# timweiland/DiffEqGMRFs.jl

Hardware: AMD Instinct MI355X
Metric: GMRF posterior solves/sec (mean+samples), 256^2 Darcy (higher is better)
Workload: dtype f64; 1 GPU; darcy256: n=65536, 64 blocks x 1024, nnz=1624084; 256 independent posterior(s) per GPU and step (4 stream(s) x batch 64), each factor + mean + 64 samples; mode=problems, samples_per_problem_per_rank=64, l_blocks_kept=False

## Files before the change

### diffeqgmrfs.jl_amd/_cabi.py

```python
from __future__ import annotations

import ctypes as C
import os
from typing import Optional

_HERE = os.path.dirname(os.path.abspath(__file__))
LIB_PATH = os.environ.get("GMRF_HIP_LIBRARY") or os.path.join(_HERE, "csrc", "libgmrf_hip.so")

GMRF_OK = 0
ERR_NOT_SPD, ERR_BAD_SHAPE, ERR_BAND, ERR_HIP, ERR_NO_FACTOR, ERR_NO_DEVICE, ERR_ALLOC, ERR_RCCL = -1, -2, -3, -4, -5, -6, -7, -8
SOLVE_FULL, SOLVE_FORWARD, SOLVE_BACKWARD = 0, 1, 2
VAR_EXACT, VAR_RBMC, VAR_MC = 0, 1, 2
BLOCK_L, BLOCK_C, BLOCK_LINV = 0, 1, 2
ORDER_REFERENCE, ORDER_TWISTED = 0, 1

EXPORTS = [
    "gmrf_bt_create", "gmrf_bt_destroy", "gmrf_last_error", "gmrf_version",
    "gmrf_bt_factor_csc", "gmrf_bt_factor_blocks", "gmrf_bt_refactor_values",
    "gmrf_bt_solve", "gmrf_bt_sample", "gmrf_bt_posterior", "gmrf_bt_set_factor_rhs", "gmrf_bt_normals", "gmrf_bt_marginal_var",
    "gmrf_bt_var_accumulate", "gmrf_bt_logdet", "gmrf_bt_get_block", "gmrf_bt_factor_buffer",
    "gmrf_bt_adopt_shape", "gmrf_bt_adopt_commit", "gmrf_bt_adopt_layout", "gmrf_bt_get_layout", "gmrf_bt_block_range",
    "gmrf_bt_set_keep_l", "gmrf_bt_storage_bytes", "gmrf_bt_set_storage", "gmrf_bt_factor_begin_csc",
    "gmrf_bt_factor_step_async", "gmrf_bt_factor_end", "gmrf_bt_stats",
    "gmrf_bt_set_profiling", "gmrf_bt_set_eager", "gmrf_bt_synchronize", "gmrf_bt_set_batch", "gmrf_bt_select_problem",
    "gmrf_bt_marginal_var_batch", "gmrf_bt_selinv", "gmrf_bt_trace_inv", "gmrf_bt_set_order", "gmrf_bt_get_order", "gmrf_bt_half_stats", "gmrf_bt_export_size", "gmrf_bt_export_factor", "gmrf_bt_import_factor",
    "gmrf_comm_unique_id", "gmrf_comm_create", "gmrf_comm_destroy", "gmrf_comm_bcast_host", "gmrf_comm_allreduce_sum",
    "gmrf_bt_bcast_blocks_async", "gmrf_bt_allgather_blocks_async", "gmrf_comm_wait", "gmrf_comm_bytes", "gmrf_streams_create", "gmrf_streams_destroy",
    "gmrf_bt_packed_size", "gmrf_bt_pack_blocks_async", "gmrf_bt_unpack_blocks_async",
    "gmrf_csr_create", "gmrf_csr_destroy", "gmrf_spmm", "gmrf_spmm_rows", "gmrf_spmm_async", "gmrf_spmm_rows_async",
    "gmrf_darcy_p1_create", "gmrf_darcy_p2_create", "gmrf_darcy_p1_destroy", "gmrf_darcy_p1_pattern", "gmrf_darcy_p1_assemble",
    "gmrf_burgers_p1_create", "gmrf_burgers_p2_create", "gmrf_burgers_line_create", "gmrf_burgers_colloc_create", "gmrf_burgers_p1_destroy", "gmrf_burgers_p1_pattern", "gmrf_burgers_p1_tangent",
    "gmrf_shallow_water_p1_create", "gmrf_shallow_water_p1_destroy", "gmrf_shallow_water_p1_pattern", "gmrf_shallow_water_p1_qpoints",
    "gmrf_shallow_water_p1_assemble", "gmrf_shallow_water_p1_operators",
    "gmrf_assemble_create", "gmrf_assemble_destroy", "gmrf_assemble_pattern", "gmrf_assemble_precision", "gmrf_assemble_rhs",
    "gmrf_burgers_p1_tangent_batch", "gmrf_assemble_precision_batch", "gmrf_assemble_rhs_batch", "gmrf_assemble_objective_batch",
    "gmrf_gn_create", "gmrf_gn_destroy", "gmrf_gn_run", "gmrf_gn_finalize",
    "gmrf_elliptic_p1_create", "gmrf_elliptic_p2_create", "gmrf_elliptic_p1_destroy", "gmrf_elliptic_p1_pattern", "gmrf_elliptic_p1_qpoints",
    "gmrf_elliptic_p1_tangent", "gmrf_elliptic_p1_tangent_batch", "gmrf_elliptic_p1_load", "gmrf_gn_create_elliptic",
    "gmrf_darcy_p1_assemble_batch", "gmrf_dc_create", "gmrf_dc_destroy", "gmrf_dc_run",
    "gmrf_burgers_prior_create", "gmrf_burgers_line_prior_create", "gmrf_burgers_prior_destroy", "gmrf_burgers_prior_pattern", "gmrf_burgers_prior_values_batch",
    "gmrf_bic_create", "gmrf_bic_destroy", "gmrf_bic_run", "gmrf_field_errors_batch",
    "gmrf_bt_logdet_batch", "gmrf_assemble_quadform_batch", "gmrf_gn_posterior",
    "gmrf_test_gemm", "gmrf_test_gemm_desc", "gmrf_test_gemm_pair", "gmrf_test_gemm_rate", "gmrf_test_gemm_shapes", "gmrf_test_potrf_tile", "gmrf_test_potrf_block", "gmrf_test_potrf_route", "gmrf_test_tile_timing", "gmrf_test_persist_stamps", "gmrf_test_persist_aborts", "gmrf_test_factor_fwd", "gmrf_test_gn_route", "gmrf_test_dc_route", "gmrf_test_bic_route", "gmrf_test_var_groups", "gmrf_test_persist_budget", "gmrf_test_clock_probe_start", "gmrf_test_clock_probe_finish",
    "gmrf_test_mfma_f64_rate", "gmrf_test_hbm_rate", "gmrf_test_microbench", "gmrf_test_symbolic_csc",
]


class SparseBlock(C.Structure):
    _fields_ = [("nnz", C.c_int64), ("ptr", C.c_void_p), ("idx", C.c_void_p), ("val", C.c_void_p)]


class Stats(C.Structure):
    _fields_ = [
        ("factor_ms", C.c_double), ("solve_ms", C.c_double), ("sample_ms", C.c_double),
        ("factor_flops", C.c_double), ("sweep_bytes", C.c_double), ("sweep_ms", C.c_double),
        ("n", C.c_int64), ("n_blocks", C.c_int64), ("block_size", C.c_int64),
        ("block_size_padded", C.c_int64), ("factor_bytes", C.c_int64),
        ("kernel_ms", C.c_double * 24), ("kernel_work", C.c_double * 24), ("kernel_launches", C.c_int64 * 24),
        ("sweep_bytes_streamed", C.c_double),
        ("persist_route", C.c_int32), ("persist_aborts", C.c_int32), ("persist_cus", C.c_int32), ("persist_refused", C.c_int32),
        ("sweep_persist", C.c_int32), ("sweep_persist_launches", C.c_int32),
    ]


class GmrfError(RuntimeError):
    def __init__(self, status: int, msg: str, info: int = 0):
        super().__init__(f"libgmrf_hip status {status}: {msg}")
        self.status = status
        self.info = info


class NotPositiveDefinite(GmrfError):
    """Julia's PosDefException(info): `.info` is the failing block (1-based)."""


_lib: Optional[C.CDLL] = None


def load() -> C.CDLL:
    global _lib
    if _lib is not None:
        return _lib
    if not os.path.exists(LIB_PATH):
        raise ImportError(
            f"{LIB_PATH} is missing: build it with `python -c 'import __graft_entry__ as g; g.build()'` "
            "or `make -C diffeqgmrfs.jl_amd/csrc` (the HIP library is the only compute path)")
    try:
        import torch
    except Exception:
        pass
    lib = C.CDLL(LIB_PATH)
    vp, i32, i64, u64, dbl = C.c_void_p, C.c_int32, C.c_int64, C.c_uint64, C.c_double
    P = C.POINTER
    sigs = {
        "gmrf_bt_create": [i32, vp, P(vp)],
        "gmrf_bt_destroy": [vp],
        "gmrf_version": [],
# ... 65 lines not shown
        "gmrf_burgers_p1_create": [i32, vp, i64, i64, dbl, dbl, P(vp)],
        "gmrf_burgers_p2_create": [i32, vp, i64, i64, dbl, dbl, P(vp)],
        "gmrf_burgers_line_create": [i32, vp, i64, i64, dbl, dbl, i32, i32, i32, dbl, P(vp)],
        "gmrf_burgers_colloc_create": [i32, vp, i64, i64, dbl, dbl, dbl, i64, vp, P(vp)],
        "gmrf_burgers_p1_destroy": [vp],
        "gmrf_burgers_p1_pattern": [vp, P(i64), vp, vp, i32],
        "gmrf_burgers_p1_tangent": [vp, vp, vp, vp],
        "gmrf_burgers_p1_tangent_batch": [vp, i64, vp, vp, vp],
        "gmrf_assemble_precision_batch": [vp, i64, vp, i64, vp, dbl, vp],
        "gmrf_assemble_rhs_batch": [vp, i64, vp, vp, vp, vp, dbl, vp],
        "gmrf_assemble_objective_batch": [vp, i64, vp, i64, vp, vp, vp, dbl, vp],
        "gmrf_gn_create": [vp, vp, vp, P(vp)],
        "gmrf_gn_create_elliptic": [vp, vp, vp, P(vp)],
        "gmrf_elliptic_p1_create": [i32, vp, i64, i64, P(vp)],
        "gmrf_elliptic_p2_create": [i32, vp, i64, i64, P(vp)],
        "gmrf_elliptic_p1_destroy": [vp],
        "gmrf_elliptic_p1_pattern": [vp, P(i64), vp, vp, i32],
        "gmrf_elliptic_p1_qpoints": [vp, vp],
        "gmrf_elliptic_p1_tangent": [vp, vp, vp, vp],
        "gmrf_elliptic_p1_tangent_batch": [vp, i64, vp, vp, vp],
        "gmrf_elliptic_p1_load": [vp, i64, vp, vp],
        "gmrf_gn_destroy": [vp],
        "gmrf_gn_run": [vp, vp, i64, vp, vp, vp, vp, dbl, dbl, i32, vp, vp, P(i32)],
        "gmrf_gn_finalize": [vp, P(i32)],
        "gmrf_darcy_p1_assemble_batch": [vp, i64, vp, i64, dbl, vp, vp],
        "gmrf_dc_create": [vp, vp, vp, P(vp)],
        "gmrf_dc_destroy": [vp],
        "gmrf_dc_run": [vp, vp, i64, dbl, vp, i64, vp, dbl, i64, u64, i32, i64, u64, vp, vp, vp, vp, P(i32)],
        "gmrf_burgers_prior_create": [i32, vp, i64, i64, dbl, dbl, dbl, P(vp)],
        "gmrf_burgers_line_prior_create": [i32, vp, i64, i64, dbl, dbl, dbl, i32, i32, dbl, dbl, i32, P(vp)],
        "gmrf_burgers_prior_destroy": [vp],
        "gmrf_burgers_prior_pattern": [vp, P(i64), vp, vp, i32],
        "gmrf_burgers_prior_values_batch": [vp, i64, vp, vp, vp, vp],
        "gmrf_bic_create": [vp, vp, vp, P(vp)],
        "gmrf_bic_destroy": [vp],
        "gmrf_bic_run": [vp, vp, vp, vp, vp, vp, P(i32)],
        "gmrf_field_errors_batch": [i32, vp, i64, i64, i64, vp, vp, vp],
        "gmrf_bt_logdet_batch": [vp, vp],
        "gmrf_assemble_quadform_batch": [vp, i64, vp, i64, vp, vp, vp],
        "gmrf_gn_posterior": [vp, vp, i64, i64, u64, i32, i64, u64, vp, vp, vp, vp, vp, vp, vp, P(i32)],
        "gmrf_shallow_water_p1_create": [i32, vp, i64, i64, P(vp)],
        "gmrf_shallow_water_p1_destroy": [vp],
        "gmrf_shallow_water_p1_pattern": [vp, i32, P(i64), vp, vp, i32],
        "gmrf_shallow_water_p1_qpoints": [vp, vp],
        "gmrf_shallow_water_p1_assemble": [vp, vp, dbl, dbl, dbl, vp, vp, vp, vp],
        "gmrf_shallow_water_p1_operators": [vp, vp, vp, vp, vp, dbl, dbl, dbl, vp, vp, vp, vp],
        "gmrf_spmm": [vp, vp, vp, i64, i64, i64],
        "gmrf_spmm_async": [vp, vp, vp, i64, i64, i64],
        "gmrf_spmm_rows_async": [vp, vp, vp, i64, i64, i64],
        "gmrf_spmm_rows": [vp, vp, vp, i64, i64, i64],
        "gmrf_test_gemm": [i32, i64, i64, i64, i32, i32, i32, i32, dbl, vp, i64, vp, i64, dbl, vp, i64],
        "gmrf_test_gemm_shapes": [vp, P(dbl), i64, P(i64)],
        "gmrf_test_gemm_desc": [i32, i32, vp, vp] + [vp, i64] * 12 + [P(i32)],
        "gmrf_test_gemm_pair": [i32, i32, i32, vp, vp, vp, vp, vp, vp, vp, vp],
        "gmrf_test_gemm_rate": [i32, i64, i64, i64, i32, i32, i32, i32, i32, i32, P(dbl)],
        "gmrf_test_potrf_tile": [i32, vp, vp, P(i32)],
        "gmrf_test_potrf_block": [i32, i64, vp, vp, P(i32)],
        "gmrf_test_potrf_route": [i32, i64, i32, i32, i64, i32, vp, vp, vp, P(i32), P(i32)],
        "gmrf_test_tile_timing": [vp, i32],
        "gmrf_test_persist_stamps": [vp, i32],
        "gmrf_test_persist_aborts": [vp, vp],
        "gmrf_test_factor_fwd": [vp, vp, vp],
        "gmrf_test_gn_route": [vp, P(i32), P(i32)],
        "gmrf_test_dc_route": [vp, vp],
        "gmrf_test_bic_route": [vp, vp],
        "gmrf_test_var_groups": [vp, vp, vp],
        "gmrf_test_persist_budget": [i32, i32, vp, vp],
        "gmrf_test_clock_probe_start": [i32, i32, i32, P(vp)],
        "gmrf_test_clock_probe_finish": [vp, vp, vp],
        "gmrf_test_mfma_f64_rate": [i32, P(dbl)],
        "gmrf_test_hbm_rate": [i32, i64, P(dbl)],
        "gmrf_test_microbench": [i32, vp, i32],
        "gmrf_test_symbolic_csc": [i64, i64, vp, vp, i32, vp],
    }
    for name, args in sigs.items():
        fn = getattr(lib, name)
        fn.argtypes = args
        fn.restype = i32
    lib.gmrf_last_error.argtypes = []
    lib.gmrf_last_error.restype = C.c_char_p
    _lib = lib
    return lib


def check(status: int, info: int = 0):
    if status == GMRF_OK:
        return
    msg = load().gmrf_last_error().decode(errors="replace")
    if status == ERR_NOT_SPD:
        raise NotPositiveDefinite(status, msg, info)
    raise GmrfError(status, msg, info)


def ptr(a) -> C.c_void_p:
    if a is None:
        return C.c_void_p(0)
    if isinstance(a, int):
        return C.c_void_p(a)
    if hasattr(a, "data_ptr"):
        return C.c_void_p(a.data_ptr())
    return C.c_void_p(a.ctypes.data)
```

### diffeqgmrfs.jl_amd/api.py

```python
from __future__ import annotations

import ctypes as C
from typing import List, Optional, Sequence, Tuple

import numpy as np
import scipy.sparse as sp

from . import _cabi
from ._cabi import GmrfError, NotPositiveDefinite


def _is_torch(x) -> bool:
    return hasattr(x, "data_ptr") and hasattr(x, "device")


def _colmajor(b, n: int):
    if _is_torch(b):
        import torch
        if b.dtype != torch.float64:
            raise TypeError("float64 required")
        if b.dim() == 1:
            if b.shape[0] != n:
                raise ValueError("dimension mismatch")
            return b.contiguous(), 1, n, True
# ... 1147 lines not shown
    def trace_inv(self, S: CsrMatrix, dvals):
        nd = 2 if self.batch == 1 else 3
        if dvals.ndim != nd or dvals.shape[-1] != S.nnz or (nd == 3 and dvals.shape[0] != self.batch):
            want = "(m, nnz)" if nd == 2 else "(batch, m, nnz)"
            raise ValueError(f"dvals must be {want} with nnz = {S.nnz}")
        m = int(dvals.shape[-2])
        if _is_torch(dvals):
            import torch
            if dvals.dtype != torch.float64:
                raise TypeError("float64 required")
            dvals = dvals.contiguous()
            out = torch.empty(dvals.shape[:-1], dtype=torch.float64, device=dvals.device)
        else:
            dvals = np.ascontiguousarray(dvals, dtype=np.float64)
            out = np.empty(dvals.shape[:-1], dtype=np.float64)
        _cabi.check(self._lib.gmrf_bt_trace_inv(self._h, S._h, _cabi.ptr(dvals), m, _cabi.ptr(out)))
        return out

    @staticmethod
    def _out_array(out, shape):
        if out is None:
            return np.empty(shape, dtype=np.float64)
        ok = tuple(out.shape) == shape and (out.is_contiguous() and str(out.dtype) == "torch.float64" if _is_torch(out)
                                            else out.flags.c_contiguous and out.dtype == np.float64)
        if not ok:
            raise ValueError(f"out must be a contiguous float64 array of shape {shape}")
        return out

    def var_accumulate(self, acc, method: str, first_id: int, k: int, seed: int = 0x5EED,
                       Q: Optional[CsrMatrix] = None):
        m = {"rbmc": _cabi.VAR_RBMC, "mc": _cabi.VAR_MC}[method]
        _cabi.check(self._lib.gmrf_bt_var_accumulate(self._h, m, first_id, k, seed,
                                                     Q._h if Q is not None else None, _cabi.ptr(acc)))
        return acc

    def stats(self) -> dict:
        s = _cabi.Stats()
        _cabi.check(self._lib.gmrf_bt_stats(self._h, C.byref(s)))
        out = {}
        for f, _ in s._fields_:
            v = getattr(s, f)
            out[f] = list(v) if hasattr(v, "__len__") else v
        return out

    def gemm_shapes(self) -> list:
        n = C.c_int64(0)
        _cabi.check(self._lib.gmrf_test_gemm_shapes(self._h, None, 0, C.byref(n)))
        buf = np.zeros((max(int(n.value), 1), 11))
        _cabi.check(self._lib.gmrf_test_gemm_shapes(self._h, buf.ctypes.data_as(C.POINTER(C.c_double)), buf.shape[0], C.byref(n)))
        names = ("class", "M", "N", "K", "tri", "lower_only", "problems", "k_bounds")
        return [dict({k: int(r[i]) for i, k in enumerate(names)}, launches=int(r[8]), ms=float(r[9]), flops=float(r[10]))
                for r in buf[: int(n.value)]]

    def set_profiling(self, level: int):
        _cabi.check(self._lib.gmrf_bt_set_profiling(self._h, level))

    def set_eager(self, eager: bool):
        _cabi.check(self._lib.gmrf_bt_set_eager(self._h, int(eager)))

    def synchronize(self):
        _cabi.check(self._lib.gmrf_bt_synchronize(self._h))

    def factor_buffer(self, kind: int) -> Tuple[int, int]:
        p = C.c_void_p()
        nbytes = C.c_int64(0)
        _cabi.check(self._lib.gmrf_bt_factor_buffer(self._h, kind, C.byref(p), C.byref(nbytes)))
        return int(p.value or 0), int(nbytes.value)

    def export_factor(self) -> np.ndarray:
        nbytes = C.c_int64(0)
        _cabi.check(self._lib.gmrf_bt_export_size(self._h, C.byref(nbytes)))
        buf = np.empty(nbytes.value, dtype=np.uint8)
        _cabi.check(self._lib.gmrf_bt_export_factor(self._h, _cabi.ptr(buf), nbytes.value))
        return buf

    def import_factor(self, image: np.ndarray):
        image = np.ascontiguousarray(image, dtype=np.uint8)
        _cabi.check(self._lib.gmrf_bt_import_factor(self._h, _cabi.ptr(image), image.size))
        hdr = image[:64].view(np.int64)
        self._set_shape(int(hdr[2]), int(hdr[3]))
        return self

    def adopt_shape(self, n: int, n_blocks: int):
        _cabi.check(self._lib.gmrf_bt_adopt_shape(self._h, n, n_blocks))
        self._set_shape(n, n_blocks)

    def get_layout(self) -> np.ndarray:
        cnt = C.c_int64(0)
        _cabi.check(self._lib.gmrf_bt_get_layout(self._h, None, 0, C.byref(cnt)))
        out = np.zeros(cnt.value, dtype=np.int64)
        _cabi.check(self._lib.gmrf_bt_get_layout(self._h, _cabi.ptr(out), out.size, C.byref(cnt)))
        return out

    def adopt_layout(self, n: int, n_blocks: int, layout=None):
        if layout is None:
            _cabi.check(self._lib.gmrf_bt_adopt_layout(self._h, n, n_blocks, None, 0))
        else:
            lay = np.ascontiguousarray(layout, dtype=np.int64)
            _cabi.check(self._lib.gmrf_bt_adopt_layout(self._h, n, n_blocks, _cabi.ptr(lay), lay.size))
        self._set_shape(n, n_blocks)

    def adopt_commit(self, l_blocks_valid: bool = False):
        _cabi.check(self._lib.gmrf_bt_adopt_commit(self._h, int(l_blocks_valid)))

    def set_keep_l(self, keep: bool):
        _cabi.check(self._lib.gmrf_bt_set_keep_l(self._h, int(keep)))
# ... 177 lines not shown
```

### diffeqgmrfs.jl_amd/csrc/gemm_f64.hpp

```cpp
#pragma once
#include <hip/hip_runtime.h>
#include <hip/hip_ext.h>
#include <stdint.h>
#include <stdlib.h>
#include <algorithm>
#include <array>
#include <map>
#include <mutex>
#include <vector>

namespace gmrf {

typedef double v4d __attribute__((ext_vector_type(4)));
typedef double v2d __attribute__((ext_vector_type(2)));

enum : int {
    TRI_A_LOWER = 1,
    TRI_A_UPPER = 2,
    TRI_B_LOWER = 4,
    TRI_B_UPPER = 8
};

struct GemmDirectOut {
    double* samples;
    double* mean;
    int64_t ld, k;
};

struct GemmArgs {
    const double* A;
    const double* B;
    double* C;
    int64_t lda, ldb, ldc;
    int64_t strideA, strideB, strideC;
    int64_t pA, pB, pC;
    int nb1;
    int M, N, K;
    int tri;
    int lower_only;
    double alpha, beta;
    const double* D;
    int64_t ldd, pD;
    unsigned long long* stamps;
    const int* kb_m = nullptr;
    const int* kb_n = nullptr;
    const int* ke_n = nullptr;
    const double* tA = nullptr;
    double* tC = nullptr;
    const double* tD = nullptr;
    int64_t ptA = 0, ptC = 0, ptD = 0;
    double tbeta = 0.0;
    const GemmDirectOut* dout = nullptr;
    int64_t o_j0 = 0, o_n = 0;
    int o_cols = 0;
};

constexpr int GEMM_BM = 64;
constexpr int GEMM_BN = 64;

template <bool ROWS_CONTIG, int BK>
__device__ __forceinline__ void gemm_load_tile(const double* __restrict__ P, int64_t ld, int row0, int k0,
                                               int t, v2d (&rg)[BK / 8]) {
    if (!ROWS_CONTIG) {
        constexpr int TPR = BK / 2, RPP = 256 / TPR;
        const int r = t / TPR, kk = (t % TPR) * 2;
        const double* p = P + (int64_t)(row0 + r) * ld + k0 + kk;
#pragma unroll
        for (int i = 0; i < BK / 8; ++i) rg[i] = *reinterpret_cast<const v2d*>(p + (int64_t)(i * RPP) * ld);
    } else {
        const int kk = t >> 5, r = (t & 31) * 2;
        const double* p = P + (int64_t)(k0 + kk) * ld + row0 + r;
#pragma unroll
        for (int i = 0; i < BK / 8; ++i) rg[i] = *reinterpret_cast<const v2d*>(p + (int64_t)(i * 8) * ld);
    }
}

template <bool ROWS_CONTIG, int BK>
__device__ __forceinline__ void gemm_tile_offsets(int64_t ld, int row0, int t, uint32_t (&off)[BK / 8]) {
    if (!ROWS_CONTIG) {
        constexpr int TPR = BK / 2, RPP = 256 / TPR;
        const int r = t / TPR, kk = (t % TPR) * 2;
#pragma unroll
        for (int i = 0; i < BK / 8; ++i) off[i] = (uint32_t)(((int64_t)(row0 + r + i * RPP) * ld + kk) * 8);
    } else {
        const int kk = t >> 5, r = (t & 31) * 2;
#pragma unroll
        for (int i = 0; i < BK / 8; ++i) off[i] = (uint32_t)(((int64_t)(kk + i * 8) * ld + row0 + r) * 8);
    }
}
template <bool ROWS_CONTIG>
__device__ __forceinline__ const char* gemm_tile_base(const double* P, int64_t ld, int k0) {
    return reinterpret_cast<const char*>(ROWS_CONTIG ? P + (int64_t)k0 * ld : P + k0);
}
template <int BK>
__device__ __forceinline__ void gemm_load_tile_off(const char* base, uint32_t (&off)[BK / 8], v2d (&rg)[BK / 8]) {
#pragma unroll
    for (int i = 0; i < BK / 8; ++i) {
        asm volatile("" : "+v"(off[i]));
        rg[i] = *reinterpret_cast<const v2d*>(base + off[i]);
// ... 632 lines not shown
```

### diffeqgmrfs.jl_amd/csrc/gemm_f64_dma.hpp

```cpp
#pragma once
#include "gemm_f64.hpp"

namespace gmrf {

constexpr int DMA_BK = 16;
constexpr int DMA_ROWS_ASCENDING = 1024;
#ifndef GMRF_DMA_READS_FIRST
#define GMRF_DMA_READS_FIRST 0
#endif

template <int BM, int BN>
constexpr size_t gemm_dma_lds_bytes(int stages) { return (size_t)stages * (BM + BN) * DMA_BK * sizeof(double); }

#define GMRF_LDS_PTR(p) ((__attribute__((address_space(3))) void*)(p))
#define GMRF_GLB_PTR(p) ((const __attribute__((address_space(1))) void*)(p))

template <int BM, int BN>
__device__ __forceinline__ void gemm_dma_tile_order(const GemmArgs& g, int bid, int gdim, int& bm, int& bn, int& z) {
    const int nx = g.N / BN, ny = g.M / BM;
    int tpp;
    if (g.lower_only == 1) {
        if (BM >= BN) tpp = (BM / BN) * ny * (ny + 1) / 2;
        else tpp = 0;
    } else tpp = nx * ny;
// ... 4 lines not shown
    if (g.lower_only == 1) {
        constexpr int R = BM / BN > 0 ? BM / BN : 1;
        const int tile = q % tpp;
        zq = q / tpp;
        const int tr = (g.tri & DMA_ROWS_ASCENDING) ? tile : tpp - 1 - tile;
        int b = (int)((sqrtf(8.0f * (float)(tr / R) + 1.0f) - 1.0f) * 0.5f);
        while (R * b * (b + 1) / 2 > tr) --b;
        while (R * (b + 1) * (b + 2) / 2 <= tr) ++b;
        bm = b;
        bn = tr - R * b * (b + 1) / 2;
    } else {
        const bool cls_n = (g.tri & (TRI_B_LOWER | TRI_B_UPPER)) || !(g.tri & (TRI_A_LOWER | TRI_A_UPPER));
        const bool desc = cls_n ? ((g.tri & TRI_B_UPPER) != 0 || (g.ke_n && !g.kb_n)) : (g.tri & TRI_A_LOWER) != 0;
        const int ncls = cls_n ? nx : ny, other = cls_n ? ny : nx;
        int c = q / (other * nzg);
        const int rem = q % (other * nzg);
        const int o = rem % other;
        zq = rem / other;
        if (desc) c = ncls - 1 - c;
        bn = cls_n ? c : o;
        bm = cls_n ? o : c;
    }
    z = xg + groups * zq;
}

template <int BM, int BN, bool B_N, int STAGES, bool A_T, bool TAIL, bool DOUT>
__device__ __forceinline__ void gemm_dma_body(const GemmArgs& g, const int bid, const int gdim) {
    constexpr int BK = DMA_BK;
    constexpr int MI = BM / 32, NJ = BN / 32;
    constexpr int NA = BM / 32, NB = BN / 32;
    constexpr int A_ST = BM * BK, B_ST = BN * BK, T_ST = TAIL ? BK : 0, ST = A_ST + B_ST + T_ST;
    static_assert(NJ % 2 == 0 || !B_N, "the [k][n] image pairs neighbouring column tiles");
    static_assert(MI % 2 == 0 || !A_T, "the [k][m] image pairs neighbouring row tiles");
    static_assert(!TAIL || (BM == 64 && BN == 64 && !A_T), "the tail row: 64 x 64 tiles");
    static_assert(!DOUT || (TAIL && B_N), "direct output: the tail-row product on B [k][n]");
    int bm, bn, z;
    gemm_dma_tile_order<BM, BN>(g, bid, gdim, bm, bn, z);
    const bool tail_owner = TAIL && (g.lower_only == 1 ? bm == bn : bm == g.M / BM - 1);
    const bool tail = DOUT || tail_owner;
    const int m0 = bm * BM, n0 = bn * BN;
    if (g.lower_only == 2 && n0 > m0 + BM - 1) return;
    const int zi = z % g.nb1, zp = z / g.nb1;
    const double* __restrict__ A = g.A + (int64_t)zi * g.strideA + (int64_t)zp * g.pA;
    const double* __restrict__ B = g.B + (int64_t)zi * g.strideB + (int64_t)zp * g.pB;
    double* C = g.C + (int64_t)zi * g.strideC + (int64_t)zp * g.pC;
    const double* Dm = g.D ? g.D + (int64_t)zp * g.pD : C;
    const int64_t ldd = g.D ? g.ldd : g.ldc;

    int kb = 0, ke = g.K;
    if (g.tri & TRI_A_LOWER) ke = min(ke, m0 + BM);
    if (g.tri & TRI_A_UPPER) kb = max(kb, m0);
    if (g.tri & TRI_B_LOWER) kb = max(kb, n0);
    if (g.tri & TRI_B_UPPER) ke = min(ke, n0 + BN);
    if (g.kb_m) kb = max(kb, g.kb_m[bm * (BM / 64)]);
    if (g.kb_n) kb = max(kb, g.kb_n[bn * (BN / 64)]);
    if (g.ke_n) ke = min(ke, g.ke_n[bn * (BN / 64) + BN / 64 - 1]);
    const int nkt = (ke > kb) ? (ke - kb) / BK : 0;

    extern __shared__ __attribute__((aligned(16))) double gsm[];
    const int t = threadIdx.x;
    const int lane = t & 63, w = __builtin_amdgcn_readfirstlane(t >> 6);
    const int wm = (w >> 1) * (BM / 2), wn = (w & 1) * (BN / 2);
    const int li = lane & 15, lq = lane >> 4;
    const bool idle = g.lower_only != 0 && ((n0 + wn) / 64 > (m0 + wm + BM / 2 - 1) / 64);

    uint32_t offa[NA], offb[NB];
#pragma unroll
    for (int i = 0; i < NA; ++i) {
        const int q = w + 4 * i;
        if (A_T) {
            constexpr int LPR = BM / 2;
            const int k = q * (64 / LPR) + lane / LPR, col = (lane % LPR) * 2;
            offa[i] = (uint32_t)(((int64_t)k * g.lda + m0 + col) * 8);
        } else {
            const int row = 8 * q + (lane >> 3), ch = (lane & 7) ^ ((row >> 1) & 7);
            offa[i] = (uint32_t)(((int64_t)(m0 + row) * g.lda + 2 * ch) * 8);
        }
    }
#pragma unroll
    for (int i = 0; i < NB; ++i) {
        const int q = w + 4 * i;
        if (B_N) {
            constexpr int LPR = BN / 2;
            const int k = q * (64 / LPR) + lane / LPR, col = (lane % LPR) * 2;
            offb[i] = (uint32_t)(((int64_t)k * g.ldb + n0 + col) * 8);
        } else {
            const int row = 8 * q + (lane >> 3), ch = (lane & 7) ^ ((row >> 1) & 7);
            offb[i] = (uint32_t)(((int64_t)(n0 + row) * g.ldb + 2 * ch) * 8);
        }
    }
    const double* arow = g.tC ? g.tA + (int64_t)zp * g.ptA : A + (int64_t)g.M * g.lda;
    auto issue = [&](int kt, int stage) {
        const int k0 = kb + kt * BK;
        const char* abase = reinterpret_cast<const char*>(A_T ? A + (int64_t)k0 * g.lda : A + k0);
        const char* bbase = reinterpret_cast<const char*>(B_N ? B + (int64_t)k0 * g.ldb : B + k0);
        double* as = gsm + stage * ST;
        double* bs = as + A_ST;
        if constexpr (TAIL)
            if (tail && w == 0 && lane < 8)
                __builtin_amdgcn_global_load_lds(GMRF_GLB_PTR(arow + k0 + 2 * lane), GMRF_LDS_PTR(bs + B_ST), 16, 0, 0);
#pragma unroll
        for (int i = 0; i < NA; ++i) {
            asm volatile("" : "+v"(offa[i]));
            __builtin_amdgcn_global_load_lds(GMRF_GLB_PTR(abase + offa[i]), GMRF_LDS_PTR(as + (w + 4 * i) * 128), 16, 0, 0);
        }
#pragma unroll
        for (int i = 0; i < NB; ++i) {
            asm volatile("" : "+v"(offb[i]));
            __builtin_amdgcn_global_load_lds(GMRF_GLB_PTR(bbase + offb[i]), GMRF_LDS_PTR(bs + (w + 4 * i) * 128), 16, 0, 0);
// ... 193 lines not shown
                    if (beta != 0.0) v += beta * Dm[(int64_t)g.M * ldd + n0 + lane];
                    C[(int64_t)g.M * g.ldc + n0 + lane] = v;
                }
            }
        }
    }
}

__global__ void set_direct_out(GemmDirectOut* o, double* samples, double* mean, int64_t ld, int64_t k) {
    o->samples = samples; o->mean = mean; o->ld = ld; o->k = k;
}

template <int BM, int BN, bool B_N, int STAGES, bool A_T = false, bool TAIL = false, bool DOUT = false>
__global__ __launch_bounds__(256, (BM + BN > 128) ? 3 : 4) void gemm_f64_dma(GemmArgs g) {
    gemm_dma_body<BM, BN, B_N, STAGES, A_T, TAIL, DOUT>(g, (int)blockIdx.x, (int)gridDim.x);
}

template <int STAGES>
__global__ __launch_bounds__(256, 4) void gemm_f64_dma_grouped(GemmArgs g0, GemmArgs g1, int wg0, int wg1, int b_n) {
    const bool second = (int)blockIdx.x >= wg0;
    const GemmArgs g = second ? g1 : g0;
    const int bid = second ? (int)blockIdx.x - wg0 : (int)blockIdx.x, gdim = second ? wg1 : wg0;
    if ((b_n >> (second ? 1 : 0)) & 1) gemm_dma_body<64, 64, true, STAGES, false, false, false>(g, bid, gdim);
    else gemm_dma_body<64, 64, false, STAGES, false, false, false>(g, bid, gdim);
}

inline int& gemm_dma_policy() {
    static int v = [] { const char* e = getenv("GMRF_GEMM_DMA"); return e ? atoi(e) : 2; }();
    return v;
}
inline int& gemm_dma_force() {
    static int v = 0;
    return v;
}
inline int gemm_dma_stages() {
    static const int v = [] { const char* e = getenv("GMRF_GEMM_DMA_STAGES"); const int s = e ? atoi(e) : 2; return s == 3 ? 3 : 2; }();
    return v;
}

inline int gemm_dma_shape(bool a_t, const GemmArgs& g, int batch) {
    const int policy = gemm_dma_force() ? 2 : gemm_dma_policy();
    if (policy == 0 || g.stamps || (g.tri & ~15) || g.K % DMA_BK || g.M % 64 || g.N % 64) return 0;
    if ((g.lda & 1) || (g.ldb & 1) || ((uintptr_t)g.A & 15) || ((uintptr_t)g.B & 15) || ((g.strideA | g.strideB | g.pA | g.pB) & 1)) return 0;
    if (((uintptr_t)g.C & 15) || (g.ldc & 1) || ((g.strideC | g.pC) & 1)) return 0;
    if (g.D && (((uintptr_t)g.D & 15) || (g.ldd & 1) || (g.pD & 1))) return 0;
    if ((int64_t)g.M * g.ldc * 8 >= ((int64_t)1 << 32) || (g.D && (int64_t)g.M * g.ldd * 8 >= ((int64_t)1 << 32))) return 0;
    if ((int64_t)(a_t ? g.K : g.M) * g.lda * 8 >= ((int64_t)1 << 32) || (int64_t)std::max(g.N, g.K) * g.ldb * 8 >= ((int64_t)1 << 32)) return 0;
    if (a_t) return 1;
    const int force = gemm_dma_force();
    if (force == 2 && g.M % 128 == 0) return 2;
    if (force == 3 && g.N % 128 == 0 && !g.lower_only) return 3;
    if (force) return 1;
    if (policy == 1) return 1;
    const bool plain = !g.lower_only && !g.tri && !g.kb_m && !g.kb_n && !g.ke_n;
    const int64_t t64 = (int64_t)(g.M / 64) * (g.N / 64) * batch;
    if (policy >= 3 || (plain && t64 >= 2048)) {
        if (g.M % 128 == 0) return 2;
        if (g.N % 128 == 0 && !g.lower_only) return 3;
    }
    return 1;
}
inline bool gemm_uses_dma(bool a_t, const GemmArgs& g, int batch) { return gemm_dma_shape(a_t, g, batch) != 0; }

inline hipError_t gemm_dma_init() {
    hipError_t e = hipSuccess;
#define GMRF_DMA_ATTR(BM, BN, BNAT, ST)                                                                          \
    if (e == hipSuccess)                                                                                          \
        e = hipFuncSetAttribute((const void*)gemm_f64_dma<BM, BN, BNAT, ST>, hipFuncAttributeMaxDynamicSharedMemorySize, \
                                (int)gemm_dma_lds_bytes<BM, BN>(ST) + 64 * 1024);
    GMRF_DMA_ATTR(64, 64, false, 2) GMRF_DMA_ATTR(64, 64, true, 2) GMRF_DMA_ATTR(64, 64, false, 3) GMRF_DMA_ATTR(64, 64, true, 3)
    GMRF_DMA_ATTR(128, 64, false, 2) GMRF_DMA_ATTR(128, 64, true, 2) GMRF_DMA_ATTR(128, 64, false, 3) GMRF_DMA_ATTR(128, 64, true, 3)
    GMRF_DMA_ATTR(64, 128, false, 2) GMRF_DMA_ATTR(64, 128, true, 2) GMRF_DMA_ATTR(64, 128, false, 3) GMRF_DMA_ATTR(64, 128, true, 3)
#undef GMRF_DMA_ATTR
    return e;
}

inline bool gemm_tail_ok(bool a_t, bool b_n, const GemmArgs& g, int batch) {
    if (a_t || gemm_uses_ll(g, batch) || gemm_dma_shape(false, g, batch) != 1) return false;
    if (g.lower_only && g.M != g.N) return false;
    if (g.tC && g.dout) return false;
    if (g.tC) {
        return g.nb1 == 1 && g.tA && ((uintptr_t)g.tA & 15) == 0 && (g.ptA & 1) == 0;
    }
    if (!b_n || g.lower_only) return false;
    if (g.dout && g.nb1 != 1) return false;
    if (g.dout && (g.beta != 0.0 || g.kb_m || g.kb_n || g.ke_n || (g.tri & (TRI_A_LOWER | TRI_A_UPPER)))) return false;
    return (int64_t)(g.M + 1) * g.ldc * 8 < ((int64_t)1 << 32) && (!g.D || (int64_t)(g.M + 1) * g.ldd * 8 < ((int64_t)1 << 32));
}
inline bool gemm_try_dma_tail(hipStream_t st, bool a_t, bool b_n, const GemmArgs& g, int batch, hipEvent_t ev_start, hipEvent_t ev_stop,
                              hipError_t* err) {
    if (!gemm_tail_ok(a_t, b_n, g, batch)) return false;
    const bool tri_grid = g.lower_only && g.M == g.N;
    GemmArgs gs = g;
    gs.lower_only = tri_grid ? 1 : 0;
    static const bool asc_off = [] { const char* e = getenv("GMRF_GEMM_G2_ORDER"); return e && atoi(e) == 0; }();
    if (tri_grid && (g.kb_m || g.kb_n) && !asc_off) gs.tri |= DMA_ROWS_ASCENDING;
    const int64_t nx = g.N / 64, ny = g.M / 64;
    const dim3 grid((unsigned)((tri_grid ? ny * (ny + 1) / 2 : nx * ny) * batch)), block(256);
    const size_t lds = (size_t)gemm_dma_stages() * (64 + 64 + DMA_BK) * DMA_BK * sizeof(double);
#define GMRF_DMA_TK(BNAT, ST)                                                                                              \
    do {                                                                                                                   \
        if (ev_start) hipExtLaunchKernelGGL((gemm_f64_dma<64, 64, BNAT, ST, false, true>), grid, block, lds, st, ev_start, ev_stop, 0, gs); \
        else hipLaunchKernelGGL((gemm_f64_dma<64, 64, BNAT, ST, false, true>), grid, block, lds, st, gs);                \
    } while (0)
#define GMRF_DMA_TKO(ST)                                                                                                   \
    do {                                                                                                                   \
        if (ev_start) hipExtLaunchKernelGGL((gemm_f64_dma<64, 64, true, ST, false, true, true>), grid, block, lds, st, ev_start, ev_stop, 0, gs); \
        else hipLaunchKernelGGL((gemm_f64_dma<64, 64, true, ST, false, true, true>), grid, block, lds, st, gs);          \
    } while (0)
    if (g.dout) {
        if (gemm_dma_stages() == 3) GMRF_DMA_TKO(3); else GMRF_DMA_TKO(2);
    } else if (gemm_dma_stages() == 3) {
        if (b_n) GMRF_DMA_TK(true, 3); else GMRF_DMA_TK(false, 3);
    } else {
        if (b_n) GMRF_DMA_TK(true, 2); else GMRF_DMA_TK(false, 2);
    }
#undef GMRF_DMA_TKO
#undef GMRF_DMA_TK
    *err = hipGetLastError();
    return true;
}

inline bool gemm_try_dma(hipStream_t st, bool a_t, bool b_n, const GemmArgs& g, int batch, hipEvent_t ev_start, hipEvent_t ev_stop,
                         hipError_t* err) {
    const int shape = gemm_dma_shape(a_t, g, batch);
    if (shape == 0) return false;
    const bool tri_grid = g.lower_only && g.M == g.N;
    GemmArgs gs = g;
    gs.lower_only = tri_grid ? 1 : (g.lower_only ? 2 : 0);
    static const bool asc_off = [] { const char* e = getenv("GMRF_GEMM_G2_ORDER"); return e && atoi(e) == 0; }();
    if (tri_grid && (g.kb_m || g.kb_n) && !asc_off) gs.tri |= DMA_ROWS_ASCENDING;
    const int stages = gemm_dma_stages();
    const dim3 block(256);
#define GMRF_DMA_GO(BM, BN)                                                                                       \
    do {                                                                                                          \
        const int64_t nx = g.N / BN, ny = g.M / BM;                                                               \
        const int64_t tiles = tri_grid ? (int64_t)(BM / BN > 0 ? BM / BN : 1) * ny * (ny + 1) / 2 : nx * ny;      \
        const dim3 grid((unsigned)(tiles * batch));                                                               \
        static const size_t lds_pad = [] { const char* e = getenv("GMRF_GEMM_DMA_LDS_PAD_KB"); return (size_t)(e ? atoi(e) : 0) * 1024; }();    \
// ... 61 lines not shown
```

### diffeqgmrfs.jl_amd/csrc/gmrf_hip.hip

```cpp
#include <hip/hip_runtime.h>
#include <dlfcn.h>
#include <stdint.h>
#include <stdlib.h>
#include <string.h>
#include <time.h>

#include <algorithm>
#include <atomic>
#include <iterator>
#include <cmath>
#include <map>
#include <memory>
#include <chrono>
#include <functional>
#include <initializer_list>
#include <mutex>
#include <string>
#include <type_traits>
#include <vector>

#include "../../include/gmrf_hip.h"
#include "assemble.hpp"
#include "fem_assemble.hpp"
#include "burgers_line.hpp"
// ... 81 lines not shown
    float* d_vals32 = nullptr;
    double* d_diag = nullptr;
    bool tiles128_ok = false;
    bool tiles_ok = false;
    DevBuf stage_x, stage_y;
    int plan_state = 0;
    int64_t* d_tile_uptr = nullptr;
    int32_t* d_ucols = nullptr;
    uint16_t* d_lidx = nullptr;
    int64_t n_ucols = 0;
    int plan_rows = 0, plan_ucap = 0, plan_ecap = 0, plan_ecap_pad = 0, plan_umax = 0;
    uint64_t id = 0;
};
static std::atomic<uint64_t> g_csr_ids{0};

struct EvPair {
    hipEvent_t a, b;
    int kind;
    double work;
    int shape = -1;
};

struct GemmShapeStat {
    int64_t key[8];
    double launches = 0, ms = 0, work = 0;
};

struct TwistState;

struct gmrf_handle {
    int device = 0;
    hipStream_t stream = nullptr;
    bool own_stream = false;
    int64_t n = 0, N = 0, bs = 0, bsp = 0, n_pad = 0;
    int64_t B = 1;
    int64_t sel = 0;
    int64_t alloc_B = 0, vals_B = 0;
    int64_t nnz_in = 0, n_entries = 0;
    uint64_t* d_keys = nullptr;
    double* d_vals = nullptr;
    int64_t* d_src = nullptr;
    double* d_nz_stage = nullptr;
    std::vector<int64_t> diag_first, diag_count, low_first, low_count;
    bool analyzed = false;
    int64_t cmin = 0, rmax = 0;
    std::vector<int> kst, mend;
    int* d_kst = nullptr;
    int* d_mend = nullptr;
    int* d_kbx = nullptr;
    int kst_cap = 0;
    double c_streamed = 0.0;
    double g2_tile_k = 0.0;
    bool c_dirty = false;
    int* d_lo_rowptr = nullptr;
    int* d_dg_rowptr = nullptr;
    int* d_bxt_uptr = nullptr; int* d_bxt_ucols = nullptr; uint16_t* d_bxt_lidx = nullptr; int* d_bxt_gtiles = nullptr;
    std::vector<int> bxt_ng;
    int bxt_ecap = 0; int bxt_nrt = 0; bool bxt_plan_ok = false;
    int64_t lo_row_max = 0;
    bool sparse_b = false;
    bool dense_g1 = false;
    double *d_L = nullptr, *d_C = nullptr, *d_Linv = nullptr;
    bool external_storage = false;
    bool keep_l = true;
    bool l_valid = false;
    bool logdet_valid = false;
    std::vector<char> got_block;
    int64_t alloc_rm = 0, alloc_wc = 0;
    bool alloc_keep_l = true;
    double *d_S = nullptr, *d_B = nullptr, *d_T = nullptr, *d_W = nullptr;
    double* d_V = nullptr;
    int64_t v_elems = 0;
    uint64_t layout_gen = 0;
    uint64_t sel_csr = 0, sel_gen = ~0ull;
    int64_t sel_nnz = 0;
    std::vector<int64_t> sel_off, sel_nd;
    int64_t* d_sel_src = nullptr;
    int64_t* d_sel_slot = nullptr;
    int64_t sel_cap = 0;
    double* d_sig = nullptr;
    int64_t sig_elems = 0;
    double* d_dv = nullptr;
    int64_t dv_elems = 0;
    int* d_info = nullptr;
    double* d_logdet = nullptr;
    int64_t alloc_N = 0, alloc_bsp = 0;
    bool factored = false;
    double *d_P = nullptr, *d_Y = nullptr, *d_Tp = nullptr;
    int64_t kp_cap = 0;
    double* d_stage = nullptr;
    int64_t stage_cap = 0;
    DevBuf mean_arena;
    double* d_acc = nullptr;
    int64_t acc_B = 0;
    int32_t var_group = 0, var_groups = 0;
    bool eager = false;
    bool split_step = false;
    bool sweep_no_gemm = false;
    bool no_fused_posterior = false;
    bool tail_probe = false;
    bool tail_refused = false;
    const double* frhs = nullptr;
    const double* fy_for = nullptr;
    bool fwd_run = false;
    bool no_factor_fwd = false;
    bool no_grouped_gemm = false;
// ... 113 lines not shown
            (void)hipEventRecord(p.a, h->stream);
        }
    }
    ~ProfScope() {
        if (on) {
            (void)hipEventRecord(p.b, h->stream);
            h->events.push_back(p);
        }
    }
};

static void prof_collect(gmrf_handle* h) {
    for (auto& p : h->events) {
        float ms = 0.f;
        (void)hipEventElapsedTime(&ms, p.a, p.b);
        h->stats.kernel_ms[p.kind] += ms; h->stats.kernel_work[p.kind] += p.work; h->stats.kernel_launches[p.kind]++;
        if (p.shape >= 0) { auto& g = h->gemm_shapes[(size_t)p.shape]; g.launches += 1; g.ms += ms; g.work += p.work; }
        h->ev_pool.push_back(p.a);
        h->ev_pool.push_back(p.b);
    }
    h->events.clear();
}

struct GemmTail {
    const double* A; int64_t pA;
    double* C; int64_t pC;
    const double* D; int64_t pD;
    double beta;
    const GemmDirectOut* out = nullptr;
    int64_t j0 = 0;
    int cols = 0;
};

static inline double gemm_flops(int M, int N, int K, int tri, int lower_only, double nprob) {
    double flops = 2.0 * M * N * (double)K * nprob;
    if (lower_only) flops *= 0.5 * (1.0 + 64.0 / std::max(M, 64));
    if (tri) flops *= 0.5 * (1.0 + 64.0 / std::max(K, 64));
    return flops;
}
static int gemm_shape_row(gmrf_handle* h, const int64_t (&key)[8]) {
    for (size_t i = 0; i < h->gemm_shapes.size(); ++i)
        if (!memcmp(h->gemm_shapes[i].key, key, sizeof(key))) return (int)i;
    GemmShapeStat st; memcpy(st.key, key, sizeof(key));
    h->gemm_shapes.push_back(st);
    return (int)h->gemm_shapes.size() - 1;
}

static gmrf_status gemm(gmrf_handle* h, bool a_t, bool b_n, int M, int N, int K, int tri, int lower_only,
                        double alpha, const double* A, int64_t lda, const double* B, int64_t ldb,
                        double beta, double* C, int64_t ldc, int64_t pA, int64_t pB, int64_t pC,
                        int batch = 1, int64_t sA = 0, int64_t sB = 0, int64_t sC = 0, const double* D = nullptr,
                        int64_t ldd = 0, int64_t pD = 0, int pclass = 0, double pwork = -1.0,
                        const int* kb_m = nullptr, const int* kb_n = nullptr, const int* ke_n = nullptr, bool tail = false,
                        const GemmTail* gt = nullptr) {
    GemmArgs g;
    if (gt) {
        if (gt->C) { g.tA = gt->A; g.ptA = gt->pA; g.tC = gt->C; g.ptC = gt->pC; g.tD = gt->D; g.ptD = gt->pD; g.tbeta = gt->beta; }
        g.dout = gt->out; g.o_j0 = gt->j0; g.o_cols = gt->cols; g.o_n = h->n;
        tail = true;
    }
    g.kb_m = kb_m; g.kb_n = kb_n; g.ke_n = ke_n;
    g.D = D; g.ldd = ldd; g.pD = pD;
    g.A = A; g.B = B; g.C = C;
    g.lda = lda; g.ldb = ldb; g.ldc = ldc;
    g.strideA = sA; g.strideB = sB; g.strideC = sC;
    g.pA = pA; g.pB = pB; g.pC = pC; g.nb1 = batch;
    g.M = M; g.N = N; g.K = K; g.tri = tri; g.lower_only = lower_only;
    g.alpha = alpha; g.beta = beta; g.stamps = nullptr;
    double flops = gemm_flops(M, N, K, tri, lower_only, batch * (double)h->B);
    if (tail) {
        if (!gemm_tail_ok(a_t, b_n, g, batch * (int)h->B)) {
            h->tail_refused = true;
            return h->tail_probe ? GMRF_OK : bad_shape("internal: a product does not qualify for the tail-row GEMM");
        }
        if (h->tail_probe) return GMRF_OK;
        flops *= (M + 1.0) / M;
        if (pwork >= 0.0) pwork *= (M + 1.0) / M;
        pclass = b_n ? 15 : 14;
        hipError_t e = hipSuccess;
        if (h->profiling > 0) {
            EvPair p;
            p.kind = pclass; p.work = pwork >= 0.0 ? pwork : flops;
            p.a = ev_get(h); p.b = ev_get(h);
            const int64_t key[8] = {pclass, M + 1, N, K, tri, lower_only, batch * h->B, (kb_m || kb_n || ke_n) ? 1 : 0};
            p.shape = gemm_shape_row(h, key);
            (void)gemm_try_dma_tail(h->gemm_stream ? h->gemm_stream : h->stream, a_t, b_n, g, batch * (int)h->B, p.a, p.b, &e);
            HIPCHK(e);
            h->events.push_back(p);
            return GMRF_OK;
        }
        (void)gemm_try_dma_tail(h->gemm_stream ? h->gemm_stream : h->stream, a_t, b_n, g, batch * (int)h->B, nullptr, nullptr, &e);
        HIPCHK(e);
        return GMRF_OK;
    }
    if (gemm_uses_big(a_t, g, batch * (int)h->B)) { pclass = b_n ? 7 : 6; pwork = -1.0; }
    else if (pclass == 0) {
        if (gemm_uses_ll(g, batch * (int)h->B)) pclass = 13;
        else if (gemm_uses_dma(a_t, g, batch * (int)h->B)) pclass = a_t ? 18 : (b_n ? 15 : 14);
        else pclass = a_t ? 12 : (b_n ? 11 : 0);
    }
    if (h->profiling > 0) {
        EvPair p;
        p.kind = pclass; p.work = pwork >= 0.0 ? pwork : flops;
        p.a = ev_get(h); p.b = ev_get(h);
        const int64_t key[8] = {pclass, M, N, K, tri, lower_only, batch * h->B, (kb_m || kb_n || ke_n) ? 1 : 0};
        p.shape = gemm_shape_row(h, key);
        HIPCHK(launch_gemm(h->gemm_stream ? h->gemm_stream : h->stream, a_t, b_n, g, batch * (int)h->B, p.a, p.b));
        h->events.push_back(p);
        return GMRF_OK;
    }
    HIPCHK(launch_gemm(h->gemm_stream ? h->gemm_stream : h->stream, a_t, b_n, g, batch * (int)h->B));
    return GMRF_OK;
}

struct GemmOne {
    bool b_n; int M, N, K, tri, lower_only;
    double alpha; const double* A; int64_t lda; const double* B; int64_t ldb; double beta; double* C; int64_t ldc;
    int64_t pA, pB, pC;
    double pwork;
};
static gmrf_status gemm_one(gmrf_handle* h, const GemmOne& q) {
    return gemm(h, false, q.b_n, q.M, q.N, q.K, q.tri, q.lower_only, q.alpha, q.A, q.lda, q.B, q.ldb, q.beta, q.C, q.ldc, q.pA, q.pB, q.pC,
                1, 0, 0, 0, nullptr, 0, 0, 0, q.pwork);
}
static gmrf_status gemm_pair(gmrf_handle* h, const GemmOne& q0, const GemmOne& q1) {
    GemmArgs g[2];
    const GemmOne* q[2] = {&q0, &q1};
    double work[2];
    for (int i = 0; i < 2; ++i) {
        GemmArgs& a = g[i];
        a.A = q[i]->A; a.B = q[i]->B; a.C = q[i]->C; a.lda = q[i]->lda; a.ldb = q[i]->ldb; a.ldc = q[i]->ldc;
        a.strideA = a.strideB = a.strideC = 0;
        a.pA = q[i]->pA; a.pB = q[i]->pB; a.pC = q[i]->pC; a.nb1 = 1;
        a.M = q[i]->M; a.N = q[i]->N; a.K = q[i]->K; a.tri = q[i]->tri; a.lower_only = q[i]->lower_only;
        a.alpha = q[i]->alpha; a.beta = q[i]->beta; a.D = nullptr; a.ldd = 0; a.pD = 0; a.stamps = nullptr;
        work[i] = q[i]->pwork >= 0.0 ? q[i]->pwork : gemm_flops(a.M, a.N, a.K, a.tri, a.lower_only, (double)h->B);
    }
    if (h->no_grouped_gemm || !gemm_grouped_ok(g[0], g[1], (int)h->B)) {
        GCHK(gemm_one(h, q0));
        return gemm_one(h, q1);
    }
    hipStream_t st = h->gemm_stream ? h->gemm_stream : h->stream;
    hipError_t e = hipSuccess;
    if (h->profiling > 0) {
        EvPair p;
        p.kind = 14; p.work = work[0] + work[1];
        p.a = ev_get(h); p.b = ev_get(h);
        const int64_t key[8] = {14, q0.M + q1.M, q0.N, q0.K, q0.tri | (q1.tri << 8), q0.lower_only | (q1.lower_only << 8), h->B, 0};
        p.shape = gemm_shape_row(h, key);
        (void)gemm_try_dma_grouped(st, q0.b_n, g[0], q1.b_n, g[1], (int)h->B, p.a, p.b, &e);
        HIPCHK(e);
        h->events.push_back(p);
        return GMRF_OK;
    }
    (void)gemm_try_dma_grouped(st, q0.b_n, g[0], q1.b_n, g[1], (int)h->B, nullptr, nullptr, &e);
    HIPCHK(e);
    return GMRF_OK;
}

static inline int64_t blk_elems(const gmrf_handle* h) { return h->bsp * h->bsp; }
static inline int64_t c_ld(const gmrf_handle* h) { return h->bsp - h->cmin; }
static inline int64_t c_blk(const gmrf_handle* h) { return h->rmax * (h->bsp - h->cmin); }
static inline int64_t stride_pL(const gmrf_handle* h) { return blk_elems(h) * (h->keep_l ? h->N : 1); }
static inline int64_t stride_pX(const gmrf_handle* h) { return blk_elems(h) * h->N; }
static inline int64_t stride_pC(const gmrf_handle* h) { return c_blk(h) * std::max<int64_t>(h->N - 1, 1); }
static inline double* l_block(const gmrf_handle* h, int64_t i) { return h->d_L + (h->keep_l ? i * blk_elems(h) : 0); }

static gmrf_status set_layout(gmrf_handle* h, int64_t cmin, int64_t rmax, const std::vector<int64_t>& kst_abs) {
    const int64_t bsp = h->bsp;
    if (cmin < 0 || cmin >= bsp || cmin % 64 || rmax <= 0 || rmax > bsp || rmax % 64) return bad_shape("bad coupling-block layout");
    const int nrt = (int)(rmax / 64), nct = (int)((bsp - cmin) / 64), ntile = (int)(bsp / 64);
    if ((int)kst_abs.size() != nrt) return bad_shape("bad coupling-block layout (row tiles)");
    (void)hipStreamSynchronize(h->stream);
    destroy_graphs(h);
    h->cmin = cmin; h->rmax = rmax;
    h->layout_gen++;
    h->kst.assign((size_t)ntile, 0);
    int64_t run = bsp - 64;
    for (int t = nrt - 1; t >= 0; --t) {
        int64_t v = std::min(std::max(kst_abs[t], cmin), bsp - 64);
        run = std::min(run, (v / 64) * 64);
        h->kst[t] = (int)(run - cmin);
    }
    if (nrt > 0) h->kst[0] = 0;
    for (int t = nrt; t < ntile; ++t) h->kst[t] = (int)(bsp - cmin);
    h->mend.assign((size_t)ntile, (int)rmax);
    for (int u = 0; u < nct; ++u) {
        int m = 0;
        for (int t = 0; t < nrt; ++t) if (h->kst[t] <= 64 * u) m = 64 * (t + 1);
        h->mend[u] = m;
    }
    h->c_streamed = 0.0; h->g2_tile_k = 0.0;
    for (int t = 0; t < nrt; ++t) {
        h->c_streamed += 64.0 * (double)(bsp - cmin - h->kst[t]);
        h->g2_tile_k += (double)(t + 1) * (double)(bsp - cmin - h->kst[t]);
    }
    if (!h->d_kst || !h->d_mend || h->kst_cap < ntile) {
        free_dev(h->d_kst); free_dev(h->d_mend); free_dev(h->d_kbx); h->d_kst = h->d_mend = h->d_kbx = nullptr; h->kst_cap = 0;
        HIPCHK(hipMalloc(&h->d_kst, sizeof(int) * ntile));
        HIPCHK(hipMalloc(&h->d_mend, sizeof(int) * ntile));
        HIPCHK(hipMalloc(&h->d_kbx, sizeof(int) * ntile));
        h->kst_cap = ntile;
    }
    {
        std::vector<int> kbx((size_t)ntile);
        for (int u = 0; u < ntile; ++u) kbx[(size_t)u] = (int)std::max<int64_t>(0, 64 * (int64_t)u - cmin);
        HIPCHK(hipMemcpyAsync(h->d_kbx, kbx.data(), sizeof(int) * ntile, hipMemcpyHostToDevice, h->stream));
        HIPCHK(hipStreamSynchronize(h->stream));
    }
    HIPCHK(hipMemcpyAsync(h->d_kst, h->kst.data(), sizeof(int) * ntile, hipMemcpyHostToDevice, h->stream));
    HIPCHK(hipMemcpyAsync(h->d_mend, h->mend.data(), sizeof(int) * ntile, hipMemcpyHostToDevice, h->stream));
    HIPCHK(hipStreamSynchronize(h->stream));
    h->c_dirty = true;
    return GMRF_OK;
}

static gmrf_status set_layout_dense(gmrf_handle* h) {
    return set_layout(h, 0, h->bsp, std::vector<int64_t>((size_t)(h->bsp / 64), 0));
}

static gmrf_status alloc_work(gmrf_handle* h);
static gmrf_status alloc_factor(gmrf_handle* h) {
    if (h->alloc_N == h->N && h->alloc_bsp == h->bsp && h->alloc_B == h->B && h->alloc_rm == h->rmax &&
        h->alloc_wc == c_ld(h) && h->alloc_keep_l == h->keep_l && h->d_Linv)
        return GMRF_OK;
    destroy_graphs(h);
    h->logdet_valid = false;
    if (h->external_storage) {
        if (h->alloc_N != h->N || h->alloc_bsp != h->bsp || h->alloc_B != h->B || h->alloc_keep_l != h->keep_l) {
// ... 62 lines not shown
    if (h->n != n || h->N != N) {
        (void)hipStreamSynchronize(h->stream);
        destroy_graphs(h);
        release_shape_buffers(h);
        h->factored = false;
        h->analyzed = false;
    }
    h->n = n; h->N = N; h->bs = bs;
    h->layout_gen++;
    h->bsp = 64 * next_pow2((bs + 63) / 64);
    h->n_pad = h->bsp * N;
    h->stats.n = n; h->stats.n_blocks = N; h->stats.block_size = bs; h->stats.block_size_padded = h->bsp;
    h->stats.factor_flops = ((double)N * bs * bs * bs / 3.0 + (double)(N - 1) * 2.0 * bs * bs * bs) * (double)h->B;
    return GMRF_OK;
}

static gmrf_status ensure_panels(gmrf_handle* h, int64_t kp) {
    if (kp <= h->kp_cap && h->d_P) return GMRF_OK;
    for (auto& kv : h->sweep_graphs) (void)hipGraphExecDestroy(kv.second);
    h->sweep_graphs.clear();
    free_dev(h->d_P); free_dev(h->d_Y); free_dev(h->d_Tp);
    h->d_P = h->d_Y = h->d_Tp = nullptr;
    HIPCHK(hipMalloc(&h->d_P, sizeof(double) * kp * h->n_pad * h->B));
    HIPCHK(hipMalloc(&h->d_Y, sizeof(double) * kp * h->n_pad * h->B));
    HIPCHK(hipMalloc(&h->d_Tp, sizeof(double) * kp * h->bsp * h->B));
    h->kp_cap = kp;
    return GMRF_OK;
}

static gmrf_status ensure_stage(gmrf_handle* h, int64_t elems) {
    if (elems <= h->stage_cap && h->d_stage) return GMRF_OK;
    free_dev(h->d_stage);
    h->d_stage = nullptr;
    HIPCHK(hipMalloc(&h->d_stage, sizeof(double) * elems));
    h->stage_cap = elems;
    return GMRF_OK;
}

struct HostEntry { uint64_t key; int64_t src; };

struct SymbolicPlan {
    std::vector<int64_t> diag_first, diag_count, low_first, low_count;
    std::vector<uint64_t> keys;
    std::vector<int64_t> src;
    int64_t cmin = 0, rmax = 0;
    std::vector<int64_t> first;
    std::vector<int> rowptr;
    int64_t max_row = 0;
    bool sparse_b = false, bxt_ok = false;
    std::vector<int> uptr, ucols, gtiles, ng;
    std::vector<uint16_t> lidx;
    int ecap = 0, nrt = 0;
    std::vector<int> drowptr;
};

static void build_symbolic(int64_t N, int64_t bsp, const std::vector<std::vector<HostEntry>>& dg,
                           const std::vector<std::vector<HostEntry>>& lo, bool no_staircase, SymbolicPlan& sp, bool group_tiles = true) {
    sp.diag_first.assign((size_t)N, 0); sp.diag_count.assign((size_t)N, 0);
    sp.low_first.assign((size_t)N, 0); sp.low_count.assign((size_t)N, 0);
    auto& keys = sp.keys; auto& src = sp.src;
    keys.clear(); src.clear();
    for (int64_t i = 0; i < N; ++i) {
        sp.diag_first[i] = (int64_t)keys.size(); sp.diag_count[i] = (int64_t)dg[i].size();
        {
            std::vector<HostEntry> drow(dg[i]);
            std::stable_sort(drow.begin(), drow.end(), [](const HostEntry& x, const HostEntry& y) { return x.key < y.key; });
            for (auto& e : drow) { keys.push_back(e.key); src.push_back(e.src); }
        }
        sp.low_first[i] = (int64_t)keys.size(); sp.low_count[i] = (int64_t)lo[i].size();
        std::vector<HostEntry> byrow(lo[i]);
        std::stable_sort(byrow.begin(), byrow.end(), [](const HostEntry& x, const HostEntry& y) { return x.key < y.key; });
        for (auto& e : byrow) { keys.push_back(e.key); src.push_back(e.src); }
    }
    {
        int64_t cmin = bsp, rmax = 0;
        std::vector<int64_t> first((size_t)(bsp / 64), bsp);
        for (int64_t i = 1; i < N; ++i)
            for (auto& e : lo[i]) {
                const int64_t r = (int64_t)(e.key >> 32), c = (int64_t)(e.key & 0xffffffffu);
                cmin = std::min(cmin, c); rmax = std::max(rmax, r + 1);
                first[(size_t)(r / 64)] = std::min(first[(size_t)(r / 64)], c);
            }
        if (rmax == 0) { cmin = 0; rmax = 64; first[0] = 0; }
        cmin = (cmin / 64) * 64;
        rmax = std::min<int64_t>(bsp, (rmax + 63) / 64 * 64);
        first.resize((size_t)(rmax / 64));
        if (no_staircase) std::fill(first.begin(), first.end(), cmin);
        sp.cmin = cmin; sp.rmax = rmax; sp.first = first;
    }
    sp.rowptr.assign((size_t)(N * (bsp + 1)), 0);
    int64_t max_row = 0;
    for (int64_t i = 1; i < N; ++i) {
        int* rp = sp.rowptr.data() + i * (bsp + 1);
        const int64_t first = sp.low_first[i], cnt = sp.low_count[i];
        for (int64_t k = 0; k < cnt; ++k) rp[(keys[first + k] >> 32) + 1]++;
        for (int64_t r = 0; r < bsp; ++r) max_row = std::max<int64_t>(max_row, rp[r + 1]);
        rp[0] = (int)first;
        for (int64_t r = 0; r < bsp; ++r) rp[r + 1] += rp[r];
    }
    sp.drowptr.assign((size_t)(N * (bsp + 1)), 0);
    if (keys.size() < ((size_t)1 << 31)) {
        for (int64_t i = 0; i < N; ++i) {
            int* rp = sp.drowptr.data() + i * (bsp + 1);
            const int64_t first = sp.diag_first[i], cnt = sp.diag_count[i];
            for (int64_t k = 0; k < cnt; ++k) rp[(keys[first + k] >> 32) + 1]++;
            rp[0] = (int)first;
            for (int64_t r = 0; r < bsp; ++r) rp[r + 1] += rp[r];
        }
    }
    sp.max_row = max_row;
    sp.sparse_b = keys.size() < ((size_t)1 << 31) && max_row <= 32 && bsp >= 64;
    sp.bxt_ok = false; sp.uptr.clear(); sp.ucols.clear(); sp.lidx.clear(); sp.gtiles.clear(); sp.ng.clear();
    if (sp.sparse_b && N > 1) {
        static const bool no_groups = [] { const char* e = getenv("GMRF_BXT_GROUPS"); return e && atoi(e) == 0; }();
        const int nrt = (int)(sp.rmax / 64);
        sp.uptr.assign((size_t)(N * (nrt + 1)), 0);
        sp.gtiles.assign((size_t)(N * nrt * 3), -1);
        sp.ng.assign((size_t)N, 0);
        sp.lidx.assign(std::max<size_t>(keys.size(), 1), 0);
        std::vector<std::vector<int>> cols((size_t)nrt);
        std::vector<int> uni, tmp;
        bool ok = true;
        int64_t pmax = 0;
        for (int64_t i = 1; i < N && ok; ++i) {
            const int* rp = sp.rowptr.data() + i * (bsp + 1);
            for (int rt = 0; rt < nrt; ++rt) {
                auto& c = cols[(size_t)rt];
                c.clear();
                for (int e = rp[rt * 64]; e < rp[rt * 64 + 64]; ++e) c.push_back((int)(keys[(size_t)e] & 0xffffffffu));
                std::sort(c.begin(), c.end());
                c.erase(std::unique(c.begin(), c.end()), c.end());
                if ((int)c.size() > BXT_UCAP) ok = false;
            }
            if (!ok) break;
            std::vector<char> taken((size_t)nrt, 0);
            int g = 0;
            for (int rt = 0; rt < nrt; ++rt) {
                if (taken[(size_t)rt]) continue;
                int* gt = sp.gtiles.data() + ((size_t)i * nrt + g) * 3;
                int cnt = 0;
                gt[cnt++] = rt; taken[(size_t)rt] = 1;
                uni = cols[(size_t)rt];
                for (int u = rt + 1; u < nrt && cnt < 3 && !no_groups && group_tiles; ++u) {
                    if (taken[(size_t)u] || cols[(size_t)u].empty()) continue;
                    tmp.clear();
                    std::set_union(uni.begin(), uni.end(), cols[(size_t)u].begin(), cols[(size_t)u].end(), std::back_inserter(tmp));
                    const size_t common = uni.size() + cols[(size_t)u].size() - tmp.size();
                    if (2 * common >= cols[(size_t)u].size() && tmp.size() <= (size_t)BXT_UCAP) {
                        gt[cnt++] = u; taken[(size_t)u] = 1;
                        uni.swap(tmp);
                    }
                }
                int64_t padded = 0;
                for (int q = 0; q < cnt; ++q) {
                    const int t = gt[q];
                    for (int e = rp[t * 64]; e < rp[t * 64 + 64]; ++e)
                        sp.lidx[(size_t)e] = (uint16_t)(std::lower_bound(uni.begin(), uni.end(), (int)(keys[(size_t)e] & 0xffffffffu)) - uni.begin());
                    for (int r = t * 64; r < t * 64 + 64; ++r) padded += (rp[r + 1] - rp[r] + 3) / 4 * 4;
                }
                pmax = std::max(pmax, padded);
                sp.uptr[(size_t)(i * (nrt + 1) + g)] = (int)sp.ucols.size();
                sp.ucols.insert(sp.ucols.end(), uni.begin(), uni.end());
                ++g;
            }
            sp.uptr[(size_t)(i * (nrt + 1) + g)] = (int)sp.ucols.size();
            for (int q = g + 1; q <= nrt; ++q) sp.uptr[(size_t)(i * (nrt + 1) + q)] = (int)sp.ucols.size();
            sp.ng[(size_t)i] = g;
        }
        const int ecap = (int)std::max<int64_t>(64, (pmax + 63) / 64 * 64);
        if (ok && bxt_tile_lds_bytes(ecap) <= 53 * 1024) { sp.bxt_ok = true; sp.ecap = ecap; sp.nrt = nrt; }
    }
}

static gmrf_status upload_entries(gmrf_handle* h, const std::vector<std::vector<HostEntry>>& dg,
                                  const std::vector<std::vector<HostEntry>>& lo, int64_t nnz_in) {
    const int64_t N = h->N;
    SymbolicPlan sp;
    build_symbolic(N, h->bsp, dg, lo, h->no_staircase, sp, h->B >= 8);
    h->diag_first = sp.diag_first; h->diag_count = sp.diag_count; h->low_first = sp.low_first; h->low_count = sp.low_count;
    const auto& keys = sp.keys; const auto& src = sp.src;
    GCHK(set_layout(h, sp.cmin, sp.rmax, sp.first));
    free_dev(h->d_keys); free_dev(h->d_vals); free_dev(h->d_src); free_dev(h->d_nz_stage);
    h->d_keys = nullptr; h->d_vals = nullptr; h->d_src = nullptr; h->d_nz_stage = nullptr;
    h->n_entries = (int64_t)keys.size();
    h->nnz_in = nnz_in;
    const size_t ne = std::max<size_t>(keys.size(), 1);
    HIPCHK(hipMalloc(&h->d_keys, ne * sizeof(uint64_t)));
    HIPCHK(hipMalloc(&h->d_vals, ne * sizeof(double) * h->B));
    HIPCHK(hipMalloc(&h->d_src, ne * sizeof(int64_t)));
    HIPCHK(hipMalloc(&h->d_nz_stage, std::max<int64_t>(nnz_in, 1) * sizeof(double) * h->B));
    h->vals_B = h->B;
    if (!keys.empty()) {
        HIPCHK(hipMemcpyAsync(h->d_keys, keys.data(), keys.size() * sizeof(uint64_t), hipMemcpyHostToDevice, h->stream));
        HIPCHK(hipMemcpyAsync(h->d_src, src.data(), src.size() * sizeof(int64_t), hipMemcpyHostToDevice, h->stream));
        HIPCHK(hipStreamSynchronize(h->stream));
    }
    free_dev(h->d_lo_rowptr);
    h->d_lo_rowptr = nullptr;
    HIPCHK(hipMalloc(&h->d_lo_rowptr, sp.rowptr.size() * sizeof(int)));
    HIPCHK(hipMemcpyAsync(h->d_lo_rowptr, sp.rowptr.data(), sp.rowptr.size() * sizeof(int), hipMemcpyHostToDevice, h->stream));
    free_dev(h->d_dg_rowptr);
    h->d_dg_rowptr = nullptr;
    HIPCHK(hipMalloc(&h->d_dg_rowptr, sp.drowptr.size() * sizeof(int)));
    HIPCHK(hipMemcpyAsync(h->d_dg_rowptr, sp.drowptr.data(), sp.drowptr.size() * sizeof(int), hipMemcpyHostToDevice, h->stream));
    HIPCHK(hipStreamSynchronize(h->stream));
    h->lo_row_max = sp.max_row;
    h->sparse_b = sp.sparse_b;
    free_dev(h->d_bxt_uptr); free_dev(h->d_bxt_ucols); free_dev(h->d_bxt_lidx); free_dev(h->d_bxt_gtiles);
    h->d_bxt_uptr = nullptr; h->d_bxt_ucols = nullptr; h->d_bxt_lidx = nullptr; h->d_bxt_gtiles = nullptr; h->bxt_plan_ok = false;
    if (sp.bxt_ok) {
        HIPCHK(hipMalloc(&h->d_bxt_gtiles, sp.gtiles.size() * sizeof(int)));
        HIPCHK(hipMemcpyAsync(h->d_bxt_gtiles, sp.gtiles.data(), sp.gtiles.size() * sizeof(int), hipMemcpyHostToDevice, h->stream));
        h->bxt_ng = sp.ng;
        HIPCHK(hipMalloc(&h->d_bxt_uptr, sp.uptr.size() * sizeof(int)));
        HIPCHK(hipMalloc(&h->d_bxt_ucols, std::max<size_t>(sp.ucols.size(), 1) * sizeof(int)));
        HIPCHK(hipMalloc(&h->d_bxt_lidx, sp.lidx.size() * sizeof(uint16_t)));
        HIPCHK(hipMemcpyAsync(h->d_bxt_uptr, sp.uptr.data(), sp.uptr.size() * sizeof(int), hipMemcpyHostToDevice, h->stream));
        if (!sp.ucols.empty()) HIPCHK(hipMemcpyAsync(h->d_bxt_ucols, sp.ucols.data(), sp.ucols.size() * sizeof(int), hipMemcpyHostToDevice, h->stream));
        HIPCHK(hipMemcpyAsync(h->d_bxt_lidx, sp.lidx.data(), sp.lidx.size() * sizeof(uint16_t), hipMemcpyHostToDevice, h->stream));
        HIPCHK(hipStreamSynchronize(h->stream));
        h->bxt_ecap = sp.ecap; h->bxt_nrt = sp.nrt; h->bxt_plan_ok = true;
    }
    h->analyzed = true;
    h->factored = false;
    return GMRF_OK;
}

static gmrf_status split_csc(int64_t n, int64_t N, int64_t bs, const int64_t* colptr, const int64_t* rowval, int32_t base,
                             std::vector<std::vector<HostEntry>>& dg, std::vector<std::vector<HostEntry>>& lo) {
    dg.assign((size_t)N, {}); lo.assign((size_t)N, {});
    if (colptr[0] != base) return bad_shape("colptr must start at the index base");
    for (int64_t c = 0; c < n; ++c) {
        const int64_t bj = c / bs;
        if (colptr[c + 1] < colptr[c]) return bad_shape("colptr must be non-decreasing");
// ... 175 lines not shown
            want = want_f;
            ok = persist_budget_claim(g_persist_claims[h->device], h, want, h->cu_count, persist_margin());
        }
    }
    h->sweep_persist_planned = ok && want_s > 0 && want >= want_s;
    const int got = ok ? want : 0;
    if (got != h->persist_cus) destroy_graphs(h);
    h->persist_cus = got;
    h->stats.persist_cus = got;
    h->stats.persist_refused = (want > 0 && !ok) ? 1 : 0;
}
static void persist_release(gmrf_handle* h) {
    std::lock_guard<std::mutex> lock(g_persist_mu);
    auto it = g_persist_claims.find(h->device);
    if (it != g_persist_claims.end()) it->second.erase(h);
    h->persist_cus = 0;
    h->stats.persist_cus = 0;
    h->sweep_persist_planned = false;
}

static void persist_give_up(gmrf_handle* h) {
    h->persist_gave_up = true; h->persist_aborts++;
    h->stats.persist_aborts = h->persist_aborts;
    persist_release(h);
    destroy_graphs(h);
}

static bool persist_fits(const gmrf_handle* h, int nt, int j0, int j1, int xrows) {
    if (h->no_persist || h->persist_gave_up || h->persist_cus <= 0) return false;
    return (int64_t)(1 + persist_tiles(nt, j0, j1, xrows)) * h->B <= h->persist_cus;
}

static gmrf_status launch_persist(gmrf_handle* h, double* S, double* L, double* X, int nt, int j0, int j1, int xrows, int blk_id,
                                  double flops) {
    const int words = persist_flag_words(nt);
    if (!h->d_pflags || h->pflags_words < (int64_t)words * h->B) return bad_shape("internal: flag words of the persistent launches not allocated");
    PersistArgs pa;
    pa.S = S; pa.L = L; pa.X = X; pa.ld = h->bsp; pa.nt = nt; pa.j0 = j0; pa.j1 = j1; pa.xrows = xrows;
    pa.tail_panel = (!xrows && j1 < nt) ? 1 : 0;
    pa.info = h->d_info; pa.blk = blk_id;
    pa.pS = h->bsp * h->bsp; pa.pL = stride_pL(h); pa.pX = stride_pX(h); pa.blk_per_problem = (int)h->N;
    pa.flags = h->d_pflags; pa.flag_stride = words;
    pa.abort_word = reinterpret_cast<unsigned*>(h->d_info + 1);
    static const int limit_ms = [] { const char* e = getenv("GMRF_PERSIST_SPIN_MS"); return e ? atoi(e) : -1; }();
    pa.spin_limit = (unsigned)(limit_ms >= 0 ? limit_ms : (h->B > 1 ? 200 : 2000)) * 100000u;
    pa.stamps = h->dbg_stamps;
    h->persist_launched = true;
    h->stats.persist_route = xrows == 1 ? 1 : (xrows == 0 ? 2 : 3);
    ProfScope ps(h, 17, flops);
    hipLaunchKernelGGL(potrf_persist<false>, dim3(1 + persist_tiles(nt, j0, j1, xrows), (unsigned)h->B), dim3(POTRF_PERSIST_THREADS), POTRF_PERSIST_LDS,
                       h->stream, pa);
    HIPCHK(hipGetLastError());
    return GMRF_OK;
}

static gmrf_status potrf_block(gmrf_handle* h, double* S, double* L, double* X, double* T, int blk_id, double* fy = nullptr) {
    const int bsp = (int)h->bsp;
    const int64_t ld = bsp;
    const int nt = bsp / 64;
    const int route = potrf_route(h);
    const bool fused = route == ROUTE_FUSED;
    if (h->xsplit > 0 && route != ROUTE_PANELS256) return bad_shape("internal: split inverse planned off the 256-column panel route");
    static const int pw_env = [] { const char* e = getenv("GMRF_PANEL_TILES"); return e ? atoi(e) : 4; }();
    const int pw = (!fused && nt >= 8) ? ((pw_env == 2 || pw_env == 8) ? pw_env : 4) : nt;
    const bool fused_in_panel = route == ROUTE_BIG_ONE;
    const bool overlap = h->capturing && h->fork_graph && nt >= 8;
    if (overlap && !h->aux) HIPCHK(hipStreamCreateWithFlags(&h->aux, hipStreamNonBlocking));
    hipEvent_t ev_fork = nullptr, ev_join = nullptr;
    if (overlap) { GCHK(fork_event(h, &ev_fork)); GCHK(fork_event(h, &ev_join)); }
    if (fused && !h->no_lookahead && !h->doubling_x && !overlap && nt >= 2 && persist_fits(h, nt, 0, nt, 1)) {
        const double t3 = 64.0 * 64.0 * 64.0;
        double fl = t3 / 3.0 * nt;
        for (int j = 0; j + 1 < nt; ++j) {
            const int m = nt - j - 1;
            fl += (double)m * t3 + 2.0 * t3 * (m * (m + 1) / 2) + 2.0 * t3 * (0.5 * (double)(j + 1) * (j + 2) + 0.625 * (j + 1));
        }
        return launch_persist(h, S, L, X, nt, 0, nt, 1, blk_id, fl);
    }
    if (fused && !h->no_lookahead && !h->doubling_x && !overlap && nt >= 2) {
        StepArgs sa;
        sa.S = S; sa.L = L; sa.X = X; sa.ld = ld; sa.nt = nt; sa.cend = nt;
        sa.info = h->d_info; sa.blk = blk_id; sa.dbg = nullptr;
        sa.pS = (int64_t)bsp * bsp; sa.pL = stride_pL(h); sa.pX = stride_pX(h); sa.blk_per_problem = (int)h->N;
        const double t3 = 64.0 * 64.0 * 64.0;
        {
            sa.j = 0; sa.lookahead = 0; sa.xrow = -1;
            ProfScope ps(h, 1, t3 / 3.0);
            hipLaunchKernelGGL(potrf_step<false>, dim3(1, 1), dim3(256), POTRF_TILE_LDS, h->stream, sa);
        }
        for (int j = 0; j + 1 < nt; ++j) {
            const int m = nt - j - 1, ntile_wg = m * (m + 1) / 2;
            sa.j = j; sa.lookahead = 1;
            sa.xrow = (j >= 1) ? j : -1; sa.xrow_first = ntile_wg;
            const int nx_wg = (j >= 1) ? 4 * j : 0;
            const double f_x = (j >= 1) ? 2.0 * t3 * (0.5 * (double)j * (j + 1) + 0.625 * j) : 0.0;
            ProfScope ps(h, 1, t3 / 3.0 + (double)m * t3 + 2.0 * t3 * ntile_wg + f_x);
            hipLaunchKernelGGL(potrf_step<false>, dim3(ntile_wg + nx_wg, 1), dim3(256), POTRF_STEP_LDS, h->stream, sa);
        }
        {
            sa.j = nt - 1; sa.lookahead = 0; sa.xrow = nt - 1; sa.xrow_first = 0;
            ProfScope ps(h, 1, 2.0 * t3 * (0.5 * (double)(nt - 1) * nt + 0.625 * (nt - 1)));
            hipLaunchKernelGGL(potrf_step<false>, dim3(4 * (nt - 1), 1), dim3(256), 64 * 18 * sizeof(double), h->stream, sa);
        }
        HIPCHK(hipGetLastError());
        return GMRF_OK;
    }
// ... 3 lines not shown
        sa.S = S; sa.L = L; sa.X = X; sa.ld = ld; sa.nt = nt; sa.cend = nt;
        sa.info = h->d_info; sa.blk = blk_id; sa.dbg = nullptr;
        sa.pS = (int64_t)bsp * bsp; sa.pL = stride_pL(h); sa.pX = stride_pX(h); sa.blk_per_problem = (int)h->N;
        const int64_t pW = (int64_t)bsp * bsp;
        const double t3 = 64.0 * 64.0 * 64.0, nb = (double)h->B;
        auto diag128 = [&](int j) -> gmrf_status {
            sa.j = j;
            ProfScope ps(h, 16, (2.0 * t3 / 3.0 + 4.0 * 2.0 * t3 * 0.625) * nb);
            static const size_t lds_pad = [] { const char* e = getenv("GMRF_DIAG128_LDS_PAD_KB"); return (size_t)(e ? atoi(e) : 0) * 1024; }();
            static const bool fat = [] { const char* e = getenv("GMRF_DIAG128_FAT"); return e && atoi(e) != 0; }();
            if (fat) hipLaunchKernelGGL(potrf_diag128, dim3(1, (unsigned)h->B), dim3(256), POTRF_DIAG128_LDS + lds_pad, h->stream, sa);
            else hipLaunchKernelGGL(potrf_diag128_slim, dim3(1, (unsigned)h->B), dim3(256), POTRF_DIAG128_SLIM_LDS + lds_pad, h->stream, sa);
            HIPCHK(hipGetLastError());
            return GMRF_OK;
        };
        static const bool no_small = [] { const char* e = getenv("GMRF_PERSIST_PANELS"); return e && atoi(e) == 0; }();
        const bool persist_panels = !no_small && !h->no_persist_panels && persist_fits(h, 4, 0, 4, 2);
        for (int j = 0; j < nt; j += 4) {
            const int64_t oa = (int64_t)j * 64, ob = oa + 128, oc = oa + 256;
            if (persist_panels) {
                const double fl = (4.0 * t3 / 3.0 + 2.0 * t3 * (6.0 * 0.625 + 10.0 + 10.0 + 6.0 * 0.625)) * nb;
                GCHK(launch_persist(h, S + oa * ld + oa, L + oa * ld + oa, X + oa * ld + oa, 4, 0, 4, 2, blk_id, fl));
            } else {
                GCHK(diag128(j));
                GCHK(gemm(h, false, false, 128, 128, 128, TRI_B_UPPER, 0, 1.0, S + ob * ld + oa, ld, X + oa * ld + oa, ld, 0.0, L + ob * ld + oa, ld,
                          sa.pS, sa.pX, sa.pL, 1, 0, 0, 0, nullptr, 0, 0, 0, 2.0 * t3 * 3.0 * 2.0 * nb));
                GCHK(gemm_pair(h,
                               GemmOne{false, 128, 128, 128, 0, 1, -1.0, L + ob * ld + oa, ld, L + ob * ld + oa, ld, 1.0, S + ob * ld + ob, ld,
                                       sa.pL, sa.pL, sa.pS, 2.0 * t3 * 2.0 * 3.0 * nb},
                               GemmOne{true, 128, 128, 128, TRI_B_LOWER, 0, 1.0, L + ob * ld + oa, ld, X + oa * ld + oa, ld, 0.0, T + ob * ld + oa, ld,
                                       sa.pL, sa.pX, pW, -1.0}));
                GCHK(diag128(j + 2));
                GCHK(gemm(h, false, true, 128, 128, 128, TRI_A_LOWER, 0, -1.0, X + ob * ld + ob, ld, T + ob * ld + oa, ld, 0.0, X + ob * ld + oa, ld,
                          sa.pX, pW, sa.pX));
            }
            const int m3 = nt - j - 4;
            const int64_t pT = bsp, pY = h->n_pad;
            if (m3 <= 0) {
                if (fy) {
                    SweepArgs sw;
                    sw.Mat = X + oa * ld + oa; sw.ld = ld; sw.Xin = h->d_ft + oa; sw.ldx = pT; sw.Bin = nullptr; sw.ldb = 0;
                    sw.Out = fy + oa; sw.ldo = pY; sw.rows = 256; sw.kdim = 256; sw.sub = 0;
                    sw.pMat = sa.pX; sw.pXin = pT; sw.pBin = 0; sw.pOut = pY;
                    ProfScope ps(h, 3, 4.0 * 256.0 * 257.0 * nb);
                    HIPCHK(launch_sweep(h->stream, false, true, 1, sw, (int)h->B));
                }
                continue;
            }
            const GemmTail tp{h->d_ft + oa, pT, fy + oa, pY, nullptr, 0, 0.0};
            const GemmTail tu{fy + oa, pY, h->d_ft + oc, pT, nullptr, 0, 1.0};
            const bool in_slot = (j == 0 && h->xsplit == 256 && !h->keep_l);
            double* Lb = in_slot ? X + oc * ld + oa : L + oc * ld + oa;
            const int64_t pLb = in_slot ? sa.pX : sa.pL;
            GCHK(gemm(h, false, false, 64 * m3, 256, 256, TRI_B_UPPER, 0, 1.0, S + oc * ld + oa, ld, X + oa * ld + oa, ld, 0.0, Lb, ld,
                      sa.pS, sa.pX, pLb, 1, 0, 0, 0, nullptr, 0, 0, 0, 2.0 * t3 * 10.0 * m3 * nb, nullptr, nullptr, nullptr, false,
                      fy ? &tp : nullptr));
            GCHK(gemm(h, false, false, m3 * 64, m3 * 64, 256, 0, 1, -1.0, Lb, ld, Lb, ld, 1.0, S + oc * ld + oc, ld, pLb, pLb, sa.pS,
                      1, 0, 0, 0, nullptr, 0, 0, 0, 2.0 * t3 * 4.0 * (m3 * (m3 + 1) / 2) * nb, nullptr, nullptr, nullptr, false,
                      fy ? &tu : nullptr));
        }
        const int p = h->xsplit;
        GCHK(doubling_levels(h, L, X, T, 256, bsp / 2, -1, p));
        if (p > 0 && !(p == 256 && !h->keep_l)) {
            hipLaunchKernelGGL(copy_rect, dim3((unsigned)((bsp - p) / 4), (unsigned)h->B), dim3(256), 0, h->stream,
                               L + (int64_t)p * ld, ld, sa.pL, X + (int64_t)p * ld, ld, sa.pX, bsp - p, p);
            HIPCHK(hipGetLastError());
        }
        return GMRF_OK;
    }
    if (h->xsplit > 0) return bad_shape("internal: split inverse planned off the 256-column panel route");
    for (int j = 0; j < nt; ++j) {
        StepArgs sa;
        sa.S = S; sa.L = L; sa.X = X; sa.ld = ld; sa.j = j; sa.nt = nt;
        sa.info = h->d_info; sa.blk = blk_id; sa.dbg = h->dbg_stamps;
        sa.pS = (int64_t)bsp * bsp; sa.pL = stride_pL(h); sa.pX = stride_pX(h); sa.blk_per_problem = (int)h->N;
        const int m = nt - j - 1;
        const int cend = std::min(nt, (j / pw + 1) * pw);
        sa.cend = cend;
        int utiles = 0;
        for (int c = j + 1; c < cend; ++c) utiles += nt - c;
        const double rem = 64.0 * m, nb = (double)h->B;
        const double f_tile = 64.0 * 64.0 * 64.0 / 3.0 * nb, f_panel = rem * 64.0 * 64.0 * nb;
        const double f_upd = 2.0 * 64.0 * 64.0 * 64.0 * utiles * nb;
        if (fused_in_panel && !h->no_lookahead && !overlap && j % pw == 0 && cend - j >= 2 && persist_fits(h, nt, j, cend, 0)) {
            const int npc = cend - j;
            double fl = 64.0 * 64.0 * 64.0 / 3.0 * npc;
            for (int jj = j; jj + 1 < cend; ++jj) {
                int ut = 0;
                for (int c = jj + 1; c < cend; ++c) ut += nt - c;
                fl += 64.0 * (nt - jj - 1) * 64.0 * 64.0 + 2.0 * 64.0 * 64.0 * 64.0 * ut;
            }
            fl += 64.0 * (nt - cend) * 64.0 * 64.0;
            GCHK(launch_persist(h, S, L, X, nt, j, cend, 0, blk_id, fl));
            j = cend - 1;
            sa.j = j;
        } else if (fused || m == 0) {
            const bool xrows = fused && !h->doubling_x && !overlap && j >= 2;
            const int ntile_wg = 1 + m * (m + 1) / 2;
            sa.xrow = xrows ? j - 1 : -1; sa.xrow_first = ntile_wg;
            const int nx_wg = xrows ? 4 * (j - 1) : 0;
            const double f_x = xrows ? 2.0 * 64.0 * 64.0 * 64.0 * (0.5 * (double)(j - 1) * j + 0.625 * (j - 1)) : 0.0;
            ProfScope ps(h, 1, f_tile + f_panel + f_upd + f_x);
            hipLaunchKernelGGL(potrf_step<false>, dim3(ntile_wg + nx_wg, (unsigned)h->B), dim3(256),
                               m == 0 ? POTRF_TILE_LDS : POTRF_STEP_LDS, h->stream, sa);
            sa.xrow = -1;
        } else if (fused_in_panel && utiles > 0) {
            ProfScope ps(h, 1, f_tile + f_panel + f_upd);
            hipLaunchKernelGGL(potrf_step<false>, dim3(1 + utiles, 1), dim3(256), POTRF_STEP_LDS, h->stream, sa);
        } else {
            {
                ProfScope ps(h, 1, f_tile);
                hipLaunchKernelGGL(potrf_step<false>, dim3(1, (unsigned)h->B), dim3(256), POTRF_TILE_LDS, h->stream, sa);
// ... 174 lines not shown
        if (!h->keep_l) {
            hipLaunchKernelGGL(logdet_blocks, dim3(1, nb), dim3(256), 0, h->stream, L, bstride, ld, (int)h->bs,
                               h->d_logdet + i, stride_pL(h), h->N);
            HIPCHK(hipGetLastError());
        }
    }
    return GMRF_OK;
}

static gmrf_status ensure_full_inverse(gmrf_handle* h) {
    if (h->xsplit <= 0) return GMRF_OK;
    const int bsp = (int)h->bsp, p = h->xsplit, q = bsp - p;
    const int64_t ld = bsp, bstride = (int64_t)bsp * bsp, pX = stride_pX(h), pW = bstride;
    for (int64_t i = 0; i < h->N; ++i) {
        double* X = h->d_Linv + i * bstride;
        double* T = h->d_T + (int64_t)p * ld;
        GCHK(gemm(h, false, true, q, p, p, TRI_B_LOWER, 0, 1.0, X + (int64_t)p * ld, ld, X, ld, 0.0, T, ld, pX, pX, pW));
        GCHK(gemm(h, false, true, q, p, q, TRI_A_LOWER, 0, -1.0, X + (int64_t)p * ld + p, ld, T, ld, 0.0, X + (int64_t)p * ld, ld, pX, pW, pX));
    }
    h->xsplit = 0;
    return GMRF_OK;
}

static std::mutex g_capture_mu;

static gmrf_status factor_fwd_ok(gmrf_handle* h, bool* ok) {
    *ok = false;
    if (!h->frhs || h->no_factor_fwd || h->B <= 1 || tw_on(h) || h->tw_blk >= 0 || h->fork_graph || h->rmax <= 0) return GMRF_OK;
    const int bsp = (int)h->bsp, nt = bsp / 64;
    if (potrf_route(h) != ROUTE_PANELS256 || bsp % 256 != 0) return GMRF_OK;
    const int64_t elems = h->B * h->n_pad + h->B * h->bsp;
    if (!h->d_fy || h->fy_elems < elems) {
        HIPCHK(hipStreamSynchronize(h->stream));
        free_dev(h->d_ft); free_dev(h->d_fy); h->d_ft = h->d_fy = nullptr; h->fy_elems = 0; h->fy_for = nullptr;
        HIPCHK(hipMalloc(&h->d_fy, sizeof(double) * (size_t)(h->B * h->n_pad)));
        HIPCHK(hipMalloc(&h->d_ft, sizeof(double) * (size_t)(h->B * h->bsp)));
        h->fy_elems = elems;
    }
    const int64_t ld = bsp, bstride = (int64_t)bsp * bsp, pX = stride_pX(h), pL = stride_pL(h), pC = stride_pC(h);
    const int cm = (int)h->cmin, rm = (int)h->rmax, W = bsp - cm;
    double* S = h->d_S; double* X = h->d_Linv; double* L = h->d_L;
    h->tail_probe = true; h->tail_refused = false;
    gmrf_status st = GMRF_OK;
    if (h->N > 1) {
        const GemmTail tg{h->d_fy + cm, h->n_pad, h->d_ft, bsp, nullptr, 0, 1.0};
        st = gemm(h, false, false, rm, rm, W, 0, 1, -1.0, h->d_C, c_ld(h), h->d_C, c_ld(h), 0.0, S, ld, pC, pC, bstride, 1, 0, 0, 0,
                  nullptr, 0, 0, 0, -1.0, h->d_kst, h->d_kst, nullptr, false, &tg);
    }
    for (int j = 0; j + 4 < nt && st == GMRF_OK; j += 4) {
        const int64_t oa = (int64_t)j * 64, oc = oa + 256;
        const int m3 = nt - j - 4;
        const GemmTail tp{h->d_ft + oa, bsp, h->d_fy + oa, h->n_pad, nullptr, 0, 0.0};
        const GemmTail tu{h->d_fy + oa, h->n_pad, h->d_ft + oc, bsp, nullptr, 0, 1.0};
        st = gemm(h, false, false, 64 * m3, 256, 256, TRI_B_UPPER, 0, 1.0, S + oc * ld + oa, ld, X + oa * ld + oa, ld, 0.0, L + oc * ld + oa, ld,
                  bstride, pX, pL, 1, 0, 0, 0, nullptr, 0, 0, 0, -1.0, nullptr, nullptr, nullptr, false, &tp);
        if (st == GMRF_OK)
            st = gemm(h, false, false, m3 * 64, m3 * 64, 256, 0, 1, -1.0, L + oc * ld + oa, ld, L + oc * ld + oa, ld, 1.0, S + oc * ld + oc, ld,
                      pL, pL, bstride, 1, 0, 0, 0, nullptr, 0, 0, 0, -1.0, nullptr, nullptr, nullptr, false, &tu);
    }
    h->tail_probe = false;
    *ok = st == GMRF_OK && !h->tail_refused;
    return GMRF_OK;
}

static gmrf_status run_factor(gmrf_handle* h, int64_t i0, int64_t i1) {
    if (h->eager || h->profiling) { h->stats.persist_route = 0; return factor_blocks_range(h, i0, i1); }
    const double* grhs = h->fwd_run ? h->frhs : nullptr;
    if (!h->factor_graph || h->factor_graph_i0 != i0 || h->factor_graph_i1 != i1 || h->factor_graph_rhs != grhs) {
        std::lock_guard<std::mutex> capture_lock(g_capture_mu);
        if (h->factor_graph) { (void)hipGraphExecDestroy(h->factor_graph); h->factor_graph = nullptr; }
        hipGraph_t graph = nullptr;
        HIPCHK(hipStreamBeginCapture(h->stream, hipStreamCaptureModeThreadLocal));
        h->capturing = true; h->fork_next = 0;
        h->stats.persist_route = 0;
        gmrf_status s = factor_blocks_range(h, i0, i1);
        h->capturing = false;
        h->factor_graph_route = h->stats.persist_route;
        hipError_t e = hipStreamEndCapture(h->stream, &graph);
        if (s != GMRF_OK) { if (graph) (void)hipGraphDestroy(graph); return s; }
        HIPCHK(e);
        HIPCHK(hipGraphInstantiate(&h->factor_graph, graph, nullptr, nullptr, 0));
        (void)hipGraphDestroy(graph);
        h->factor_graph_i0 = i0; h->factor_graph_i1 = i1; h->factor_graph_rhs = grhs;
    }
    h->xsplit = planned_xsplit(h);
    h->stats.persist_route = h->factor_graph_route;
    if (h->factor_graph_route) h->persist_launched = true;
    HIPCHK(hipGraphLaunch(h->factor_graph, h->stream));
    return GMRF_OK;
}

static gmrf_status persist_check_range(gmrf_handle* h, int64_t i0, int64_t i1, int* hinfo_out) {
    int hinfo2[2] = {0, 0};
    HIPCHK(hipMemcpyAsync(hinfo2, h->d_info, 2 * sizeof(int), hipMemcpyDeviceToHost, h->stream));
    HIPCHK(hipStreamSynchronize(h->stream));
    h->persist_launched = false;
    if (hinfo2[1] != 0) {
        persist_give_up(h);
        const int restore[4] = {h->info_checked, 0, 0, 0};
        HIPCHK(hipMemcpyAsync(h->d_info, restore, 4 * sizeof(int), hipMemcpyHostToDevice, h->stream));
        if (h->d_pflags) HIPCHK(hipMemsetAsync(h->d_pflags, 0, sizeof(unsigned) * (size_t)h->pflags_words, h->stream));
        h->stats.persist_route = 0;
        GCHK(factor_blocks_range(h, i0, i1));
        HIPCHK(hipMemcpyAsync(hinfo2, h->d_info, 2 * sizeof(int), hipMemcpyDeviceToHost, h->stream));
        HIPCHK(hipStreamSynchronize(h->stream));
        h->persist_launched = false;
    }
    h->info_checked = hinfo2[0];
    if (hinfo_out) *hinfo_out = hinfo2[0];
    return GMRF_OK;
}
// ... 225 lines not shown
    const int64_t ldc = c_ld(h), cstride = c_blk(h);
    const int cm = (int)h->cmin, rm = (int)h->rmax, wc = bsp - cm;
    const int pclass = (kp == 1) ? 3 : 2;
    const double blk_work_c = ((kp == 1) ? 8.0 * h->c_streamed : 2.0 * h->c_streamed * kp) * nprob;
    const double blk_work_t = ((kp == 1) ? 4.0 * bsp * (double)(bsp + 1) : 1.0 * bsp * (double)(bsp + 1) * kp) * nprob;
    const bool via_gemm = (kp % 64 == 0) && !h->sweep_no_gemm && (int64_t)nprob * (bsp / 64) * (kp / 64) >= 128;
    if (tail && (!via_gemm || !backward)) return bad_shape("internal: the tail row needs the backward sweep on the GEMM");
    if (dout && !tail) return bad_shape("internal: direct output needs the tail-row sweep");
    for (int64_t step = 0; step < N; ++step) {
        const int64_t i = backward ? (N - 1 - step) : step;
        double* rhs = Pin + i * bsp;
        if (step > 0) {
            const int64_t ci = backward ? i : (i - 1);
            const int64_t prev = backward ? (i + 1) : (i - 1);
            const double* Cs = h->d_C + ci * cstride;
            const double* xin = Yout + prev * bsp + (backward ? 0 : cm);
            double* out = rhs + (backward ? cm : 0);
            const int rows = backward ? wc : rm, kdim = backward ? rm : wc;
            if (via_gemm) {
                GCHK(gemm(h, false, backward, kp, rows, kdim, 0, 0, -1.0, xin, npad, Cs, ldc, 1.0, out, npad, pPanel, pCm,
                          pPanel, 1, 0, 0, 0, nullptr, 0, 0, 0, 2.0 * h->c_streamed * kp * nprob,
                          nullptr, backward ? nullptr : h->d_kst, backward ? h->d_mend : nullptr, tail));
            } else {
                s.Mat = Cs; s.ld = ldc; s.Xin = xin; s.ldx = npad; s.Bin = out; s.ldb = npad; s.Out = out; s.ldo = npad;
                s.rows = rows; s.kdim = kdim; s.sub = 1;
                s.pMat = pCm; s.pXin = pPanel; s.pBin = pPanel; s.pOut = pPanel;
                s.kst = h->d_kst; s.mend = h->d_mend;
                ProfScope ps(h, pclass, blk_work_c);
                HIPCHK(launch_sweep(h->stream, backward, false, kp, s, nprob));
            }
        }
        const double* X = h->d_Linv + i * bstride;
        double* yout = Yout + i * bsp;
        auto direct = [&](int first) { return GemmTail{nullptr, 0, nullptr, 0, nullptr, 0, 0.0, dout, i * h->bs + first, (int)h->bs - first}; };
        if (h->xsplit > 0) {
            const int p = h->xsplit, q = bsp - p;
            const double* Xbb = X + (int64_t)p * ld + p;
            const double* Lba = X + (int64_t)p * ld;
            for (int part = 0; part < 3; ++part) {
                const int which = backward ? 2 - part : part;
                if (via_gemm) {
                    constexpr int64_t z0 = 0;
                    const GemmTail da = direct(0), db = direct(p);
                    if (which == 0)
                        GCHK(gemm(h, false, backward, kp, p, p, backward ? TRI_B_LOWER : TRI_B_UPPER, 0, 1.0, rhs, npad, X, ld, 0.0, yout, npad,
                                  pPanel, pX, pPanel, 1, z0, z0, z0, nullptr, z0, z0, 0, -1.0, nullptr, nullptr, nullptr, tail,
                                  dout ? &da : nullptr));
                    else if (which == 2)
                        GCHK(gemm(h, false, backward, kp, q, q, backward ? TRI_B_LOWER : TRI_B_UPPER, 0, 1.0, rhs + p, npad, Xbb, ld, 0.0,
                                  yout + p, npad, pPanel, pX, pPanel, 1, z0, z0, z0, nullptr, z0, z0, 0, -1.0, nullptr, nullptr, nullptr, tail,
                                  dout ? &db : nullptr));
                    else if (!backward)
                        GCHK(gemm(h, false, false, kp, q, p, 0, 0, -1.0, yout, npad, Lba, ld, 1.0, rhs + p, npad, pPanel, pX, pPanel));
                    else
                        GCHK(gemm(h, false, true, kp, p, q, 0, 0, -1.0, yout + p, npad, Lba, ld, 1.0, rhs, npad, pPanel, pX, pPanel,
                                  1, z0, z0, z0, nullptr, z0, z0, 0, -1.0, nullptr, nullptr, nullptr, tail));
                } else {
                    s.ld = ld; s.ldx = npad; s.ldo = npad; s.pMat = pX; s.pXin = pPanel; s.pOut = pPanel; s.kst = nullptr; s.mend = nullptr;
                    if (which == 0) { s.Mat = X; s.Xin = rhs; s.Bin = nullptr; s.ldb = 0; s.Out = yout; s.rows = p; s.kdim = p; s.sub = 0; s.pBin = 0; }
                    else if (which == 2) { s.Mat = Xbb; s.Xin = rhs + p; s.Bin = nullptr; s.ldb = 0; s.Out = yout + p; s.rows = q; s.kdim = q; s.sub = 0; s.pBin = 0; }
                    else if (!backward) { s.Mat = Lba; s.Xin = yout; s.Bin = rhs + p; s.ldb = npad; s.Out = rhs + p; s.rows = q; s.kdim = p; s.sub = 1; s.pBin = pPanel; }
                    else { s.Mat = Lba; s.Xin = yout + p; s.Bin = rhs; s.ldb = npad; s.Out = rhs; s.rows = p; s.kdim = q; s.sub = 1; s.pBin = pPanel; }
                    const double frac = which == 0 ? (double)p * (p + 1) : (which == 2 ? (double)q * (q + 1) : 2.0 * p * q);
                    ProfScope ps(h, pclass, blk_work_t * frac / ((double)bsp * (bsp + 1)));
                    HIPCHK(launch_sweep(h->stream, backward, which != 1, kp, s, nprob));
                }
            }
        } else if (via_gemm) {
            const GemmTail da = direct(0);
            GCHK(gemm(h, false, backward, kp, bsp, bsp, backward ? TRI_B_LOWER : TRI_B_UPPER, 0, 1.0, rhs, npad, X, ld, 0.0,
                      yout, npad, pPanel, pX, pPanel, 1, 0, 0, 0, nullptr, 0, 0, 0, -1.0, nullptr, nullptr, nullptr, tail, dout ? &da : nullptr));
        } else {
            s.Mat = X; s.ld = ld; s.Xin = rhs; s.ldx = npad; s.Bin = nullptr; s.ldb = 0; s.Out = yout; s.ldo = npad;
            s.rows = bsp; s.kdim = bsp; s.sub = 0;
            s.pMat = pX; s.pXin = pPanel; s.pBin = 0; s.pOut = pPanel;
            s.kst = nullptr; s.mend = nullptr;
            ProfScope ps(h, pclass, blk_work_t);
            HIPCHK(launch_sweep(h->stream, backward, true, kp, s, nprob));
        }
    }
    return GMRF_OK;
}

constexpr int SWEEP_BACKWARD_YP = 3, SWEEP_BACKWARD_TAIL = 4;
static gmrf_status run_sweeps(gmrf_handle* h, int mode, int kp) {
    auto body = [&]() -> gmrf_status {
        if (mode == GMRF_SOLVE_FORWARD) return sweep_launches(h, false, kp, h->d_P, h->d_Y);
        if (mode == SWEEP_BACKWARD_TAIL) return sweep_launches(h, true, kp, h->d_P, h->d_Y, true, h->d_dout);
        if (mode == SWEEP_BACKWARD_YP) return sweep_launches(h, true, kp, h->d_Y, h->d_P);
        if (mode == GMRF_SOLVE_BACKWARD) return sweep_launches(h, true, kp, h->d_P, h->d_Y);
        GCHK(sweep_launches(h, false, kp, h->d_P, h->d_Y));
        return sweep_launches(h, true, kp, h->d_Y, h->d_P);
    };
    const bool persistent = mode != SWEEP_BACKWARD_TAIL && sweep_persist_ok(h, kp);
    if (persistent) {
        GCHK(sweep_persist_prepare(h, kp));
        h->sweep_persist_launched = true;
        h->stats.sweep_persist = 1;
        h->stats.sweep_persist_launches += (mode == GMRF_SOLVE_FULL) ? 2 : 1;
    }
    if (h->eager || h->profiling) return body();
    const int64_t key = ((int64_t)h->xsplit << 32) | ((int64_t)mode * 4096 + kp) |
                        (persistent ? ((int64_t)1 << 60) : 0);
    auto it = h->sweep_graphs.find(key);
    if (it == h->sweep_graphs.end()) {
        std::lock_guard<std::mutex> capture_lock(g_capture_mu);
        hipGraph_t graph = nullptr;
        hipGraphExec_t exec = nullptr;
        HIPCHK(hipStreamBeginCapture(h->stream, hipStreamCaptureModeThreadLocal));
// ... 56 lines not shown
static gmrf_status tw_sample(gmrf_handle* h, uint64_t seed, int64_t first_id, int64_t k, const double* mean, const double* z,
                             double* out, int64_t ld);
static gmrf_status tw_logdet(gmrf_handle* h, double* out);
static gmrf_status tw_get_block(gmrf_handle* h, int32_t kind, int64_t i, double* out, int64_t ld);
static gmrf_status tw_var_exact(gmrf_handle* h, double* d_out);
static gmrf_status tw_var_accumulate_dev(gmrf_handle* h, int method, int64_t first_id, int64_t k, uint64_t seed, const gmrf_csr* Q,
                                         double* d_acc);

extern "C" {

int32_t gmrf_version(void) { return 100; }
const char* gmrf_last_error(void) { return g_last_error.c_str(); }

gmrf_status gmrf_bt_create(int32_t device, void* stream, gmrf_handle** out) {
    if (!out) return bad_shape("null out pointer");
    int count = 0;
    if (hipGetDeviceCount(&count) != hipSuccess || count <= 0 || device < 0 || device >= count) {
        (void)hipGetLastError();
        g_last_error = "no HIP device visible (libgmrf_hip needs an MI355X / gfx950 GPU)";
        return GMRF_ERR_NO_DEVICE;
    }
    HIPCHK(hipSetDevice(device));
    gmrf_handle* h = new gmrf_handle();
    memset(&h->stats, 0, sizeof(h->stats));
    h->device = device;
    if (stream) { h->stream = (hipStream_t)stream; h->own_stream = false; }
    else { HIPCHK(hipStreamCreateWithFlags(&h->stream, hipStreamNonBlocking)); h->own_stream = true; }
    HIPCHK(hipMalloc(&h->d_info, 4 * sizeof(int)));
    HIPCHK(hipMemsetAsync(h->d_info, 0, 4 * sizeof(int), h->stream));
    HIPCHK(hipStreamSynchronize(h->stream));
    HIPCHK(hipEventCreate(&h->ev0));
    HIPCHK(hipEventCreate(&h->ev1));
    HIPCHK(hipFuncSetAttribute((const void*)potrf_step<false>, hipFuncAttributeMaxDynamicSharedMemorySize, (int)POTRF_STEP_LDS));
    HIPCHK(hipFuncSetAttribute((const void*)potrf_diag128, hipFuncAttributeMaxDynamicSharedMemorySize, 160 * 1024));
    HIPCHK(hipFuncSetAttribute((const void*)potrf_persist<false>, hipFuncAttributeMaxDynamicSharedMemorySize, (int)POTRF_PERSIST_LDS));
    HIPCHK(hipDeviceGetAttribute(&h->cu_count, hipDeviceAttributeMultiprocessorCount, device));
    { const char* e = getenv("GMRF_PERSIST"); if (e && atoi(e) == 0) h->no_persist = true; }
    { const char* e = getenv("GMRF_SWEEP_PERSIST"); if (e && atoi(e) == 0) h->no_sweep_persist = true; }
    HIPCHK(hipFuncSetAttribute((const void*)potrf_diag128_slim, hipFuncAttributeMaxDynamicSharedMemorySize, 160 * 1024));
    HIPCHK(gemm_init());
    HIPCHK(gemm_dma_init());
    *out = h;
    return GMRF_OK;
}

gmrf_status gmrf_bt_destroy(gmrf_handle* h) {
    if (!h) return GMRF_OK;
    (void)hipSetDevice(h->device);
    tw_free(h);
    (void)hipStreamSynchronize(h->stream);
    persist_release(h);
    destroy_graphs(h);
    free_dev(h->d_keys); free_dev(h->d_vals); free_dev(h->d_src); free_dev(h->d_nz_stage);
    free_dev(h->d_lo_rowptr); free_dev(h->d_dg_rowptr); free_dev(h->d_kst); free_dev(h->d_mend);
    free_dev(h->d_bxt_uptr); free_dev(h->d_bxt_ucols); free_dev(h->d_bxt_lidx); free_dev(h->d_bxt_gtiles);
    if (!h->external_storage) { free_dev(h->d_L); free_dev(h->d_C); free_dev(h->d_Linv); }
    else if (!h->keep_l) free_dev(h->d_L);
    free_dev(h->d_S); free_dev(h->d_B); free_dev(h->d_T); free_dev(h->d_W);
    free_dev(h->d_sweep_flags); free_dev(h->d_Tsw); free_dev(h->d_P2); free_dev(h->d_Y2); free_dev(h->d_T2);
    if (h->h_sweep_abort) { (void)hipHostFree(h->h_sweep_abort); h->h_sweep_abort = nullptr; }
    free_dev(h->d_dout); free_dev(h->d_info); free_dev(h->d_logdet); free_dev(h->d_pflags); free_dev(h->d_kbx); free_dev(h->d_V);
    free_dev(h->d_P); free_dev(h->d_Y); free_dev(h->d_Tp);
    free_dev(h->d_stage); h->mean_arena.release(); free_dev(h->d_acc);
    free_dev(h->d_ft); free_dev(h->d_fy);
    free_dev(h->d_sel_src); free_dev(h->d_sel_slot); free_dev(h->d_sig); free_dev(h->d_dv);
    for (auto e : h->ev_pool) (void)hipEventDestroy(e);
    if (h->ev0) (void)hipEventDestroy(h->ev0);
    if (h->ev1) (void)hipEventDestroy(h->ev1);
    for (auto e : h->fork_events) (void)hipEventDestroy(e);
    if (h->aux) (void)hipStreamDestroy(h->aux);
    if (h->own_stream) (void)hipStreamDestroy(h->stream);
    delete h;
    return GMRF_OK;
}

gmrf_status gmrf_bt_set_batch(gmrf_handle* h, int64_t batch) {
    if (!h || batch < 1 || batch > 4096) return bad_shape("batch must be in [1, 4096]");
    if (batch != 1) GCHK(tw_refuse(h, "gmrf_bt_set_batch (batch > 1)"));
    if (batch != h->B) {
        HIPCHK(hipSetDevice(h->device));
        HIPCHK(hipStreamSynchronize(h->stream));
        destroy_graphs(h);
        h->B = batch;
        h->sel = 0;
        h->factored = false;
        release_shape_buffers(h);
        if (h->n > 0) (void)set_shape(h, h->n, h->N);
    }
    return GMRF_OK;
}

gmrf_status gmrf_bt_select_problem(gmrf_handle* h, int64_t p) {
    if (!h || p < 0 || p >= h->B) return bad_shape("problem index out of range");
    h->sel = p;
    return GMRF_OK;
}

gmrf_status gmrf_bt_set_profiling(gmrf_handle* h, int32_t level) {
    if (!h) return bad_shape("null handle");
    h->profiling = level;
    if (h->tw)
        for (gmrf_handle* s : {h->tw->top, h->tw->bot}) if (s) GCHK(gmrf_bt_set_profiling(s, level));
    if (level > 0 && h->events.empty()) h->gemm_shapes.clear();
    for (int i = 0; i < GMRF_KERNEL_CLASSES; ++i) { h->stats.kernel_ms[i] = h->stats.kernel_work[i] = 0; h->stats.kernel_launches[i] = 0; }
    return GMRF_OK;
}

gmrf_status gmrf_bt_set_eager(gmrf_handle* h, int32_t eager) {
    if (!h) return bad_shape("null handle");
    if (((eager & 2) != 0) != h->split_step) { destroy_graphs(h); h->split_step = (eager & 2) != 0; }
    if (((eager & 4) != 0) != h->sweep_no_gemm) { destroy_graphs(h); h->sweep_no_gemm = (eager & 4) != 0; }
    if (((eager & 8) != 0) != h->dense_g1) { destroy_graphs(h); h->dense_g1 = (eager & 8) != 0; }
    if (((eager & 16) != 0) != h->fork_graph) { destroy_graphs(h); h->fork_graph = (eager & 16) != 0; }
    h->no_staircase = (eager & 32) != 0;
    if (((eager & 128) != 0) != h->doubling_x) { destroy_graphs(h); h->doubling_x = (eager & 128) != 0; }
    if (((eager & 256) != 0) != h->no_lookahead) { destroy_graphs(h); h->no_lookahead = (eager & 256) != 0; }
    if (((eager & 4096) != 0) != h->no_xsplit) { destroy_graphs(h); h->no_xsplit = (eager & 4096) != 0; }
    if (((eager & 8192) != 0) != h->no_persist) { destroy_graphs(h); h->no_persist = (eager & 8192) != 0; }
    if (((eager & 32768) != 0) != h->no_persist_panels) { destroy_graphs(h); h->no_persist_panels = (eager & 32768) != 0; }
    if (((eager & 65536) != 0) != h->no_sweep_persist) { destroy_graphs(h); h->no_sweep_persist = (eager & 65536) != 0; }
    if (((eager & 131072) != 0) != h->no_scatter_fold) { destroy_graphs(h); h->no_scatter_fold = (eager & 131072) != 0; }
    h->no_fused_posterior = (eager & 262144) != 0;
    h->no_factor_fwd = (eager & 524288) != 0;
    if (((eager & 1048576) != 0) != h->no_grouped_gemm) { destroy_graphs(h); h->no_grouped_gemm = (eager & 1048576) != 0; }
    if (eager != h->eager_bits) h->fy_for = nullptr;
    h->eager = (eager & 1) != 0;
    h->eager_bits = eager;
    if (h->tw)
        for (gmrf_handle* s : {h->tw->top, h->tw->bot})
            if (s) {
                GCHK(gmrf_bt_set_eager(s, eager));
                if (h->tw->bot) s->no_sweep_persist = true;
            }
    return GMRF_OK;
}

gmrf_status gmrf_bt_synchronize(gmrf_handle* h) {
    if (!h) return bad_shape("null handle");
    HIPCHK(hipStreamSynchronize(h->stream));
    if (tw_on(h)) HIPCHK(hipStreamSynchronize(h->tw->bot->stream));
    return GMRF_OK;
}

gmrf_status gmrf_bt_stats(gmrf_handle* h, gmrf_stats* out) {
    if (!h || !out) return bad_shape("null pointer");
    if (tw_on(h)) {
        const gmrf_stats &a = h->tw->top->stats, &b = h->tw->bot->stats;
        *out = h->stats;
        out->persist_route = a.persist_route;
        out->persist_aborts = a.persist_aborts + b.persist_aborts;
        out->persist_cus = a.persist_cus + b.persist_cus;
        out->persist_refused = a.persist_refused | b.persist_refused;
        out->factor_bytes = a.factor_bytes + b.factor_bytes;
        return GMRF_OK;
    }
    h = tw_route(h);
    *out = h->stats;
    return GMRF_OK;
}

gmrf_status gmrf_bt_factor_csc(gmrf_handle* h, int64_t n, int64_t n_blocks, const int64_t* colptr,
                               const int64_t* rowval, const double* nzval, int32_t index_base,
                               int32_t* info) {
    if (!h) return bad_shape("null handle");
    HIPCHK(hipSetDevice(h->device));
    if (info) *info = 0;
    if (h->order == GMRF_ORDER_TWISTED) {
        GCHK(tw_analyze(h, n, n_blocks, colptr, rowval, index_base));
        return tw_numeric(h, nzval, info);
    }
    GCHK(analyze_csc(h, n, n_blocks, colptr, rowval, index_base));
    return numeric_factor(h, nzval, info);
}

gmrf_status gmrf_bt_factor_begin_csc(gmrf_handle* h, int64_t n, int64_t n_blocks, const int64_t* colptr,
                                     const int64_t* rowval, const double* nzval, int32_t index_base) {
    GCHK(tw_refuse(h, "gmrf_bt_factor_begin_csc"));
// ... 3459 lines not shown
        HIPCHK(hipStreamSynchronize(h->stream));
        return GMRF_OK;
    }));
    return GMRF_OK;
}

static double tw_step_ratio() {
    static const double r = [] { const char* e = getenv("GMRF_TWIST_RATIO"); const double v = e ? atof(e) : 0.0; return v > 0.0 ? v : 1.5; }();
    return r;
}
static int64_t tw_auto_meet(int64_t N, bool top_persist, bool bot_persist) {
    if (N < 3) return N - 1;
    const double a = top_persist ? 1.0 : tw_step_ratio(), b = bot_persist ? 1.0 : tw_step_ratio();
    const int64_t m = (int64_t)std::llround((double)(N - 1) * b / (a + b));
    return std::min<int64_t>(std::max<int64_t>(m, 1), N - 2);
}

static void tw_drop_own_factor(gmrf_handle* h) {
    (void)hipStreamSynchronize(h->stream);
    persist_release(h);
    destroy_graphs(h);
    h->factored = false;
    h->xsplit = 0;
    h->l_valid = h->logdet_valid = false;
    if (h->external_storage) return;
    free_dev(h->d_L); free_dev(h->d_C); free_dev(h->d_Linv);
    free_dev(h->d_S); free_dev(h->d_B); free_dev(h->d_T); free_dev(h->d_W); free_dev(h->d_logdet); free_dev(h->d_V);
    h->d_L = h->d_C = h->d_Linv = h->d_S = h->d_B = h->d_T = h->d_W = h->d_logdet = h->d_V = nullptr;
    h->v_elems = 0;
    h->alloc_N = h->alloc_bsp = h->alloc_B = 0;
    h->stats.factor_bytes = 0;
}

static void tw_free(gmrf_handle* h) {
    TwistState* t = h->tw;
    if (!t) return;
    if (t->bot) (void)hipStreamSynchronize(t->bot->stream);
    (void)hipStreamSynchronize(h->stream);
    if (t->top) (void)gmrf_bt_destroy(t->top);
    if (t->bot) (void)gmrf_bt_destroy(t->bot);
    free_dev(t->d_mkeys); free_dev(t->d_msrc); free_dev(t->d_mvals);
    free_dev(t->d_Bm); free_dev(t->d_HJ); free_dev(t->d_W); free_dev(t->d_Smm);
    free_dev(t->d_nz); free_dev(t->d_z); free_dev(t->d_var);
    if (t->ev_fork) (void)hipEventDestroy(t->ev_fork);
    if (t->ev_join) (void)hipEventDestroy(t->ev_join);
    delete t;
    h->tw = nullptr;
}

static gmrf_status tw_new_half(gmrf_handle* h, hipStream_t st, gmrf_handle** out) {
    GCHK(gmrf_bt_create(h->device, (void*)st, out));
    GCHK(gmrf_bt_set_eager(*out, h->eager_bits));
    (*out)->profiling = h->profiling;
    return GMRF_OK;
}

static gmrf_status tw_fork(gmrf_handle* h) {
    HIPCHK(hipEventRecord(h->tw->ev_fork, h->stream));
    HIPCHK(hipStreamWaitEvent(h->tw->bot->stream, h->tw->ev_fork, 0));
    return GMRF_OK;
}
static gmrf_status tw_join(gmrf_handle* h) {
    HIPCHK(hipEventRecord(h->tw->ev_join, h->tw->bot->stream));
    HIPCHK(hipStreamWaitEvent(h->stream, h->tw->ev_join, 0));
    return GMRF_OK;
}

static gmrf_status tw_analyze(gmrf_handle* h, int64_t n, int64_t N, const int64_t* colptr, const int64_t* rowval, int32_t base) {
    if (!colptr || !rowval) return bad_shape("null CSC arrays");
    if (h->B != 1) return bad_shape("the twisted order needs batch 1");
    tw_drop_own_factor(h);
    GCHK(set_shape(h, n, N));
    h->analyzed = false;
    if (h->meet_req > N - 1) return bad_shape("twisted order: meet must lie in [0, N_blocks - 1] (or -1: automatic)");
    const int64_t bs = h->bs;
    std::vector<std::vector<HostEntry>> dg, lo;
    GCHK(split_csc(n, N, bs, colptr, rowval, base, dg, lo));
    if (!h->tw) {
        h->tw = new TwistState();
        HIPCHK(hipEventCreateWithFlags(&h->tw->ev_fork, hipEventDisableTiming));
        HIPCHK(hipEventCreateWithFlags(&h->tw->ev_join, hipEventDisableTiming));
    }
    TwistState* t = h->tw;
    if (!t->top) GCHK(tw_new_half(h, h->stream, &t->top));
    int64_t m = h->meet_req;
    if (m < 0 && N < 3) m = N - 1;
    if (m < 0 || m < N - 1) {
        if (!t->bot) { GCHK(ensure_aux(h)); GCHK(tw_new_half(h, h->aux, &t->bot)); }
        t->top->no_sweep_persist = t->bot->no_sweep_persist = true;
    }
    if (m < 0) {
        const int64_t bsp = 64 * next_pow2((bs + 63) / 64);
        for (gmrf_handle* s : {t->top, t->bot}) {
            const int64_t keep = s->bsp;
            s->bsp = bsp;
            persist_plan(s);
            s->bsp = keep;
        }
        m = tw_auto_meet(N, t->top->persist_cus > 0, t->bot->persist_cus > 0);
    }
    if (m == N - 1 && t->bot) { (void)gmrf_bt_destroy(t->bot); t->bot = nullptr; }
    if (!t->bot) t->top->no_sweep_persist = h->no_sweep_persist;
    t->m = m; t->N = N; t->n = n; t->bs = bs; t->nnz = colptr[n] - base;
    const int64_t nnz = t->nnz;
    {
        std::vector<std::vector<HostEntry>> dgt(dg.begin(), dg.begin() + m + 1), lot(lo.begin(), lo.begin() + m + 1);
// ... 440 lines not shown
    return GMRF_OK;
}

gmrf_status gmrf_test_gemm_pair(int32_t device, int32_t batch, int32_t grouped, const int64_t* desc, const double* ab,
                                const double* A0, const double* B0, double* C0, const double* A1, const double* B1, double* C1) {
    if (!desc || !ab || !A0 || !B0 || !C0 || !A1 || !B1 || !C1 || batch < 1) return bad_shape("gemm pair test: null pointer / batch");
    HIPCHK(hipSetDevice(device));
    HIPCHK(gemm_init());
    HIPCHK(gemm_dma_init());
    const double* hA[2] = {A0, A1};
    const double* hB[2] = {B0, B1};
    double* hC[2] = {C0, C1};
    double *dA[2] = {nullptr, nullptr}, *dB[2] = {nullptr, nullptr}, *dC[2] = {nullptr, nullptr};
    GemmArgs g[2];
    bool b_n[2];
    auto drop = [&]() { for (int i = 0; i < 2; ++i) { free_dev(dA[i]); free_dev(dB[i]); free_dev(dC[i]); } };
    for (int i = 0; i < 2; ++i) {
        const int64_t M = desc[6 * i], N = desc[6 * i + 1], K = desc[6 * i + 2];
        b_n[i] = desc[6 * i + 3] != 0;
        if (M <= 0 || N <= 0 || K <= 0 || M % 64 || N % 64 || K % 16) { drop(); return bad_shape("gemm pair test sizes"); }
        const size_t na = sizeof(double) * M * K * batch, nb = sizeof(double) * K * N * batch, nc = sizeof(double) * M * N * batch;
        hipError_t e = hipMalloc(&dA[i], na);
        if (e == hipSuccess) e = hipMalloc(&dB[i], nb);
        if (e == hipSuccess) e = hipMalloc(&dC[i], nc);
        if (e == hipSuccess) e = hipMemcpy(dA[i], hA[i], na, hipMemcpyHostToDevice);
        if (e == hipSuccess) e = hipMemcpy(dB[i], hB[i], nb, hipMemcpyHostToDevice);
        if (e == hipSuccess) e = hipMemcpy(dC[i], hC[i], nc, hipMemcpyHostToDevice);
        if (e != hipSuccess) { drop(); HIPCHK(e); }
        GemmArgs& a = g[i];
        a.A = dA[i]; a.B = dB[i]; a.C = dC[i]; a.lda = K; a.ldb = b_n[i] ? N : K; a.ldc = N;
        a.strideA = a.strideB = a.strideC = 0;
        a.pA = M * K; a.pB = K * N; a.pC = M * N; a.nb1 = 1;
        a.M = (int)M; a.N = (int)N; a.K = (int)K; a.tri = (int)desc[6 * i + 4]; a.lower_only = (int)desc[6 * i + 5];
        a.alpha = ab[2 * i]; a.beta = ab[2 * i + 1]; a.D = nullptr; a.ldd = 0; a.pD = 0; a.stamps = nullptr;
    }
    const int saved = gemm_big_policy(), saved_ll = gemm_ll_policy(), saved_dma = gemm_dma_policy(), saved_force = gemm_dma_force();
    gemm_big_policy() = 2; gemm_ll_policy() = 2; gemm_dma_policy() = 2; gemm_dma_force() = 1;
    hipError_t le = hipSuccess;
    bool ok = true;
    if (grouped) ok = gemm_try_dma_grouped(nullptr, b_n[0], g[0], b_n[1], g[1], batch, nullptr, nullptr, &le);
    else {
        for (int i = 0; i < 2 && ok && le == hipSuccess; ++i) ok = gemm_try_dma(nullptr, false, b_n[i], g[i], batch, nullptr, nullptr, &le);
    }
    gemm_big_policy() = saved; gemm_ll_policy() = saved_ll; gemm_dma_policy() = saved_dma; gemm_dma_force() = saved_force;
    if (!ok) { drop(); return bad_shape("gemm pair test: not a pair of LDS-DMA products"); }
    if (le == hipSuccess) le = hipDeviceSynchronize();
    for (int i = 0; i < 2 && le == hipSuccess; ++i)
        le = hipMemcpy(hC[i], dC[i], sizeof(double) * g[i].M * g[i].N * batch, hipMemcpyDeviceToHost);
    drop();
    HIPCHK(le);
    return GMRF_OK;
}

gmrf_status gmrf_test_gemm_desc(int32_t device, int32_t route, const int64_t* desc, const double* abt,
                                const double* A, int64_t nA, const double* B, int64_t nB, double* C, int64_t nC,
                                const double* D, int64_t nD, const double* tA, int64_t ntA, double* tC, int64_t ntC,
                                const double* tD, int64_t ntD, const int32_t* kb_m, int64_t n_kb_m, const int32_t* kb_n,
                                int64_t n_kb_n, const int32_t* ke_n, int64_t n_ke_n, double* samples, int64_t n_samples,
                                double* mean, int64_t n_mean, int32_t* family) {
    if (!desc || !abt || !A || !B || !C || !family) return bad_shape("gemm desc test: null pointer");
    *family = 0;
    const int64_t M = desc[0], N = desc[1], K = desc[2];
    const bool a_t = desc[3] != 0, b_n = desc[4] != 0;
    const int64_t tri = desc[5], lower_only = desc[6], batch = desc[7], nb1 = desc[8];
    const int64_t lda = desc[9], ldb = desc[10], ldc = desc[11], ldd = desc[12];
    const int64_t sA = desc[13], sB = desc[14], sC = desc[15], pA = desc[16], pB = desc[17], pC = desc[18], pD = desc[19];
    const int64_t ptA = desc[20], ptC = desc[21], ptD = desc[22], o_j0 = desc[23], o_n = desc[24], o_cols = desc[25];
    const int64_t o_ld = desc[26], o_k = desc[27];
    if (route < 0 || route > 7) return bad_shape("gemm desc test: unknown route");
    if (M <= 0 || N <= 0 || K <= 0 || M % 64 || N % 64 || K % 16 || M > 16384 || N > 16384 || K > 16384)
        return bad_shape("gemm desc test: sizes");
    if (tri < 0 || tri > 15 || (lower_only != 0 && lower_only != 1)) return bad_shape("gemm desc test: tri / lower_only");
    if (batch < 1 || nb1 < 1 || batch % nb1 || batch > 4096) return bad_shape("gemm desc test: batch is not a multiple of nb1");
    const int64_t strides[] = {sA, sB, sC, pA, pB, pC, pD, ptA, ptC, ptD};
    for (int64_t s : strides)
        if (s < 0 || s > ((int64_t)1 << 40)) return bad_shape("gemm desc test: negative stride");
    const bool tail = route == 6, own_tail = tail && tC != nullptr, dout = tail && samples != nullptr;
    if (!tail && (tA || tC || tD || samples || mean)) return bad_shape("gemm desc test: tail operands without the tail route");
    if (dout && (!mean || own_tail)) return bad_shape("gemm desc test: direct output");
    if (!dout && mean) return bad_shape("gemm desc test: mean without samples");
    if (own_tail && !tA) return bad_shape("gemm desc test: tC without tA");
    if (!own_tail && (tA || tD)) return bad_shape("gemm desc test: tA / tD without tC");
    const int64_t rows = M + ((tail && !own_tail) ? 1 : 0);
    if (lda < (a_t ? M : K) || ldb < (b_n ? N : K) || ldc < N || (D && ldd < N) || lda > ((int64_t)1 << 24) || ldb > ((int64_t)1 << 24) ||
        ldc > ((int64_t)1 << 24) || ldd > ((int64_t)1 << 24))
        return bad_shape("gemm desc test: leading dimension");
    const int64_t np = batch / nb1, zin = (nb1 - 1), zout = (np - 1);
    const int64_t needA = zin * sA + zout * pA + (a_t ? (K - 1) * lda + M : (rows - 1) * lda + K);
    const int64_t needB = zin * sB + zout * pB + (b_n ? (K - 1) * ldb + N : (N - 1) * ldb + K);
    const int64_t needC = zin * sC + zout * pC + (rows - 1) * ldc + N;
    const int64_t needD = zout * pD + (rows - 1) * ldd + N;
    if (needA > nA || needB > nB || needC > nC || (D && needD > nD)) return bad_shape("gemm desc test: operand buffer too small");
    if (own_tail && (zout * ptA + K > ntA || zout * ptC + N > ntC || (tD && zout * ptD + N > ntD)))
        return bad_shape("gemm desc test: tail buffer too small");
    if ((kb_m && n_kb_m < M / 64) || (kb_n && n_kb_n < N / 64) || (ke_n && n_ke_n < N / 64)) return bad_shape("gemm desc test: K bounds too short");
    const int32_t* kbs[3] = {kb_m, kb_n, ke_n};
    const int64_t nkb[3] = {M / 64, N / 64, N / 64};
    for (int a = 0; a < 3; ++a)
        for (int64_t i = 0; kbs[a] && i < nkb[a]; ++i)
            if (kbs[a][i] < 0 || kbs[a][i] > K || kbs[a][i] % 64) return bad_shape("gemm desc test: K bound value");
    if (dout) {
        if (o_k < 0 || o_k > M || o_cols < 0 || o_cols > N || o_j0 < 0 || o_ld < 0 || o_n < 0 || o_ld > ((int64_t)1 << 24) || o_n > ((int64_t)1 << 30))
            return bad_shape("gemm desc test: direct-out fields");
        if (o_cols > 0 && o_k > 0 && (zout * o_k + o_k - 1) * o_ld + o_j0 + o_cols > n_samples) return bad_shape("gemm desc test: samples too small");
        if (o_cols > 0 && zout * o_n + o_j0 + o_cols > n_mean) return bad_shape("gemm desc test: mean too small");
    }
    HIPCHK(hipSetDevice(device));
    HIPCHK(gemm_init());
    HIPCHK(gemm_dma_init());

    std::vector<void*> owned;
    auto drop = [&]() { for (void* p : owned) free_dev(p); owned.clear(); };
    hipError_t e = hipSuccess;
    auto up = [&](const void* host, int64_t count, size_t elem) -> void* {
        if (!host || e != hipSuccess) return nullptr;
        void* d = nullptr;
        e = hipMalloc(&d, std::max<size_t>((size_t)count * elem, 16));
        if (e != hipSuccess) return nullptr;
        owned.push_back(d);
        if (count > 0) e = hipMemcpy(d, host, (size_t)count * elem, hipMemcpyHostToDevice);
        return d;
    };
    GemmArgs g;
    g.A = (const double*)up(A, nA, 8); g.B = (const double*)up(B, nB, 8); g.C = (double*)up(C, nC, 8);
    g.D = (const double*)up(D, nD, 8);
    g.tA = (const double*)up(tA, ntA, 8); g.tC = (double*)up(tC, ntC, 8); g.tD = (const double*)up(tD, ntD, 8);
    g.kb_m = (const int*)up(kb_m, n_kb_m, 4); g.kb_n = (const int*)up(kb_n, n_kb_n, 4); g.ke_n = (const int*)up(ke_n, n_ke_n, 4);
    double* d_samples = (double*)up(samples, n_samples, 8);
    double* d_mean = (double*)up(mean, n_mean, 8);
    GemmDirectOut* d_out = nullptr;
    if (dout && e == hipSuccess) {
        e = hipMalloc(&d_out, sizeof(GemmDirectOut));
        if (e == hipSuccess) {
            owned.push_back(d_out);
            hipLaunchKernelGGL(set_direct_out, dim3(1), dim3(1), 0, nullptr, d_out, d_samples, d_mean, o_ld, o_k);
            e = hipGetLastError();
        }
    }
    if (e != hipSuccess) { drop(); HIPCHK(e); }
    g.lda = lda; g.ldb = ldb; g.ldc = ldc; g.ldd = D ? ldd : 0;
    g.strideA = sA; g.strideB = sB; g.strideC = sC; g.pA = pA; g.pB = pB; g.pC = pC; g.pD = D ? pD : 0;
    g.nb1 = (int)nb1; g.M = (int)M; g.N = (int)N; g.K = (int)K; g.tri = (int)tri; g.lower_only = (int)lower_only;
    g.alpha = abt[0]; g.beta = abt[1]; g.tbeta = abt[2];
    g.ptA = ptA; g.ptC = ptC; g.ptD = ptD;
    g.stamps = nullptr;
    g.dout = d_out; g.o_j0 = o_j0; g.o_n = o_n; g.o_cols = (int)o_cols;

    const int saved_big = gemm_big_policy(), saved_ll = gemm_ll_policy(), saved_dma = gemm_dma_policy(), saved_force = gemm_dma_force();
    auto restore = [&]() { gemm_big_policy() = saved_big; gemm_ll_policy() = saved_ll; gemm_dma_policy() = saved_dma; gemm_dma_force() = saved_force; };
    static const int big_p[] = {2, 1, 2, 2, 2, 2, 2, 0};
    static const int ll_p[] = {2, 2, 0, 2, 2, 2, 2, 0};
    static const int dma_p[] = {0, 0, 0, 2, 2, 2, 1, 2};
    static const int force_p[] = {0, 0, 0, 1, 2, 3, 0, 0};
    gemm_big_policy() = big_p[route]; gemm_ll_policy() = ll_p[route]; gemm_dma_policy() = dma_p[route]; gemm_dma_force() = force_p[route];
    const int nz = (int)batch;
    int fam;
    hipError_t le = hipSuccess;
    if (tail) {
        fam = gemm_try_dma_tail(nullptr, a_t, b_n, g, nz, nullptr, nullptr, &le) ? (dout ? 9 : 8) : 0;
    } else {
        if (gemm_uses_big(a_t, g, nz)) fam = 3;
        else if (!gemm_uses_ll(g, nz) && gemm_dma_shape(a_t, g, nz) != 0) fam = 4 + gemm_dma_shape(a_t, g, nz);
        else if (gemm_uses_ll(g, nz)) fam = 4;
        else {
            const bool tri_grid = lower_only && M == N;
            const int64_t sx = N / GEMM_BN, sy = M / GEMM_BM;
            fam = (K % 32 == 0 ? 2 : 1) + ((tri_grid ? sx * (sx + 1) / 2 : sx * sy) * batch > 768 ? 256 : 0);
        }
        static const int want[] = {0, 3, 4, 5, 6, 7};
        if (route == 0 ? (fam & 255) > 2 : (route < 6 && fam != want[route])) fam = 0;
        if (fam) le = launch_gemm(nullptr, a_t, b_n, g, nz);
    }
    restore();
    if (!fam) { drop(); return bad_shape("gemm desc test: the descriptor does not qualify for the route"); }
    if (le == hipSuccess) le = hipDeviceSynchronize();
    if (le == hipSuccess) le = hipMemcpy(C, g.C, sizeof(double) * nC, hipMemcpyDeviceToHost);
    if (le == hipSuccess && own_tail) le = hipMemcpy(tC, g.tC, sizeof(double) * ntC, hipMemcpyDeviceToHost);
    if (le == hipSuccess && dout && n_samples > 0) le = hipMemcpy(samples, d_samples, sizeof(double) * n_samples, hipMemcpyDeviceToHost);
    if (le == hipSuccess && dout && n_mean > 0) le = hipMemcpy(mean, d_mean, sizeof(double) * n_mean, hipMemcpyDeviceToHost);
    drop();
    HIPCHK(le);
    *family = fam;
    return GMRF_OK;
}

gmrf_status gmrf_test_gemm_shapes(gmrf_handle* h, double* rows, int64_t cap_rows, int64_t* n_rows) {
    if (!h || !n_rows) return bad_shape("null argument");
    HIPCHK(hipStreamSynchronize(h->stream));
    prof_collect(h);
    *n_rows = (int64_t)h->gemm_shapes.size();
    for (int64_t i = 0; rows && i < std::min<int64_t>(cap_rows, *n_rows); ++i) {
        const auto& g = h->gemm_shapes[(size_t)i];
        for (int c = 0; c < 8; ++c) rows[i * 11 + c] = (double)g.key[c];
        rows[i * 11 + 8] = g.launches; rows[i * 11 + 9] = g.ms; rows[i * 11 + 10] = g.work;
    }
    return GMRF_OK;
}

struct ClockProbe { int device; hipStream_t st; unsigned long long* d; int n; };
gmrf_status gmrf_test_clock_probe_start(int32_t device, int32_t n, int32_t sleeps, void** probe) {
    if (!probe || n < 2 || n > 100000 || sleeps < 1 || sleeps > 64) return bad_shape("clock probe: 2 <= n <= 100000, 1 <= sleeps <= 64");
    HIPCHK(hipSetDevice(device));
    ClockProbe* p = new ClockProbe{device, nullptr, nullptr, n};
    auto drop = [&](hipError_t e) {
        if (p->d) (void)hipFree(p->d);
        if (p->st) (void)hipStreamDestroy(p->st);
        delete p;
        g_last_error = std::string("clock probe: ") + hipGetErrorString(e);
        return GMRF_ERR_HIP;
    };
    hipError_t e = hipStreamCreateWithFlags(&p->st, hipStreamNonBlocking);
    if (e == hipSuccess) e = hipMalloc(&p->d, sizeof(unsigned long long) * 2 * 8 * (size_t)n);
    if (e == hipSuccess) e = hipMemsetAsync(p->d, 0, sizeof(unsigned long long) * 2 * 8 * (size_t)n, p->st);
    if (e != hipSuccess) return drop(e);
    hipLaunchKernelGGL(clock_probe_kernel, dim3(8), dim3(64), 0, p->st, p->d, n, sleeps);
    if ((e = hipGetLastError()) != hipSuccess) return drop(e);
    *probe = p;
    return GMRF_OK;
}
gmrf_status gmrf_test_clock_probe_finish(void* probe, double* ghz, double* t_ms) {
    ClockProbe* p = static_cast<ClockProbe*>(probe);
    if (!p || !ghz) return bad_shape("null pointer");
    std::vector<unsigned long long> h((size_t)2 * 8 * p->n);
    hipError_t e = hipSetDevice(p->device);
    if (e == hipSuccess) e = hipStreamSynchronize(p->st);
    if (e == hipSuccess) e = hipMemcpy(h.data(), p->d, h.size() * sizeof(unsigned long long), hipMemcpyDeviceToHost);
    if (e != hipSuccess) {
        (void)hipFree(p->d); (void)hipStreamDestroy(p->st);
        delete p;
        g_last_error = std::string("clock probe: ") + hipGetErrorString(e);
        return GMRF_ERR_HIP;
    }
    for (int i = 0; i + 1 < p->n; ++i) {
        double v[8];
        for (int b = 0; b < 8; ++b) {
// ... 229 lines not shown
            if (hipStreamSynchronize(h->stream) != hipSuccess) s = GMRF_ERR_HIP;
            if (s == GMRF_OK && hi[1] != 0) persist_give_up(h);
            *info = hi[0];
            route[0] = potrf_route(h); route[1] = h->stats.persist_route; route[2] = h->xsplit; route[3] = h->persist_aborts;
        }
    }
    gmrf_bt_destroy(h);
    return s;
}

gmrf_status gmrf_test_mfma_f64_rate(int32_t device, double* tflops) {
    HIPCHK(hipSetDevice(device));
    double* d;
    HIPCHK(hipMalloc(&d, 64));
    hipEvent_t a, b;
    HIPCHK(hipEventCreate(&a)); HIPCHK(hipEventCreate(&b));
    const int iters = 20000, blocks = 256 * 2;
    hipLaunchKernelGGL(mfma_f64_rate_kernel, dim3(blocks), dim3(256), 0, nullptr, d, 100);
    HIPCHK(hipDeviceSynchronize());
    HIPCHK(hipEventRecord(a, nullptr));
    hipLaunchKernelGGL(mfma_f64_rate_kernel, dim3(blocks), dim3(256), 0, nullptr, d, iters);
    HIPCHK(hipEventRecord(b, nullptr));
    HIPCHK(hipEventSynchronize(b));
    float ms = 0.f;
    HIPCHK(hipEventElapsedTime(&ms, a, b));
    const double flops = (double)blocks * 4  * iters * 4.0 * 2048.0;
    *tflops = flops / (ms * 1e-3) / 1e12;
    hipFree(d); hipEventDestroy(a); hipEventDestroy(b);
    return GMRF_OK;
}


gmrf_status gmrf_test_symbolic_csc(int64_t n, int64_t n_blocks, const int64_t* colptr, const int64_t* rowval, int32_t index_base,
                                   int64_t* out8) {
    if (!colptr || !rowval || !out8) return bad_shape("null pointer");
    if (n <= 0 || n_blocks <= 0 || n % n_blocks != 0) return bad_shape("n must be a positive multiple of N_blocks");
    const int64_t bs = n / n_blocks, bsp = 64 * next_pow2((bs + 63) / 64);
    std::vector<std::vector<HostEntry>> dg, lo;
    GCHK(split_csc(n, n_blocks, bs, colptr, rowval, index_base, dg, lo));
    SymbolicPlan sp;
    build_symbolic(n_blocks, bsp, dg, lo, false, sp);
    uint64_t sum = 1469598103934665603ull;
    auto mix = [&sum](uint64_t v) { sum = (sum ^ v) * 1099511628211ull; };
    for (uint64_t k : sp.keys) mix(k);
    for (int64_t v : sp.src) mix((uint64_t)v);
    for (int v : sp.rowptr) mix((uint64_t)(uint32_t)v);
    for (int v : sp.uptr) mix((uint64_t)(uint32_t)v);
    for (int v : sp.gtiles) mix((uint64_t)(uint32_t)v);
    for (int v : sp.ucols) mix((uint64_t)(uint32_t)v);
    for (uint16_t v : sp.lidx) mix(v);
    for (int64_t v : sp.first) mix((uint64_t)v);
    out8[0] = sp.cmin; out8[1] = sp.rmax; out8[2] = (int64_t)sp.keys.size(); out8[3] = sp.max_row; out8[4] = sp.sparse_b;
    out8[5] = sp.bxt_ok; out8[6] = sp.ecap; out8[7] = (int64_t)(sum >> 1);
    return GMRF_OK;
}

gmrf_status gmrf_test_microbench(int32_t device, double* out, int32_t n) {
    if (!out || n < 16) return bad_shape("need 16 outputs");
    HIPCHK(hipSetDevice(device));
    unsigned long long* d_t; double* d_s; int* d_i;
    HIPCHK(hipMalloc(&d_t, 64)); HIPCHK(hipMalloc(&d_s, 64)); HIPCHK(hipMalloc(&d_i, 64));
    hipEvent_t a, b;
    HIPCHK(hipEventCreate(&a)); HIPCHK(hipEventCreate(&b));
    unsigned long long ht[2];
    float ms = 0.f;
    auto timed = [&](auto launch, double flops, int idx) -> gmrf_status {
        launch(); HIPCHK(hipDeviceSynchronize());
        HIPCHK(hipEventRecord(a, nullptr)); launch(); HIPCHK(hipEventRecord(b, nullptr));
        HIPCHK(hipEventSynchronize(b)); HIPCHK(hipEventElapsedTime(&ms, a, b));
        HIPCHK(hipMemcpy(ht, d_t, 16, hipMemcpyDeviceToHost));
        out[idx] = flops / (ms * 1e-3) / 1e12;
        out[idx + 1] = (double)ht[0] / (double)ht[1] * 0.1;
        return GMRF_OK;
    };
    const int it = 20000;
    GCHK(timed([&] { hipLaunchKernelGGL((mb_mfma_f64<4>), dim3(256), dim3(256), 0, nullptr, d_t, d_s, it); },
               256.0 * 4 * it * 4 * 2048.0, 0));
    GCHK(timed([&] { hipLaunchKernelGGL((mb_mfma_f64<4>), dim3(512), dim3(256), 0, nullptr, d_t, d_s, it); },
               512.0 * 4 * it * 4 * 2048.0, 2));
    GCHK(timed([&] { hipLaunchKernelGGL((mb_mfma_f64<1>), dim3(256), dim3(256), 0, nullptr, d_t, d_s, it); },
               256.0 * 4 * it * 1 * 2048.0, 4));
    GCHK(timed([&] { hipLaunchKernelGGL(mb_valu_f64, dim3(512), dim3(256), 0, nullptr, d_t, d_s, it * 4); },
               512.0 * 256 * (it * 4.0) * 8 * 2.0, 6));
    GCHK(timed([&] { hipLaunchKernelGGL((mb_mfma_f64<4>), dim3(1), dim3(64), 0, nullptr, d_t, d_s, it); },
               1.0 * it * 4 * 2048.0, 8));
    out[10] = (double)ht[0] / (it * 4.0);
    hipLaunchKernelGGL(mb_null, dim3(1), dim3(64), 0, nullptr, d_i);
    HIPCHK(hipDeviceSynchronize());
    HIPCHK(hipEventRecord(a, nullptr));
    for (int i = 0; i < 2000; ++i) hipLaunchKernelGGL(mb_null, dim3(1), dim3(64), 0, nullptr, d_i);
    HIPCHK(hipEventRecord(b, nullptr));
    HIPCHK(hipEventSynchronize(b)); HIPCHK(hipEventElapsedTime(&ms, a, b));
    out[11] = ms * 1e3 / 2000.0;
    {
        hipStream_t st; HIPCHK(hipStreamCreateWithFlags(&st, hipStreamNonBlocking));
        hipGraph_t g; hipGraphExec_t ge;
        HIPCHK(hipStreamBeginCapture(st, hipStreamCaptureModeThreadLocal));
        for (int i = 0; i < 2000; ++i) hipLaunchKernelGGL(mb_null, dim3(1), dim3(64), 0, st, d_i);
        HIPCHK(hipStreamEndCapture(st, &g));
        HIPCHK(hipGraphInstantiate(&ge, g, nullptr, nullptr, 0));
        HIPCHK(hipGraphLaunch(ge, st)); HIPCHK(hipStreamSynchronize(st));
        HIPCHK(hipEventRecord(a, st)); HIPCHK(hipGraphLaunch(ge, st)); HIPCHK(hipEventRecord(b, st));
        HIPCHK(hipEventSynchronize(b)); HIPCHK(hipEventElapsedTime(&ms, a, b));
        out[12] = ms * 1e3 / 2000.0;
        (void)hipGraphExecDestroy(ge); (void)hipGraphDestroy(g); (void)hipStreamDestroy(st);
    }
// ... 41 lines not shown
```

### include/gmrf_hip.h

```cpp
#ifndef GMRF_HIP_H
#define GMRF_HIP_H

#include <stdint.h>

#ifdef __cplusplus
extern "C" {
#endif

typedef int32_t gmrf_status;

enum {
    GMRF_OK = 0,
    GMRF_ERR_NOT_SPD = -1,
    GMRF_ERR_BAD_SHAPE = -2,
    GMRF_ERR_BAND = -3,
    GMRF_ERR_HIP = -4,
    GMRF_ERR_NO_FACTOR = -5,
    GMRF_ERR_NO_DEVICE = -6,
    GMRF_ERR_ALLOC = -7,
    GMRF_ERR_RCCL = -8
};

enum { GMRF_SOLVE_FULL = 0, GMRF_SOLVE_FORWARD = 1, GMRF_SOLVE_BACKWARD = 2 };
enum { GMRF_VAR_EXACT = 0, GMRF_VAR_RBMC = 1, GMRF_VAR_MC = 2 };
// ... 233 lines not shown
gmrf_status gmrf_bic_destroy(gmrf_bic* g);
gmrf_status gmrf_bic_run(gmrf_bic* g, const double* ic, double* x_ic_out, double* q_values_out, double* qx_out, double* bulk_out,
                         int32_t* info);

gmrf_status gmrf_field_errors_batch(int32_t device, void* stream, int64_t batch, int64_t n, int64_t first, const double* pred,
                                    const double* soln, double* out);

typedef struct gmrf_elliptic_p1 gmrf_elliptic_p1;
gmrf_status gmrf_elliptic_p1_create(int32_t device, void* stream, int64_t nx, int64_t ny, gmrf_elliptic_p1** out);
gmrf_status gmrf_elliptic_p1_destroy(gmrf_elliptic_p1* e);
gmrf_status gmrf_elliptic_p1_pattern(const gmrf_elliptic_p1* e, int64_t* nnz_out, int64_t* rowptr, int64_t* colidx,
                                     int32_t index_base);
gmrf_status gmrf_elliptic_p1_qpoints(const gmrf_elliptic_p1* e, double* xy);
gmrf_status gmrf_elliptic_p1_tangent(gmrf_elliptic_p1* e, const double* w, double* vals_out, double* f_out);
gmrf_status gmrf_elliptic_p1_tangent_batch(gmrf_elliptic_p1* e, int64_t batch, const double* w, double* vals_out, double* f_out);
gmrf_status gmrf_elliptic_p1_load(gmrf_elliptic_p1* e, int64_t batch, const double* src_q, double* b_out);
gmrf_status gmrf_elliptic_p2_create(int32_t device, void* stream, int64_t nx, int64_t ny, gmrf_elliptic_p1** out);
gmrf_status gmrf_gn_create_elliptic(gmrf_handle* h, gmrf_assembler* as, gmrf_elliptic_p1* e, gmrf_gn** out);

gmrf_status gmrf_darcy_p1_assemble_batch(gmrf_darcy_p1* d, int64_t batch, const double* coeff_tables, int64_t ng, double beta,
                                         double* vals_out, double* f_out);
typedef struct gmrf_dc gmrf_dc;
gmrf_status gmrf_dc_create(gmrf_handle* h, gmrf_assembler* as, gmrf_darcy_p1* d, gmrf_dc** out);
gmrf_status gmrf_dc_destroy(gmrf_dc* g);
gmrf_status gmrf_dc_run(gmrf_dc* g, const double* coeff_tables, int64_t ng, double beta, const double* q_nzval, int64_t q_stride,
                        const double* q_mu, double q_eps, int64_t k_samples, uint64_t sample_seed, int32_t var_method, int64_t k_var,
                        uint64_t var_seed, double* mean_out, double* samples_out, double* std_out, double* std_norm_out,
                        int32_t* info);

typedef struct gmrf_swe_p1 gmrf_swe_p1;
gmrf_status gmrf_shallow_water_p1_create(int32_t device, void* stream, int64_t nx, int64_t ny, gmrf_swe_p1** out);
gmrf_status gmrf_shallow_water_p1_destroy(gmrf_swe_p1* w);
gmrf_status gmrf_shallow_water_p1_pattern(const gmrf_swe_p1* w, int32_t which, int64_t* nnz_out, int64_t* rowptr, int64_t* colidx,
                                          int32_t index_base);
gmrf_status gmrf_shallow_water_p1_qpoints(const gmrf_swe_p1* w, double* xy);
gmrf_status gmrf_shallow_water_p1_assemble(gmrf_swe_p1* w, const double* H_q, double k, double f, double g, const uint8_t* prescribed,
                                           double* K_vals, double* M_lumped, double* S_vals);
gmrf_status gmrf_shallow_water_p1_operators(gmrf_swe_p1* w, const double* K_vals, const double* M_lumped, const double* S_vals,
                                            const uint8_t* prescribed, double kappa_matern, double tau, double dt, double* G_vals,
                                            double* J_vals, double* M_tilde, double* beta);

gmrf_status gmrf_test_gemm(int32_t device, int64_t M, int64_t N, int64_t K, int32_t transA,
                           int32_t transB, int32_t tri_flags, int32_t lower_only,
                           double alpha, const double* A, int64_t lda, const double* B,
                           int64_t ldb, double beta, double* C, int64_t ldc);
gmrf_status gmrf_test_gemm_pair(int32_t device, int32_t batch, int32_t grouped, const int64_t* desc, const double* ab,
                                const double* A0, const double* B0, double* C0, const double* A1, const double* B1, double* C1);
gmrf_status gmrf_test_gemm_desc(int32_t device, int32_t route, const int64_t* desc, const double* abt,
                                const double* A, int64_t nA, const double* B, int64_t nB, double* C, int64_t nC,
                                const double* D, int64_t nD, const double* tA, int64_t ntA, double* tC, int64_t ntC,
                                const double* tD, int64_t ntD, const int32_t* kb_m, int64_t n_kb_m, const int32_t* kb_n,
                                int64_t n_kb_n, const int32_t* ke_n, int64_t n_ke_n, double* samples, int64_t n_samples,
                                double* mean, int64_t n_mean, int32_t* family);
gmrf_status gmrf_test_gemm_rate(int32_t device, int64_t M, int64_t N, int64_t K, int32_t transB,
                                int32_t tri_flags, int32_t lower_only, int32_t batch,
                                int32_t big, int32_t reps, double* ms_per_launch);
gmrf_status gmrf_test_gemm_shapes(gmrf_handle* h, double* rows, int64_t cap_rows, int64_t* n_rows);
gmrf_status gmrf_test_potrf_tile(int32_t device, double* tile64 ,
                                 double* inv64, int32_t* info);
gmrf_status gmrf_test_tile_timing(double* out, int32_t n);
gmrf_status gmrf_test_potrf_block(int32_t device, int64_t bs, double* S ,
                                  double* Linv, int32_t* info);
gmrf_status gmrf_test_potrf_route(int32_t device, int64_t bs, int32_t batch, int32_t eager_bits, int64_t cmin, int32_t keep_l,
                                  double* S, double* L, double* Linv, int32_t* info, int32_t* route);
gmrf_status gmrf_test_persist_stamps(double* out, int32_t n);
gmrf_status gmrf_test_persist_aborts(gmrf_handle* h, int32_t* n);
gmrf_status gmrf_test_factor_fwd(gmrf_handle* h, int32_t* state, double* y_out);
gmrf_status gmrf_test_gn_route(gmrf_gn* g, int32_t* iterations, int32_t* fwd_iterations);
gmrf_status gmrf_test_dc_route(gmrf_dc* g, int32_t* fwd_in_factor);
gmrf_status gmrf_test_bic_route(gmrf_bic* g, int32_t* fwd_in_factor);
gmrf_status gmrf_test_var_groups(gmrf_handle* h, int32_t* group_size, int32_t* groups);
gmrf_status gmrf_test_persist_budget(int32_t cus, int32_t n, const int32_t* demands, int32_t* granted);
gmrf_status gmrf_test_mfma_f64_rate(int32_t device, double* tflops);
gmrf_status gmrf_test_clock_probe_start(int32_t device, int32_t n, int32_t sleeps, void** probe);
gmrf_status gmrf_test_clock_probe_finish(void* probe, double* ghz, double* t_ms);
gmrf_status gmrf_test_hbm_rate(int32_t device, int64_t bytes, double* gbps);
gmrf_status gmrf_test_microbench(int32_t device, double* out, int32_t n);
gmrf_status gmrf_test_symbolic_csc(int64_t n, int64_t n_blocks, const int64_t* colptr, const int64_t* rowval,
                                   int32_t index_base, int64_t* out8);

#ifdef __cplusplus
}
#endif
#endif
```

Before: 54940 solves/s.

## Skip structurally zero K ranges in panel GEMMs using a per-row-tile sparsity envelope

Builds a per-block, per-64-row-tile envelope (first nonzero column and fill extent) during symbolic analysis. It derives K-begin and K-end bounds per panel, uploads them to the device, and passes them to the DMA GEMM through a new ke_m bound, so tiles skip zero K ranges in the factor's panel and update GEMMs. The aim is to cut wasted f64 MFMA work on the banded Darcy blocks. In exchange it adds host symbolic cost, device memory, fallback logic for the big/LL routes, and more complex kernel bound computation that relies on the fill envelope being correct.

```diff
diff --git a/diffeqgmrfs.jl_amd/_cabi.py b/diffeqgmrfs.jl_amd/_cabi.py
--- a/diffeqgmrfs.jl_amd/_cabi.py
+++ b/diffeqgmrfs.jl_amd/_cabi.py
@@ -41,8 +41,8 @@
     "gmrf_burgers_prior_create", "gmrf_burgers_line_prior_create", "gmrf_burgers_prior_destroy", "gmrf_burgers_prior_pattern", "gmrf_burgers_prior_values_batch",
     "gmrf_bic_create", "gmrf_bic_destroy", "gmrf_bic_run", "gmrf_field_errors_batch",
     "gmrf_bt_logdet_batch", "gmrf_assemble_quadform_batch", "gmrf_gn_posterior",
-    "gmrf_test_gemm", "gmrf_test_gemm_desc", "gmrf_test_gemm_pair", "gmrf_test_gemm_rate", "gmrf_test_gemm_shapes", "gmrf_test_potrf_tile", "gmrf_test_potrf_block", "gmrf_test_potrf_route", "gmrf_test_tile_timing", "gmrf_test_persist_stamps", "gmrf_test_persist_aborts", "gmrf_test_factor_fwd", "gmrf_test_gn_route", "gmrf_test_dc_route", "gmrf_test_bic_route", "gmrf_test_var_groups", "gmrf_test_persist_budget", "gmrf_test_clock_probe_start", "gmrf_test_clock_probe_finish",
-    "gmrf_test_mfma_f64_rate", "gmrf_test_hbm_rate", "gmrf_test_microbench", "gmrf_test_symbolic_csc",
+    "gmrf_test_gemm", "gmrf_test_gemm_desc", "gmrf_test_gemm_env", "gmrf_test_envelope", "gmrf_test_gemm_pair", "gmrf_test_gemm_rate", "gmrf_test_gemm_shapes", "gmrf_test_potrf_tile", "gmrf_test_potrf_block", "gmrf_test_potrf_route", "gmrf_test_tile_timing", "gmrf_test_persist_stamps", "gmrf_test_persist_aborts", "gmrf_test_factor_fwd", "gmrf_test_gn_route", "gmrf_test_dc_route", "gmrf_test_bic_route", "gmrf_test_var_groups", "gmrf_test_persist_budget", "gmrf_test_clock_probe_start", "gmrf_test_clock_probe_finish",
+    "gmrf_test_mfma_f64_rate", "gmrf_test_hbm_rate", "gmrf_test_microbench", "gmrf_test_symbolic_csc", "gmrf_test_envelope_csc",
 ]
 
 
@@ -214,6 +214,8 @@
         "gmrf_test_gemm": [i32, i64, i64, i64, i32, i32, i32, i32, dbl, vp, i64, vp, i64, dbl, vp, i64],
         "gmrf_test_gemm_shapes": [vp, P(dbl), i64, P(i64)],
         "gmrf_test_gemm_desc": [i32, i32, vp, vp] + [vp, i64] * 12 + [P(i32)],
+        "gmrf_test_gemm_env": [i32, i32, vp, vp] + [vp, i64] * 11 + [i32, P(i32)],
+        "gmrf_test_envelope": [vp, vp, vp, i64, P(i64), P(i32)],
         "gmrf_test_gemm_pair": [i32, i32, i32, vp, vp, vp, vp, vp, vp, vp, vp],
         "gmrf_test_gemm_rate": [i32, i64, i64, i64, i32, i32, i32, i32, i32, i32, P(dbl)],
         "gmrf_test_potrf_tile": [i32, vp, vp, P(i32)],
@@ -234,6 +236,7 @@
         "gmrf_test_hbm_rate": [i32, i64, P(dbl)],
         "gmrf_test_microbench": [i32, vp, i32],
         "gmrf_test_symbolic_csc": [i64, i64, vp, vp, i32, vp],
+        "gmrf_test_envelope_csc": [i64, i64, vp, vp, i32, vp, vp, vp, i64, P(i64)],
     }
     for name, args in sigs.items():
         fn = getattr(lib, name)
diff --git a/diffeqgmrfs.jl_amd/api.py b/diffeqgmrfs.jl_amd/api.py
--- a/diffeqgmrfs.jl_amd/api.py
+++ b/diffeqgmrfs.jl_amd/api.py
@@ -1223,6 +1223,15 @@
         return [dict({k: int(r[i]) for i, k in enumerate(names)}, launches=int(r[8]), ms=float(r[9]), flops=float(r[10]))
                 for r in buf[: int(n.value)]]
 
+    def envelope(self):
+        n, state = C.c_int64(0), C.c_int32(0)
+        _cabi.check(self._lib.gmrf_test_envelope(self._h, None, None, 0, C.byref(n), C.byref(state)))
+        if n.value == 0:
+            return None, None, int(state.value)
+        lo, hi = np.zeros(n.value, np.int32), np.zeros(n.value, np.int32)
+        _cabi.check(self._lib.gmrf_test_envelope(self._h, _cabi.ptr(lo), _cabi.ptr(hi), n.value, C.byref(n), C.byref(state)))
+        return lo, hi, int(state.value)
+
     def set_profiling(self, level: int):
         _cabi.check(self._lib.gmrf_bt_set_profiling(self._h, level))
 
diff --git a/diffeqgmrfs.jl_amd/csrc/gemm_f64.hpp b/diffeqgmrfs.jl_amd/csrc/gemm_f64.hpp
--- a/diffeqgmrfs.jl_amd/csrc/gemm_f64.hpp
+++ b/diffeqgmrfs.jl_amd/csrc/gemm_f64.hpp
@@ -45,6 +45,7 @@
     const int* kb_m = nullptr;
     const int* kb_n = nullptr;
     const int* ke_n = nullptr;
+    const int* ke_m = nullptr;
     const double* tA = nullptr;
     double* tC = nullptr;
     const double* tD = nullptr;
diff --git a/diffeqgmrfs.jl_amd/csrc/gemm_f64_dma.hpp b/diffeqgmrfs.jl_amd/csrc/gemm_f64_dma.hpp
--- a/diffeqgmrfs.jl_amd/csrc/gemm_f64_dma.hpp
+++ b/diffeqgmrfs.jl_amd/csrc/gemm_f64_dma.hpp
@@ -80,9 +80,10 @@
     if (g.tri & TRI_A_UPPER) kb = max(kb, m0);
     if (g.tri & TRI_B_LOWER) kb = max(kb, n0);
     if (g.tri & TRI_B_UPPER) ke = min(ke, n0 + BN);
-    if (g.kb_m) kb = max(kb, g.kb_m[bm * (BM / 64)]);
-    if (g.kb_n) kb = max(kb, g.kb_n[bn * (BN / 64)]);
+    if (g.kb_m) kb = max(kb, BM > 64 ? min(g.kb_m[bm * (BM / 64)], g.kb_m[bm * (BM / 64) + BM / 64 - 1]) : g.kb_m[bm]);
+    if (g.kb_n) kb = max(kb, BN > 64 ? min(g.kb_n[bn * (BN / 64)], g.kb_n[bn * (BN / 64) + BN / 64 - 1]) : g.kb_n[bn]);
     if (g.ke_n) ke = min(ke, g.ke_n[bn * (BN / 64) + BN / 64 - 1]);
+    if (g.ke_m) ke = min(ke, BM > 64 ? max(g.ke_m[bm * (BM / 64)], g.ke_m[bm * (BM / 64) + BM / 64 - 1]) : g.ke_m[bm]);
     const int nkt = (ke > kb) ? (ke - kb) / BK : 0;
 
     extern __shared__ __attribute__((aligned(16))) double gsm[];
@@ -382,7 +383,7 @@
     if (force == 3 && g.N % 128 == 0 && !g.lower_only) return 3;
     if (force) return 1;
     if (policy == 1) return 1;
-    const bool plain = !g.lower_only && !g.tri && !g.kb_m && !g.kb_n && !g.ke_n;
+    const bool plain = !g.lower_only && !g.tri && !g.kb_m && !g.kb_n && !g.ke_n && !g.ke_m;
     const int64_t t64 = (int64_t)(g.M / 64) * (g.N / 64) * batch;
     if (policy >= 3 || (plain && t64 >= 2048)) {
         if (g.M % 128 == 0) return 2;
@@ -414,7 +415,7 @@
     }
     if (!b_n || g.lower_only) return false;
     if (g.dout && g.nb1 != 1) return false;
-    if (g.dout && (g.beta != 0.0 || g.kb_m || g.kb_n || g.ke_n || (g.tri & (TRI_A_LOWER | TRI_A_UPPER)))) return false;
+    if (g.dout && (g.beta != 0.0 || g.kb_m || g.kb_n || g.ke_n || g.ke_m || (g.tri & (TRI_A_LOWER | TRI_A_UPPER)))) return false;
     return (int64_t)(g.M + 1) * g.ldc * 8 < ((int64_t)1 << 32) && (!g.D || (int64_t)(g.M + 1) * g.ldd * 8 < ((int64_t)1 << 32));
 }
 inline bool gemm_try_dma_tail(hipStream_t st, bool a_t, bool b_n, const GemmArgs& g, int batch, hipEvent_t ev_start, hipEvent_t ev_stop,
diff --git a/diffeqgmrfs.jl_amd/csrc/gmrf_hip.hip b/diffeqgmrfs.jl_amd/csrc/gmrf_hip.hip
--- a/diffeqgmrfs.jl_amd/csrc/gmrf_hip.hip
+++ b/diffeqgmrfs.jl_amd/csrc/gmrf_hip.hip
@@ -157,6 +157,13 @@
     double c_streamed = 0.0;
     double g2_tile_k = 0.0;
     bool c_dirty = false;
+    std::vector<int> env_lo, env_hi, env_host, env_ken;
+    std::vector<unsigned char> env_has, env_ken_has;
+    int* d_env = nullptr;
+    int* d_env_ken = nullptr;
+    bool env_ok = false;
+    bool no_env = false;
+    bool tw_half = false;
     int* d_lo_rowptr = nullptr;
     int* d_dg_rowptr = nullptr;
     int* d_bxt_uptr = nullptr; int* d_bxt_ucols = nullptr; uint16_t* d_bxt_lidx = nullptr; int* d_bxt_gtiles = nullptr;
@@ -376,7 +383,7 @@
                         int batch = 1, int64_t sA = 0, int64_t sB = 0, int64_t sC = 0, const double* D = nullptr,
                         int64_t ldd = 0, int64_t pD = 0, int pclass = 0, double pwork = -1.0,
                         const int* kb_m = nullptr, const int* kb_n = nullptr, const int* ke_n = nullptr, bool tail = false,
-                        const GemmTail* gt = nullptr) {
+                        const GemmTail* gt = nullptr, const int* ke_m = nullptr, bool hints = false) {
     GemmArgs g;
     if (gt) {
         if (gt->C) { g.tA = gt->A; g.ptA = gt->pA; g.tC = gt->C; g.ptC = gt->pC; g.tD = gt->D; g.ptD = gt->pD; g.tbeta = gt->beta; }
@@ -391,6 +398,11 @@
     g.pA = pA; g.pB = pB; g.pC = pC; g.nb1 = batch;
     g.M = M; g.N = N; g.K = K; g.tri = tri; g.lower_only = lower_only;
     g.alpha = alpha; g.beta = beta; g.stamps = nullptr;
+    g.ke_m = ke_m;
+    if ((ke_m || hints) && (gemm_uses_big(a_t, g, batch * (int)h->B) || gemm_uses_ll(g, batch * (int)h->B) || !gemm_uses_dma(a_t, g, batch * (int)h->B))) {
+        g.ke_m = ke_m = nullptr;
+        if (hints) { g.kb_m = kb_m = nullptr; g.kb_n = kb_n = nullptr; g.ke_n = ke_n = nullptr; pwork = -1.0; }
+    }
     double flops = gemm_flops(M, N, K, tri, lower_only, batch * (double)h->B);
     if (tail) {
         if (!gemm_tail_ok(a_t, b_n, g, batch * (int)h->B)) {
@@ -406,7 +418,7 @@
             EvPair p;
             p.kind = pclass; p.work = pwork >= 0.0 ? pwork : flops;
             p.a = ev_get(h); p.b = ev_get(h);
-            const int64_t key[8] = {pclass, M + 1, N, K, tri, lower_only, batch * h->B, (kb_m || kb_n || ke_n) ? 1 : 0};
+            const int64_t key[8] = {pclass, M + 1, N, K, tri, lower_only, batch * h->B, (kb_m || kb_n || ke_n || ke_m) ? 1 : 0};
             p.shape = gemm_shape_row(h, key);
             (void)gemm_try_dma_tail(h->gemm_stream ? h->gemm_stream : h->stream, a_t, b_n, g, batch * (int)h->B, p.a, p.b, &e);
             HIPCHK(e);
@@ -427,7 +439,7 @@
         EvPair p;
         p.kind = pclass; p.work = pwork >= 0.0 ? pwork : flops;
         p.a = ev_get(h); p.b = ev_get(h);
-        const int64_t key[8] = {pclass, M, N, K, tri, lower_only, batch * h->B, (kb_m || kb_n || ke_n) ? 1 : 0};
+        const int64_t key[8] = {pclass, M, N, K, tri, lower_only, batch * h->B, (kb_m || kb_n || ke_n || ke_m) ? 1 : 0};
         p.shape = gemm_shape_row(h, key);
         HIPCHK(launch_gemm(h->gemm_stream ? h->gemm_stream : h->stream, a_t, b_n, g, batch * (int)h->B, p.a, p.b));
         h->events.push_back(p);
@@ -499,6 +511,7 @@
     destroy_graphs(h);
     h->cmin = cmin; h->rmax = rmax;
     h->layout_gen++;
+    h->env_ok = false;
     h->kst.assign((size_t)ntile, 0);
     int64_t run = bsp - 64;
     for (int t = nrt - 1; t >= 0; --t) {
@@ -667,7 +680,35 @@
     std::vector<uint16_t> lidx;
     int ecap = 0, nrt = 0;
     std::vector<int> drowptr;
+    std::vector<int> env_lo, env_hi;
 };
+
+static void build_envelope(int64_t N, int64_t bsp, const std::vector<std::vector<HostEntry>>& dg, int64_t rmax, SymbolicPlan& sp) {
+    const int nt = (int)(bsp / 64);
+    sp.env_lo.assign((size_t)(N * nt), 0);
+    sp.env_hi.assign((size_t)(N * nt), (int)bsp);
+    std::vector<int64_t> lo((size_t)nt), hi((size_t)nt);
+    for (int64_t i = 0; i < N; ++i) {
+        const int64_t rm = i > 0 ? rmax : 0;
+        for (int t = 0; t < nt; ++t) lo[(size_t)t] = 64 * (int64_t)t;
+        for (auto& e : dg[(size_t)i]) {
+            const int64_t r = (int64_t)(e.key >> 32), c = (int64_t)(e.key & 0xffffffffu);
+            lo[(size_t)(r / 64)] = std::min(lo[(size_t)(r / 64)], c);
+        }
+        for (int t = 0; t < nt; ++t) { lo[(size_t)t] = lo[(size_t)t] / 64 * 64; hi[(size_t)t] = 0; }
+        for (auto& e : dg[(size_t)i]) {
+            const int64_t r = (int64_t)(e.key >> 32), c = (int64_t)(e.key & 0xffffffffu);
+            const int64_t p0 = lo[(size_t)(r / 64)] / 256 * 256;
+            if (c >= p0 && c < p0 + 256) hi[(size_t)(r / 64)] = std::max(hi[(size_t)(r / 64)], c + 1);
+        }
+        for (int t = 0; t < nt; ++t) {
+            if (64 * (int64_t)t < rm) continue;
+            const int64_t p0 = lo[(size_t)t] / 256 * 256;
+            sp.env_lo[(size_t)(i * nt + t)] = (int)lo[(size_t)t];
+            sp.env_hi[(size_t)(i * nt + t)] = (int)((64 * (int64_t)t < p0 + 256) ? std::min(p0 + 256, bsp) : (hi[(size_t)t] + 63) / 64 * 64);
+        }
+    }
+}
 
 static void build_symbolic(int64_t N, int64_t bsp, const std::vector<std::vector<HostEntry>>& dg,
                            const std::vector<std::vector<HostEntry>>& lo, bool no_staircase, SymbolicPlan& sp, bool group_tiles = true) {
@@ -703,6 +744,7 @@
         if (no_staircase) std::fill(first.begin(), first.end(), cmin);
         sp.cmin = cmin; sp.rmax = rmax; sp.first = first;
     }
+    build_envelope(N, bsp, dg, sp.rmax, sp);
     sp.rowptr.assign((size_t)(N * (bsp + 1)), 0);
     int64_t max_row = 0;
     for (int64_t i = 1; i < N; ++i) {
@@ -787,6 +829,67 @@
     }
 }
 
+struct EnvHost { std::vector<int> host, ken; std::vector<unsigned char> has, ken_has; bool any = false; };
+static void derive_envelope(int64_t N, int64_t bsp, const SymbolicPlan& sp, EnvHost& o) {
+    const int nt = (int)(bsp / 64), np = nt / 4;
+    auto& env_host = o.host; auto& env_has = o.has; auto& env_ken = o.ken; auto& env_ken_has = o.ken_has;
+    env_host.assign((size_t)(N * np * 4 * nt), 0);
+    env_has.assign((size_t)(N * np), 0);
+    env_ken.assign((size_t)(N * 4), 0);
+    env_ken_has.assign((size_t)N, 0);
+    bool any = false;
+    for (int64_t i = 0; i < N; ++i)
+        for (int p = 0; p < np; ++p) {
+            const int oa = 256 * p, m3 = nt - 4 * p - 4;
+            int* a = env_host.data() + (size_t)((i * np + p) * 4) * nt;
+            unsigned char has = 0;
+            for (int bm = 0; bm < m3; ++bm) {
+                const int t = 4 * p + 4 + bm, lo = sp.env_lo[(size_t)(i * nt + t)], hi = sp.env_hi[(size_t)(i * nt + t)];
+                const int kb = std::min(std::max(lo - oa, 0), 256);
+                const int ke = (lo >= oa && lo < oa + 256) ? std::min(std::max(hi - oa, kb), 256) : 256;
+                a[bm] = kb; a[nt + bm] = ke;
+                const bool last = bm == m3 - 1;
+                a[2 * nt + bm] = last ? 0 : kb; a[3 * nt + bm] = last ? 256 : ke;
+                if (kb > 0) has |= 1;
+                if (kb > 0 || ke < 256) has |= 2;
+                if (!last && (kb > 0 || ke < 256)) has |= 4;
+            }
+            for (int bm = m3; bm < nt; ++bm) { a[bm] = a[2 * nt + bm] = 0; a[nt + bm] = a[3 * nt + bm] = 256; }
+            env_has[(size_t)(i * np + p)] = has;
+            any = any || has;
+            if (p == 0 && m3 > 0) {
+                for (int bn = 0; bn < 4; ++bn) {
+                    int end = 0;
+                    for (int bm = 0; bm < m3; ++bm) if (a[bm] <= 64 * bn) end = 64 * (bm + 1);
+                    env_ken[(size_t)(i * 4 + bn)] = end;
+                    if (end < 64 * m3) env_ken_has[(size_t)i] = 1;
+                }
+            }
+        }
+    o.any = any;
+}
+static gmrf_status upload_envelope(gmrf_handle* h, const SymbolicPlan& sp) {
+    h->env_ok = false;
+    const int64_t N = h->N, bsp = h->bsp;
+    const int nt = (int)(bsp / 64);
+    if (N <= 0 || bsp % 256 != 0 || (int64_t)sp.env_lo.size() != N * nt) return GMRF_OK;
+    h->env_lo = sp.env_lo; h->env_hi = sp.env_hi;
+    EnvHost eh;
+    derive_envelope(N, bsp, sp, eh);
+    h->env_host.swap(eh.host); h->env_has.swap(eh.has); h->env_ken.swap(eh.ken); h->env_ken_has.swap(eh.ken_has);
+    const bool any = eh.any;
+    free_dev(h->d_env); free_dev(h->d_env_ken);
+    h->d_env = nullptr; h->d_env_ken = nullptr;
+    if (!any) return GMRF_OK;
+    HIPCHK(hipMalloc(&h->d_env, h->env_host.size() * sizeof(int)));
+    HIPCHK(hipMalloc(&h->d_env_ken, h->env_ken.size() * sizeof(int)));
+    HIPCHK(hipMemcpyAsync(h->d_env, h->env_host.data(), h->env_host.size() * sizeof(int), hipMemcpyHostToDevice, h->stream));
+    HIPCHK(hipMemcpyAsync(h->d_env_ken, h->env_ken.data(), h->env_ken.size() * sizeof(int), hipMemcpyHostToDevice, h->stream));
+    HIPCHK(hipStreamSynchronize(h->stream));
+    h->env_ok = true;
+    return GMRF_OK;
+}
+
 static gmrf_status upload_entries(gmrf_handle* h, const std::vector<std::vector<HostEntry>>& dg,
                                   const std::vector<std::vector<HostEntry>>& lo, int64_t nnz_in) {
     const int64_t N = h->N;
@@ -795,6 +898,7 @@
     h->diag_first = sp.diag_first; h->diag_count = sp.diag_count; h->low_first = sp.low_first; h->low_count = sp.low_count;
     const auto& keys = sp.keys; const auto& src = sp.src;
     GCHK(set_layout(h, sp.cmin, sp.rmax, sp.first));
+    GCHK(upload_envelope(h, sp));
     free_dev(h->d_keys); free_dev(h->d_vals); free_dev(h->d_src); free_dev(h->d_nz_stage);
     h->d_keys = nullptr; h->d_vals = nullptr; h->d_src = nullptr; h->d_nz_stage = nullptr;
     h->n_entries = (int64_t)keys.size();
@@ -1076,6 +1180,38 @@
                        h->stream, pa);
     HIPCHK(hipGetLastError());
     return GMRF_OK;
+}
+
+struct EnvPanel { const int* pp_kb; const int* pp_ke; const int* upd_kb; double units_pp, units_upd; };
+static double env_units_pp(const int* host, int nt, int m3, int a) {
+    double u = 0.0;
+    for (int bm = 0; bm < m3; ++bm)
+        for (int bn = 0; bn < 4; ++bn) u += std::max(0, std::min(64 * (bn + 1), host[(a + 1) * nt + bm]) - host[a * nt + bm]) / 64;
+    return u;
+}
+static double env_units_upd(const int* host, int m3) {
+    double u = 0.0;
+    for (int bm = 0; bm < m3; ++bm)
+        for (int bn = 0; bn <= bm; ++bn) u += (256 - std::max(host[bm], host[bn])) / 64;
+    return u;
+}
+static EnvPanel env_panel(const gmrf_handle* h, int64_t i, int p, bool tail_rides) {
+    const int nt = (int)(h->bsp / 64), np = nt / 4, m3 = nt - 4 * p - 4;
+    EnvPanel e{nullptr, nullptr, nullptr, 10.0 * m3, 4.0 * (m3 * (m3 + 1) / 2)};
+    if (!h->env_ok || h->no_env || h->B <= 1 || h->tw || h->tw_half || h->tw_blk >= 0 || i < 0 || i >= h->N || p < 0 || p >= np || m3 <= 0) return e;
+    const size_t at = (size_t)((i * np + p) * 4) * nt;
+    const unsigned char has = h->env_has[(size_t)(i * np + p)];
+    const int* host = h->env_host.data() + at;
+    if (has & (tail_rides ? 4 : 2)) {
+        const int a = tail_rides ? 2 : 0;
+        e.pp_kb = h->d_env + at + (size_t)a * nt; e.pp_ke = h->d_env + at + (size_t)(a + 1) * nt;
+        e.units_pp = env_units_pp(host, nt, m3, a);
+    }
+    if (has & 1) {
+        e.upd_kb = h->d_env + at;
+        e.units_upd = env_units_upd(host, m3);
+    }
+    return e;
 }
 
 static gmrf_status potrf_block(gmrf_handle* h, double* S, double* L, double* X, double* T, int blk_id, double* fy = nullptr) {
@@ -1185,12 +1321,13 @@
             const bool in_slot = (j == 0 && h->xsplit == 256 && !h->keep_l);
             double* Lb = in_slot ? X + oc * ld + oa : L + oc * ld + oa;
             const int64_t pLb = in_slot ? sa.pX : sa.pL;
+            const EnvPanel ev = env_panel(h, blk_id - 1, j / 4, fy != nullptr);
             GCHK(gemm(h, false, false, 64 * m3, 256, 256, TRI_B_UPPER, 0, 1.0, S + oc * ld + oa, ld, X + oa * ld + oa, ld, 0.0, Lb, ld,
-                      sa.pS, sa.pX, pLb, 1, 0, 0, 0, nullptr, 0, 0, 0, 2.0 * t3 * 10.0 * m3 * nb, nullptr, nullptr, nullptr, false,
-                      fy ? &tp : nullptr));
+                      sa.pS, sa.pX, pLb, 1, 0, 0, 0, nullptr, 0, 0, 0, 2.0 * t3 * ev.units_pp * nb, ev.pp_kb, nullptr, nullptr, false,
+                      fy ? &tp : nullptr, ev.pp_ke, true));
             GCHK(gemm(h, false, false, m3 * 64, m3 * 64, 256, 0, 1, -1.0, Lb, ld, Lb, ld, 1.0, S + oc * ld + oc, ld, pLb, pLb, sa.pS,
-                      1, 0, 0, 0, nullptr, 0, 0, 0, 2.0 * t3 * 4.0 * (m3 * (m3 + 1) / 2) * nb, nullptr, nullptr, nullptr, false,
-                      fy ? &tu : nullptr));
+                      1, 0, 0, 0, nullptr, 0, 0, 0, 2.0 * t3 * ev.units_upd * nb, ev.upd_kb, ev.upd_kb, nullptr, false,
+                      fy ? &tu : nullptr, nullptr, true));
         }
         const int p = h->xsplit;
         GCHK(doubling_levels(h, L, X, T, 256, bsp / 2, -1, p));
@@ -1471,11 +1608,12 @@
         const int m3 = nt - j - 4;
         const GemmTail tp{h->d_ft + oa, bsp, h->d_fy + oa, h->n_pad, nullptr, 0, 0.0};
         const GemmTail tu{h->d_fy + oa, h->n_pad, h->d_ft + oc, bsp, nullptr, 0, 1.0};
+        const EnvPanel ev = env_panel(h, std::min<int64_t>(1, h->N - 1), j / 4, true);
         st = gemm(h, false, false, 64 * m3, 256, 256, TRI_B_UPPER, 0, 1.0, S + oc * ld + oa, ld, X + oa * ld + oa, ld, 0.0, L + oc * ld + oa, ld,
-                  bstride, pX, pL, 1, 0, 0, 0, nullptr, 0, 0, 0, -1.0, nullptr, nullptr, nullptr, false, &tp);
+                  bstride, pX, pL, 1, 0, 0, 0, nullptr, 0, 0, 0, -1.0, ev.pp_kb, nullptr, nullptr, false, &tp, ev.pp_ke, true);
         if (st == GMRF_OK)
             st = gemm(h, false, false, m3 * 64, m3 * 64, 256, 0, 1, -1.0, L + oc * ld + oa, ld, L + oc * ld + oa, ld, 1.0, S + oc * ld + oc, ld,
-                      pL, pL, bstride, 1, 0, 0, 0, nullptr, 0, 0, 0, -1.0, nullptr, nullptr, nullptr, false, &tu);
+                      pL, pL, bstride, 1, 0, 0, 0, nullptr, 0, 0, 0, -1.0, ev.upd_kb, ev.upd_kb, nullptr, false, &tu, nullptr, true);
     }
     h->tail_probe = false;
     *ok = st == GMRF_OK && !h->tail_refused;
@@ -1807,9 +1945,14 @@
                                   dout ? &db : nullptr));
                     else if (!backward)
                         GCHK(gemm(h, false, false, kp, q, p, 0, 0, -1.0, yout, npad, Lba, ld, 1.0, rhs + p, npad, pPanel, pX, pPanel));
-                    else
+                    else {
+                        const bool env = p == 256 && h->env_ok && !h->no_env && !h->tw && !h->tw_half && h->tw_blk < 0 && h->env_ken_has[(size_t)i];
+                        double units = 0.0;
+                        for (int bn = 0; env && bn < 4; ++bn) units += h->env_ken[(size_t)(i * 4 + bn)] / 64;
                         GCHK(gemm(h, false, true, kp, p, q, 0, 0, -1.0, yout + p, npad, Lba, ld, 1.0, rhs, npad, pPanel, pX, pPanel,
-                                  1, z0, z0, z0, nullptr, z0, z0, 0, -1.0, nullptr, nullptr, nullptr, tail));
+                                  1, z0, z0, z0, nullptr, z0, z0, 0, env ? 2.0 * kp * 64.0 * 64.0 * units * nprob : -1.0, nullptr, nullptr,
+                                  env ? h->d_env_ken + i * 4 : nullptr, tail, nullptr, nullptr, env));
+                    }
                 } else {
                     s.ld = ld; s.ldx = npad; s.ldo = npad; s.pMat = pX; s.pXin = pPanel; s.pOut = pPanel; s.kst = nullptr; s.mend = nullptr;
                     if (which == 0) { s.Mat = X; s.Xin = rhs; s.Bin = nullptr; s.ldb = 0; s.Out = yout; s.rows = p; s.kdim = p; s.sub = 0; s.pBin = 0; }
@@ -1972,7 +2115,7 @@
     persist_release(h);
     destroy_graphs(h);
     free_dev(h->d_keys); free_dev(h->d_vals); free_dev(h->d_src); free_dev(h->d_nz_stage);
-    free_dev(h->d_lo_rowptr); free_dev(h->d_dg_rowptr); free_dev(h->d_kst); free_dev(h->d_mend);
+    free_dev(h->d_lo_rowptr); free_dev(h->d_dg_rowptr); free_dev(h->d_kst); free_dev(h->d_mend); free_dev(h->d_env); free_dev(h->d_env_ken);
     free_dev(h->d_bxt_uptr); free_dev(h->d_bxt_ucols); free_dev(h->d_bxt_lidx); free_dev(h->d_bxt_gtiles);
     if (!h->external_storage) { free_dev(h->d_L); free_dev(h->d_C); free_dev(h->d_Linv); }
     else if (!h->keep_l) free_dev(h->d_L);
@@ -2043,6 +2186,7 @@
     h->no_fused_posterior = (eager & 262144) != 0;
     h->no_factor_fwd = (eager & 524288) != 0;
     if (((eager & 1048576) != 0) != h->no_grouped_gemm) { destroy_graphs(h); h->no_grouped_gemm = (eager & 1048576) != 0; }
+    if (((eager & 2097152) != 0) != h->no_env) { destroy_graphs(h); h->no_env = (eager & 2097152) != 0; }
     if (eager != h->eager_bits) h->fy_for = nullptr;
     h->eager = (eager & 1) != 0;
     h->eager_bits = eager;
@@ -5608,6 +5752,7 @@
     GCHK(gmrf_bt_create(h->device, (void*)st, out));
     GCHK(gmrf_bt_set_eager(*out, h->eager_bits));
     (*out)->profiling = h->profiling;
+    (*out)->tw_half = true;
     return GMRF_OK;
 }
 
@@ -6154,12 +6299,12 @@
     return GMRF_OK;
 }
 
-gmrf_status gmrf_test_gemm_desc(int32_t device, int32_t route, const int64_t* desc, const double* abt,
-                                const double* A, int64_t nA, const double* B, int64_t nB, double* C, int64_t nC,
-                                const double* D, int64_t nD, const double* tA, int64_t ntA, double* tC, int64_t ntC,
-                                const double* tD, int64_t ntD, const int32_t* kb_m, int64_t n_kb_m, const int32_t* kb_n,
-                                int64_t n_kb_n, const int32_t* ke_n, int64_t n_ke_n, double* samples, int64_t n_samples,
-                                double* mean, int64_t n_mean, int32_t* family) {
+static gmrf_status gemm_desc_run(int32_t device, int32_t route, const int64_t* desc, const double* abt,
+                                 const double* A, int64_t nA, const double* B, int64_t nB, double* C, int64_t nC,
+                                 const double* D, int64_t nD, const double* tA, int64_t ntA, double* tC, int64_t ntC,
+                                 const double* tD, int64_t ntD, const int32_t* kb_m, int64_t n_kb_m, const int32_t* kb_n,
+                                 int64_t n_kb_n, const int32_t* ke_n, int64_t n_ke_n, double* samples, int64_t n_samples,
+                                 double* mean, int64_t n_mean, int32_t* family, const int32_t* ke_m, int64_t n_ke_m, int32_t grouped) {
     if (!desc || !abt || !A || !B || !C || !family) return bad_shape("gemm desc test: null pointer");
     *family = 0;
     const int64_t M = desc[0], N = desc[1], K = desc[2];
@@ -6195,10 +6340,12 @@
     if (needA > nA || needB > nB || needC > nC || (D && needD > nD)) return bad_shape("gemm desc test: operand buffer too small");
     if (own_tail && (zout * ptA + K > ntA || zout * ptC + N > ntC || (tD && zout * ptD + N > ntD)))
         return bad_shape("gemm desc test: tail buffer too small");
-    if ((kb_m && n_kb_m < M / 64) || (kb_n && n_kb_n < N / 64) || (ke_n && n_ke_n < N / 64)) return bad_shape("gemm desc test: K bounds too short");
-    const int32_t* kbs[3] = {kb_m, kb_n, ke_n};
-    const int64_t nkb[3] = {M / 64, N / 64, N / 64};
-    for (int a = 0; a < 3; ++a)
+    if ((kb_m && n_kb_m < M / 64) || (kb_n && n_kb_n < N / 64) || (ke_n && n_ke_n < N / 64) || (ke_m && n_ke_m < M / 64))
+        return bad_shape("gemm desc test: K bounds too short");
+    if (grouped < 0 || grouped > 2 || (grouped && route != 3)) return bad_shape("gemm desc test: grouped launches are of the 64 x 64 LDS-DMA kernel");
+    const int32_t* kbs[4] = {kb_m, kb_n, ke_n, ke_m};
+    const int64_t nkb[4] = {M / 64, N / 64, N / 64, M / 64};
+    for (int a = 0; a < 4; ++a)
         for (int64_t i = 0; kbs[a] && i < nkb[a]; ++i)
             if (kbs[a][i] < 0 || kbs[a][i] > K || kbs[a][i] % 64) return bad_shape("gemm desc test: K bound value");
     if (dout) {
@@ -6228,6 +6375,7 @@
     g.D = (const double*)up(D, nD, 8);
     g.tA = (const double*)up(tA, ntA, 8); g.tC = (double*)up(tC, ntC, 8); g.tD = (const double*)up(tD, ntD, 8);
     g.kb_m = (const int*)up(kb_m, n_kb_m, 4); g.kb_n = (const int*)up(kb_n, n_kb_n, 4); g.ke_n = (const int*)up(ke_n, n_ke_n, 4);
+    g.ke_m = (const int*)up(ke_m, n_ke_m, 4);
     double* d_samples = (double*)up(samples, n_samples, 8);
     double* d_mean = (double*)up(mean, n_mean, 8);
     GemmDirectOut* d_out = nullptr;
@@ -6271,7 +6419,12 @@
         }
         static const int want[] = {0, 3, 4, 5, 6, 7};
         if (route == 0 ? (fam & 255) > 2 : (route < 6 && fam != want[route])) fam = 0;
-        if (fam) le = launch_gemm(nullptr, a_t, b_n, g, nz);
+        if (fam && grouped) {
+            GemmArgs g2 = g;
+            g2.C = (double*)up(C, nC, 8);
+            le = e;
+            if (le == hipSuccess && !gemm_try_dma_grouped(nullptr, b_n, grouped == 1 ? g : g2, b_n, grouped == 1 ? g2 : g, nz, nullptr, nullptr, &le)) fam = 0;
+        } else if (fam) le = launch_gemm(nullptr, a_t, b_n, g, nz);
     }
     restore();
     if (!fam) { drop(); return bad_shape("gemm desc test: the descriptor does not qualify for the route"); }
@@ -6283,6 +6436,34 @@
     drop();
     HIPCHK(le);
     *family = fam;
+    return GMRF_OK;
+}
+
+gmrf_status gmrf_test_gemm_desc(int32_t device, int32_t route, const int64_t* desc, const double* abt,
+                                const double* A, int64_t nA, const double* B, int64_t nB, double* C, int64_t nC,
+                                const double* D, int64_t nD, const double* tA, int64_t ntA, double* tC, int64_t ntC,
+                                const double* tD, int64_t ntD, const int32_t* kb_m, int64_t n_kb_m, const int32_t* kb_n,
+                                int64_t n_kb_n, const int32_t* ke_n, int64_t n_ke_n, double* samples, int64_t n_samples,
+                                double* mean, int64_t n_mean, int32_t* family) {
+    return gemm_desc_run(device, route, desc, abt, A, nA, B, nB, C, nC, D, nD, tA, ntA, tC, ntC, tD, ntD, kb_m, n_kb_m, kb_n, n_kb_n,
+                         ke_n, n_ke_n, samples, n_samples, mean, n_mean, family, nullptr, 0, 0);
+}
+gmrf_status gmrf_test_gemm_env(int32_t device, int32_t route, const int64_t* desc, const double* abt,
+                               const double* A, int64_t nA, const double* B, int64_t nB, double* C, int64_t nC,
+                               const double* D, int64_t nD, const double* tA, int64_t ntA, double* tC, int64_t ntC,
+                               const double* tD, int64_t ntD, const int32_t* kb_m, int64_t n_kb_m, const int32_t* kb_n,
+                               int64_t n_kb_n, const int32_t* ke_n, int64_t n_ke_n, const int32_t* ke_m, int64_t n_ke_m,
+                               int32_t grouped, int32_t* family) {
+    return gemm_desc_run(device, route, desc, abt, A, nA, B, nB, C, nC, D, nD, tA, ntA, tC, ntC, tD, ntD, kb_m, n_kb_m, kb_n, n_kb_n,
+                         ke_n, n_ke_n, nullptr, 0, nullptr, 0, family, ke_m, n_ke_m, grouped);
+}
+gmrf_status gmrf_test_envelope(gmrf_handle* h, int32_t* lo, int32_t* hi, int64_t cap, int64_t* n_vals, int32_t* state) {
+    if (!h || !n_vals || !state) return bad_shape("null argument");
+    const int64_t want = h->N * (h->bsp / 64);
+    const bool have = h->bsp % 256 == 0 && (int64_t)h->env_lo.size() == want && h->analyzed;
+    *n_vals = have ? want : 0;
+    *state = !have ? 0 : (h->env_ok ? 2 : 1);
+    for (int64_t i = 0; have && lo && hi && i < std::min(cap, want); ++i) { lo[i] = h->env_lo[(size_t)i]; hi[i] = h->env_hi[(size_t)i]; }
     return GMRF_OK;
 }
 
@@ -6618,6 +6799,33 @@
     for (int64_t v : sp.first) mix((uint64_t)v);
     out8[0] = sp.cmin; out8[1] = sp.rmax; out8[2] = (int64_t)sp.keys.size(); out8[3] = sp.max_row; out8[4] = sp.sparse_b;
     out8[5] = sp.bxt_ok; out8[6] = sp.ecap; out8[7] = (int64_t)(sum >> 1);
+    return GMRF_OK;
+}
+
+gmrf_status gmrf_test_envelope_csc(int64_t n, int64_t n_blocks, const int64_t* colptr, const int64_t* rowval, int32_t index_base,
+                                   int32_t* lo, int32_t* hi, double* units, int64_t cap, int64_t* n_vals) {
+    if (!colptr || !rowval || !n_vals) return bad_shape("null pointer");
+    if (n <= 0 || n_blocks <= 0 || n % n_blocks != 0) return bad_shape("n must be a positive multiple of N_blocks");
+    const int64_t bs = n / n_blocks, bsp = 64 * next_pow2((bs + 63) / 64);
+    std::vector<std::vector<HostEntry>> dg, lw;
+    GCHK(split_csc(n, n_blocks, bs, colptr, rowval, index_base, dg, lw));
+    SymbolicPlan sp;
+    build_symbolic(n_blocks, bsp, dg, lw, false, sp);
+    const int nt = (int)(bsp / 64), np = nt / 4;
+    *n_vals = bsp % 256 == 0 ? n_blocks * nt : 0;
+    if (*n_vals == 0 || !lo || !hi || cap < *n_vals) return GMRF_OK;
+    for (int64_t k = 0; k < *n_vals; ++k) { lo[k] = sp.env_lo[(size_t)k]; hi[k] = sp.env_hi[(size_t)k]; }
+    if (units) {
+        EnvHost eh;
+        derive_envelope(n_blocks, bsp, sp, eh);
+        for (int64_t i = 0; i < n_blocks; ++i)
+            for (int p = 0; p < np; ++p) {
+                const int* host = eh.host.data() + (size_t)((i * np + p) * 4) * nt;
+                const int m3 = nt - 4 * p - 4;
+                double* u = units + (i * np + p) * 3;
+                u[0] = env_units_pp(host, nt, m3, 0); u[1] = env_units_pp(host, nt, m3, 2); u[2] = env_units_upd(host, m3);
+            }
+    }
     return GMRF_OK;
 }
 
diff --git a/include/gmrf_hip.h b/include/gmrf_hip.h
--- a/include/gmrf_hip.h
+++ b/include/gmrf_hip.h
@@ -309,6 +309,13 @@
                                 const double* tD, int64_t ntD, const int32_t* kb_m, int64_t n_kb_m, const int32_t* kb_n,
                                 int64_t n_kb_n, const int32_t* ke_n, int64_t n_ke_n, double* samples, int64_t n_samples,
                                 double* mean, int64_t n_mean, int32_t* family);
+gmrf_status gmrf_test_gemm_env(int32_t device, int32_t route, const int64_t* desc, const double* abt,
+                               const double* A, int64_t nA, const double* B, int64_t nB, double* C, int64_t nC,
+                               const double* D, int64_t nD, const double* tA, int64_t ntA, double* tC, int64_t ntC,
+                               const double* tD, int64_t ntD, const int32_t* kb_m, int64_t n_kb_m, const int32_t* kb_n,
+                               int64_t n_kb_n, const int32_t* ke_n, int64_t n_ke_n, const int32_t* ke_m, int64_t n_ke_m,
+                               int32_t grouped, int32_t* family);
+gmrf_status gmrf_test_envelope(gmrf_handle* h, int32_t* lo, int32_t* hi, int64_t cap, int64_t* n_vals, int32_t* state);
 gmrf_status gmrf_test_gemm_rate(int32_t device, int64_t M, int64_t N, int64_t K, int32_t transB,
                                 int32_t tri_flags, int32_t lower_only, int32_t batch,
                                 int32_t big, int32_t reps, double* ms_per_launch);
@@ -336,6 +343,9 @@
 gmrf_status gmrf_test_symbolic_csc(int64_t n, int64_t n_blocks, const int64_t* colptr, const int64_t* rowval,
                                    int32_t index_base, int64_t* out8);
 
+gmrf_status gmrf_test_envelope_csc(int64_t n, int64_t n_blocks, const int64_t* colptr, const int64_t* rowval, int32_t index_base,
+                                   int32_t* lo, int32_t* hi, double* units, int64_t cap, int64_t* n_vals);
+
 #ifdef __cplusplus
 }
 #endif
```

After: 56630 solves/s (median of 6 runs). +3.1%, better.
